# nunofachada/cl_ops

Measured on AMD Instinct MI355X. Metric: Mkeys/s sorting 2^28 uint32 (satradix, 4-bit digits); achieved % of HBM roofline, higher is better.
Workload: dtype u32

## Files before the change

### cl_ops_amd/_hip.py

```python
import ctypes as C
import os

_HERE = os.path.dirname(os.path.abspath(__file__))
LIB_PATH = os.environ.get("CLO_HIP_LIBRARY") or os.path.join(_HERE, "lib", "libcl_ops_hip.so")

if not os.path.exists(LIB_PATH):
    raise ImportError(
        "cl_ops_amd: %s is missing. Build it with `python -c 'import __graft_entry__ as g; g.build()'` "
        "or `make -C cl_ops_amd/csrc` (needs hipcc). There is no fallback path." % LIB_PATH)

lib = C.CDLL(LIB_PATH, mode=C.RTLD_GLOBAL)

vp, sz, ci = C.c_void_p, C.c_size_t, C.c_int


class DeviceProps(C.Structure):
    _fields_ = [("name", C.c_char * 128), ("compute_units", ci), ("max_threads_per_block", ci),
                ("wavefront_size", ci), ("lds_bytes_per_block", sz), ("global_mem_bytes", sz),
                ("gcn_arch", C.c_char * 64)]


def _sig(name, restype, *argtypes):
    try:
        f = getattr(lib, name)
    except AttributeError:
        if os.environ.get("CLO_HIP_LIBRARY"):
            return None
        raise
    f.restype = restype
    f.argtypes = list(argtypes)
    return f


_sig("clo_hip_device_count", ci, C.POINTER(ci))
_sig("clo_hip_set_device", ci, ci)
_sig("clo_hip_get_device", ci, C.POINTER(ci))
_sig("clo_hip_get_device_props", ci, ci, C.POINTER(DeviceProps))
_sig("clo_hip_stream_create", ci, C.POINTER(vp))
_sig("clo_hip_stream_create_high_priority", ci, C.POINTER(vp))
_sig("clo_hip_stream_destroy", ci, vp)
_sig("clo_hip_stream_synchronize", ci, vp)
_sig("clo_hip_malloc", ci, C.POINTER(vp), sz)
_sig("clo_hip_free", ci, vp)
_sig("clo_hip_memcpy_h2d_async", ci, vp, vp, sz, vp)
_sig("clo_hip_memcpy_d2h_async", ci, vp, vp, sz, vp)
_sig("clo_hip_memcpy_d2d_async", ci, vp, vp, sz, vp)
_sig("clo_hip_memset_async", ci, vp, ci, sz, vp)
_sig("clo_hip_host_register", ci, vp, sz)
_sig("clo_hip_host_unregister", ci, vp)
_sig("clo_hip_stream_is_capturing", ci, vp)
_sig("clo_hip_graph_capture_begin", ci, vp)
_sig("clo_hip_graph_capture_end", ci, vp, C.POINTER(vp))
_sig("clo_hip_graph_launch", ci, vp, vp)
_sig("clo_hip_graph_destroy", ci, vp)
_sig("clo_hip_timing_enabled", ci)
_sig("clo_hip_event_create", ci, C.POINTER(vp))
_sig("clo_hip_event_destroy", ci, vp)
_sig("clo_hip_event_record", ci, vp, vp)
_sig("clo_hip_event_synchronize", ci, vp)
_sig("clo_hip_event_query", ci, vp)
_sig("clo_hip_env_refresh", None)
_sig("clo_hip_event_elapsed_ms", ci, vp, vp, C.POINTER(C.c_float))
_sig("clo_hip_stream_wait_event", ci, vp, vp)
_sig("clo_hip_error_string", C.c_char_p, ci)
_sig("clo_hip_scan_workspace_bytes", sz, sz, ci, ci)
_sig("clo_hip_scan_workspace_init", ci, vp, sz, vp)
_sig("clo_hip_scan_workspace_forget", ci, vp)
_sig("clo_hip_scan_workspace_set_epoch", ci, vp, C.c_uint, vp)
_sig("clo_hip_scan_exclusive", ci, vp, vp, sz, ci, ci, ci, vp, sz, vp)
_sig("clo_hip_scan_exclusive_carry", ci, vp, vp, sz, ci, ci, ci, vp, vp, vp, sz, vp)
_sig("clo_hip_scan_fp_workspace_bytes", sz, sz, ci)
_sig("clo_hip_scan_is_typed", ci, ci, ci)
_sig("clo_hip_scan_typed_workspace_bytes", sz, sz, ci)
_sig("clo_hip_scan_exclusive_typed", ci, vp, vp, sz, ci, ci, vp, sz, vp)
_sig("clo_hip_scan_exclusive_fp", ci, vp, vp, sz, ci, ci, vp, sz, vp)
_sig("clo_hip_reduce_sum", ci, vp, sz, ci, ci, vp, vp)
_sig("clo_hip_radix_workspace_bytes", sz, sz, ci, ci, ci)
_sig("clo_hip_radix_polls", ci, sz, ci, ci)
_sig("clo_hip_radix_sort", ci, vp, vp, vp, sz, ci, ci, ci, ci, ci, vp, sz, vp)
_sig("clo_hip_radix_takes_first_digits", ci, sz, ci, ci, ci)
_sig("clo_hip_radix_sort_fed", ci, vp, vp, vp, sz, ci, ci, ci, ci, ci, vp, vp, sz, vp)
_sig("clo_hip_radix_seg_workspace_bytes", sz, sz, ci, ci, ci)
_sig("clo_hip_radix_sort_segmented", ci, vp, vp, vp, sz, C.POINTER(sz), ci, C.POINTER(sz), C.POINTER(sz), C.POINTER(ci), ci,
     ci, ci, ci, ci, vp, sz, vp, C.POINTER(ci))
_sig("clo_hip_radix_sort_segmented2", ci, vp, vp, vp, vp, sz, C.POINTER(sz), ci, C.POINTER(sz), C.POINTER(sz), C.POINTER(ci), C.POINTER(ci), ci,
     ci, ci, ci, ci, vp, sz, vp, C.POINTER(ci))
_sig("clo_hip_msd_histogram", ci, vp, sz, ci, ci, ci, ci, vp, vp)
_sig("clo_hip_msd_partition", ci, vp, vp, sz, ci, ci, ci, ci, vp, vp, sz, vp)
_sig("clo_hip_msd_workspace_bytes", sz, sz, ci, ci)
_sig("clo_hip_bitonic_padded_numel", sz, sz)
_sig("clo_hip_bitonic_simple", ci, vp, sz, ci, ci, ci, ci, ci, ci, C.POINTER(ci), vp)
_sig("clo_hip_bitonic_tiled", ci, vp, sz, ci, ci, ci, ci, ci, ci, C.POINTER(ci), vp)
_sig("clo_hip_bitonic_any", ci, vp, sz, ci, ci, ci, ci, ci, ci, C.POINTER(ci), vp)
_sig("clo_hip_kernel_lds_bytes", sz, C.c_char_p, ci, ci)
_sig("clo_hip_bitonic_jit_create", ci, ci, ci, C.c_char_p, C.c_char_p, C.c_char_p, C.POINTER(vp), C.POINTER(C.c_char_p))
_sig("clo_hip_bitonic_jit_destroy", None, vp)
_sig("clo_hip_bitonic_jit_sort", ci, vp, vp, sz, ci, C.POINTER(ci), vp)
_sig("clo_hip_bitonic_jit_gselect", ci, vp, vp, vp, sz, vp)
_sig("clo_hip_check_status", ci, vp, vp)
_sig("clo_hip_rccl_unique_id", ci, vp)
_sig("clo_hip_rccl_comm_create", ci, C.POINTER(vp), vp, ci, ci)
_sig("clo_hip_rccl_comm_destroy", ci, vp)
_sig("clo_hip_rccl_comm_abort", ci, vp)
_sig("clo_hip_rccl_all_gather_u64", ci, vp, vp, vp, sz, vp)
_sig("clo_hip_rccl_all_to_all_v", ci, vp, ci, ci, vp, vp, vp, vp, vp, vp, vp)
_sig("clo_hip_set_launch_observer", ci, vp, vp)
_sig("clo_hip_radix_jit_create", ci, ci, ci, C.c_char_p, C.c_char_p, C.POINTER(vp), C.POINTER(C.c_char_p))
_sig("clo_hip_radix_jit_destroy", None, vp)
_sig("clo_hip_radix_jit_sort", ci, vp, vp, vp, vp, vp, sz, ci, vp, sz, vp)
_sig("clo_hip_timing_enable", ci, ci)
_sig("clo_hip_timing_reset", ci)
_sig("clo_hip_timing_read", ci, C.c_char_p, C.POINTER(C.c_uint), C.POINTER(C.c_float))


CLO_HIP_EARGS, CLO_HIP_EUNSUPPORTED, CLO_HIP_EWORKSPACE, CLO_HIP_ETIMEOUT = -1, -2, -3, -4


class HipError(RuntimeError):
    def __init__(self, status, what=""):
        self.status = status
        msg = lib.clo_hip_error_string(status)
        super().__init__("%s: %s (status %d)" % (what or "clo_hip", msg.decode() if msg else "?", status))


def check(status, what=""):
    if status != 0:
        raise HipError(status, what)


def device_count():
    n = ci(0)
    st = lib.clo_hip_device_count(C.byref(n))
    return n.value if st == 0 else 0


def timing_read(label):
    n, ms = C.c_uint(0), C.c_float(0)
    check(lib.clo_hip_timing_read(label.encode(), C.byref(n), C.byref(ms)), "clo_hip_timing_read")
    return n.value, ms.value
```

### cl_ops_amd/csrc/hip/clo_hip_internal.h

```cpp
#ifndef CLO_HIP_INTERNAL_H
#define CLO_HIP_INTERNAL_H

#include <stddef.h>
#include <stdint.h>

#include "clo_hip.h"

#define CLO_WS_STATUS_OFFSET 0
#define CLO_WS_EPOCH_WORD    2
#define CLO_WS_DONE_WORD     3
#define CLO_WS_TICKET_WORD   16
#define CLO_WS_MAX_PASSES    64
#define CLO_WS_HEADER_BYTES  512

struct clo_hip_env_t { unsigned max_spins; int radix_sweep; int r1_pools; int no_digits; int bitonic_merge2; };
const clo_hip_env_t* clo_hip_env();
int clo_radixw_preload();

inline bool clo_misaligned(const void* p, size_t align) { return ((uintptr_t) p & (align - 1)) != 0; }
inline bool clo_ws_misaligned(const void* ws) { return clo_misaligned(ws, CLO_HIP_WORKSPACE_ALIGN); }

#ifdef __HIPCC__
#include <hip/hip_runtime.h>

void clo_timing_begin(const char* label, hipStream_t s);
void clo_timing_end(hipStream_t s);
struct clo_timing_scope {
	hipStream_t s;
	clo_timing_scope(const char* label, hipStream_t stream) : s(stream) { clo_timing_begin(label, s); }
	~clo_timing_scope() { clo_timing_end(s); }
};

struct clo_keyx {
	unsigned long long sign, field;
	int kind;
};
template <typename E>
__device__ __forceinline__ E clo_keyx_fwd(E x, const clo_keyx& k) {
	if (k.kind == 1) return (E) (x ^ (E) k.sign);
	if (k.kind == 2) return (E) (x ^ ((x & (E) k.sign) ? (E) k.field : (E) k.sign));
	return x;
}
template <typename E>
__device__ __forceinline__ E clo_keyx_inv(E x, const clo_keyx& k) {
	if (k.kind == 1) return (E) (x ^ (E) k.sign);
	if (k.kind == 2) return (E) (x ^ ((x & (E) k.sign) ? (E) k.sign : (E) k.field));
	return x;
}
inline clo_keyx clo_keyx_make(int kind, int key_shift, int key_bits) {
	clo_keyx k = { 0, 0, 0 };
	if (kind == 1 || kind == 2) {
		k.kind = kind;
		k.sign = 1ull << (key_shift + key_bits - 1);
		k.field = (key_bits >= 64 ? ~0ull : ((1ull << key_bits) - 1ull)) << key_shift;
	}
	return k;
}

struct clo_kv_io {
	const void* keys_in;
	const unsigned* values_in;
	void* keys_out;
	unsigned* values_out;
};

size_t clo_radix4_workspace_bytes(size_t n, int elem_size, int digit_bits, int key_bits);
int clo_radix4_sort_kv(const clo_kv_io& io, void* pairs_a, void* pairs_b, size_t n, int key_size, int key_shift,
	int key_bits, int digit_bits, clo_keyx kx, void* ws, hipStream_t s);
size_t clo_radix4_partition_workspace_bytes(size_t n, int elem_size, int bits);
int clo_radix4_partition(const void* src, void* dst, size_t n, int elem_size, unsigned shift, int bits,
	unsigned long long* counts, void* ws, hipStream_t s);
int clo_radix4_sort(const void* src, void* dst, void* tmp, size_t n, int elem_size, int key_shift,
	int key_bits, int digit_bits, clo_keyx kx, const unsigned char* first_dig, void* ws, hipStream_t s);
int clo_radix4_takes_first_digits(size_t n, int elem_size, int digit_bits);
size_t clo_radix4_lds_bytes(int elem_size, int digit_bits);
int clo_radix1_applies(size_t n, int elem_size, int digit_bits);
size_t clo_radix1_workspace_bytes(size_t n, int elem_size, int key_bits);
int clo_radix1_sort(const void* src, void* dst, void* tmp, size_t n, int elem_size, int key_shift, int key_bits,
	clo_keyx kx, void* ws, unsigned* status, hipStream_t s);
int clo_bitonic_tiled_e1(void* data, size_t numel, int key_shift, int key_bits, int key_size, int key_kind, int descending, int* launches, hipStream_t s);
int clo_bitonic_tiled_e2(void* data, size_t numel, int key_shift, int key_bits, int key_size, int key_kind, int descending, int* launches, hipStream_t s);
int clo_bitonic_tiled_e4(void* data, size_t numel, int key_shift, int key_bits, int key_size, int key_kind, int descending, int* launches, hipStream_t s);
int clo_bitonic_tiled_e8(void* data, size_t numel, int key_shift, int key_bits, int key_size, int key_kind, int descending, int* launches, hipStream_t s);
size_t clo_radixw_lds_bytes(int digit_bits);
struct clo_radix_counters { unsigned* thist; unsigned* toff; unsigned* partial; unsigned* tinfo; unsigned tiles; bool big; };
int clo_radixw_launch_tilehist(const void* in, size_t n, int elem_size, int bits, unsigned shift, unsigned mask,
	const clo_radix_counters& c, clo_keyx kx, hipStream_t s);
int clo_radixw_launch_tilehist_kv(const void* keys, size_t n, int key_size, int bits, unsigned shift, unsigned mask,
	const clo_radix_counters& c, clo_keyx kx, hipStream_t s);
int clo_radixw_launch_tilehist_bytes(const unsigned char* dig, size_t n, int elem_size, int bits, unsigned mask,
	const clo_radix_counters& c, hipStream_t s);
int clo_radixw_launch_offsets(int bits, const clo_radix_counters& c, const unsigned** dbase, hipStream_t s);
size_t clo_radixw_partial_rows(size_t tiles);

#define CLO_SEG_MAX 256
struct clo_seg_tile { unsigned in_base, count_seg, out_base, seg_n; };
struct clo_seg_chunk { unsigned t0, tend, c_first, seg_last; };
struct clo_seg_pieces {
	unsigned n[CLO_SEG_MAX], in_base[CLO_SEG_MAX];
	unsigned short seg[CLO_SEG_MAX];
};
struct clo_seg_tables { const clo_seg_tile* tiles; const clo_seg_chunk* chunks; unsigned ntiles, nchunks, nseg; };
int clo_radixw_launch_tilehist_seg(const void* in, const void* in2, const clo_seg_tables& sg, int elem_size, int bits, unsigned shift, unsigned mask,
	const clo_radix_counters& c, hipStream_t s);
int clo_radixw_launch_tilehist_bytes_seg(const unsigned char* dig, const clo_seg_tables& sg, int elem_size, int bits, unsigned mask,
	const clo_radix_counters& c, hipStream_t s);
int clo_radixw_launch_offsets_seg(int bits, const clo_radix_counters& c, const clo_seg_tables& sg, const unsigned** dbase, hipStream_t s);
size_t clo_radixw_partial_rows_seg(size_t chunks, size_t nseg);
int clo_radixw_seg_build(const size_t* piece_n, const size_t* piece_base, const int* piece_seg, const int* piece_src, int npieces, int nseg, size_t tile,
	clo_seg_tile* tiles, clo_seg_chunk* chunks, unsigned* ntiles, unsigned* nchunks, hipStream_t s);
void clo_radixw_seg_bounds(size_t numel, int npieces, int nseg, size_t tile, size_t* max_tiles, size_t* max_chunks);
size_t clo_radix4_seg_workspace_bytes(size_t n, int nseg, int elem_size, int digit_bits);
int clo_radix4_sort_segmented(const void* src, const void* src2, void* a, void* b, size_t n, const size_t* seg_counts, int nseg,
	const size_t* piece_n, const size_t* piece_base, const int* piece_seg, const int* piece_src, int npieces, int elem_size, int key_shift,
	int key_bits, int digit_bits, void* ws, hipStream_t s, int* result_in_b);

typedef unsigned long long clo_u64;

#define CLO_LB_EPOCH_MAX ((1u << 30) - 1u)
#define CLO_LB_AGG    1u
#define CLO_LB_PREFIX 2u

__device__ __forceinline__ clo_u64 clo_lb_pack(unsigned epoch, unsigned state, unsigned value) {
	return ((clo_u64) ((epoch << 2) | state) << 32) | value;
}
__device__ __forceinline__ unsigned clo_lb_tag(clo_u64 g) { return (unsigned) (g >> 32); }
__device__ __forceinline__ unsigned clo_lb_val(clo_u64 g) { return (unsigned) g; }

__device__ __forceinline__ clo_u64 clo_ld_agent(const clo_u64* p) {
	return __hip_atomic_load(p, __ATOMIC_RELAXED, __HIP_MEMORY_SCOPE_AGENT);
}
__device__ __forceinline__ void clo_st_agent(clo_u64* p, clo_u64 v) {
	__hip_atomic_store(p, v, __ATOMIC_RELAXED, __HIP_MEMORY_SCOPE_AGENT);
}

#define CLO_MAX_SPINS (1u << 22)

__device__ __forceinline__ unsigned clo_lane_id() {
	return __builtin_amdgcn_mbcnt_hi(~0u, __builtin_amdgcn_mbcnt_lo(~0u, 0u));
}

__device__ __forceinline__ unsigned clo_mbcnt(clo_u64 mask) {
	return __builtin_amdgcn_mbcnt_hi((unsigned) (mask >> 32),
		__builtin_amdgcn_mbcnt_lo((unsigned) mask, 0u));
}

__device__ __forceinline__ void clo_lds_barrier() {
	__builtin_amdgcn_fence(__ATOMIC_RELEASE, "workgroup", "local");
	__builtin_amdgcn_s_barrier();
	__builtin_amdgcn_fence(__ATOMIC_ACQUIRE, "workgroup", "local");
}

template <int CTRL, int ROW_MASK, typename T>
__device__ __forceinline__ T clo_dpp_add(T x) {
	static_assert(sizeof(T) == 4 || sizeof(T) == 8, "32- or 64-bit integers");
	if constexpr (sizeof(T) == 4) {
		return (T) ((unsigned) x + (unsigned) __builtin_amdgcn_update_dpp(0, (int) x, CTRL, ROW_MASK, 0xF, true));
	} else {
		const unsigned long long v = (unsigned long long) x;
		const unsigned lo = (unsigned) __builtin_amdgcn_update_dpp(0, (int) (unsigned) v, CTRL, ROW_MASK, 0xF, true);
		const unsigned hi = (unsigned) __builtin_amdgcn_update_dpp(0, (int) (unsigned) (v >> 32), CTRL, ROW_MASK, 0xF, true);
		return (T) (v + (((unsigned long long) hi << 32) | lo));
	}
}

template <typename T>
__device__ __forceinline__ T clo_wave_scan_inclusive(T x, unsigned lane) {
	(void) lane;
	x = clo_dpp_add<0x111, 0xF>(x);
	x = clo_dpp_add<0x112, 0xF>(x);
	x = clo_dpp_add<0x114, 0xF>(x);
	x = clo_dpp_add<0x118, 0xF>(x);
	x = clo_dpp_add<0x142, 0xA>(x);
	x = clo_dpp_add<0x143, 0xC>(x);
	return x;
}

template <typename T>
__device__ __forceinline__ T clo_wave_reduce_sum(T x) {
	const T incl = clo_wave_scan_inclusive<T>(x, 0u);
	if constexpr (sizeof(T) == 4) {
		return (T) (unsigned) __builtin_amdgcn_readlane((int) incl, 63);
	} else {
		const unsigned long long v = (unsigned long long) incl;
		const unsigned lo = (unsigned) __builtin_amdgcn_readlane((int) (unsigned) v, 63);
		const unsigned hi = (unsigned) __builtin_amdgcn_readlane((int) (unsigned) (v >> 32), 63);
		return (T) (((unsigned long long) hi << 32) | lo);
	}
}

#endif
#endif
```

### cl_ops_amd/csrc/hip/clo_hip_radix.hip

```cpp
#include <hip/hip_runtime.h>

#include "clo_hip.h"
#include "clo_hip_internal.h"

namespace {

constexpr int HIST_THREADS = 256;
constexpr int HIST_ITEMS = 16;

template <typename E>
__global__ __launch_bounds__(HIST_THREADS)
void clo_msd_hist_kernel(const E* __restrict__ in, size_t n, unsigned shift, unsigned mask,
	unsigned long long* __restrict__ counts) {
	__shared__ unsigned h[HIST_THREADS / 64][8];
	const unsigned tid = threadIdx.x, wave = tid >> 6;
	if (tid < (HIST_THREADS / 64) * 8) (&h[0][0])[tid] = 0;
	__syncthreads();
	const size_t chunk = (size_t) HIST_THREADS * HIST_ITEMS;
	for (size_t base = (size_t) blockIdx.x * chunk; base < n; base += (size_t) gridDim.x * chunk) {
		#pragma unroll
		for (int i = 0; i < HIST_ITEMS; ++i) {
			const size_t idx = base + (size_t) i * HIST_THREADS + tid;
			if (idx < n) atomicAdd(&h[wave][(unsigned) (in[idx] >> shift) & mask & 7u], 1u);
		}
	}
	__syncthreads();
	if (tid <= mask && tid < 8) {
		unsigned s = 0;
		#pragma unroll
		for (int w = 0; w < HIST_THREADS / 64; ++w) s += h[w][tid];
		if (s) atomicAdd(&counts[tid], (unsigned long long) s);
	}
}

template <typename E>
int msd_hist_impl(const void* src, size_t n, unsigned shift, unsigned mask, uint64_t* counts, hipStream_t s) {
	unsigned blocks = (unsigned) ((n + HIST_THREADS * HIST_ITEMS - 1) / (HIST_THREADS * HIST_ITEMS));
	if (blocks > 2048) blocks = 2048;
	if (blocks == 0) blocks = 1;
	hipLaunchKernelGGL((clo_msd_hist_kernel<E>), dim3(blocks), dim3(HIST_THREADS), 0, s,
		(const E*) src, n, shift, mask, (unsigned long long*) counts);
	return (int) hipGetLastError();
}

}

extern "C" {

size_t clo_hip_radix_workspace_bytes(size_t numel, int elem_size, int key_bits, int digit_bits) {
	if (digit_bits < 1 || digit_bits > 8 || key_bits < 1) return 0;
	return clo_radix4_workspace_bytes(numel, elem_size, digit_bits, key_bits);
}

int clo_hip_radix_polls(size_t numel, int elem_size, int digit_bits) {
	return clo_radix1_applies(numel, elem_size, digit_bits) ? 1 : 0;
}

int clo_hip_radix_takes_first_digits(size_t numel, int elem_size, int key_kind, int digit_bits) {
	return key_kind == 0 ? clo_radix4_takes_first_digits(numel, elem_size, digit_bits) : 0;
}

int clo_hip_radix_sort(const void* src, void* dst, void* tmp, size_t numel,
	int elem_size, int key_shift, int key_bits, int key_kind, int digit_bits,
	void* workspace, size_t workspace_bytes, void* stream) {
	return clo_hip_radix_sort_fed(src, dst, tmp, numel, elem_size, key_shift, key_bits, key_kind, digit_bits, nullptr,
		workspace, workspace_bytes, stream);
}

int clo_hip_radix_sort_fed(const void* src, void* dst, void* tmp, size_t numel,
	int elem_size, int key_shift, int key_bits, int key_kind, int digit_bits, const unsigned char* first_digits,
	void* workspace, size_t workspace_bytes, void* stream) {

	if (numel == 0) return 0;
	if (!src || !dst || !tmp || !workspace || tmp == src || tmp == dst || clo_ws_misaligned(workspace)) return CLO_HIP_EARGS;
	if (key_bits < 1 || key_shift < 0 || key_shift + key_bits > 8 * elem_size) return CLO_HIP_EARGS;
	if (key_kind < 0 || key_kind > 2) return CLO_HIP_EARGS;
	if (key_kind == 2 && key_bits != 16 && key_bits != 32 && key_bits != 64) return CLO_HIP_EARGS;
	if (digit_bits < 1 || digit_bits > 8) return CLO_HIP_EUNSUPPORTED;
	if (numel > 0xffffffffull) return CLO_HIP_EARGS;
	if (workspace_bytes < clo_hip_radix_workspace_bytes(numel, elem_size, key_bits, digit_bits)) return CLO_HIP_EWORKSPACE;
	hipStream_t s = (hipStream_t) stream;
	const clo_keyx kx = clo_keyx_make(key_kind, key_shift, key_bits);
	return clo_radix4_sort(src, dst, tmp, numel, elem_size, key_shift, key_bits, digit_bits, kx, first_digits, workspace, s);
}

size_t clo_hip_radix_kv_workspace_bytes(size_t numel, int key_size, int key_bits, int digit_bits) {
	if (key_size != 1 && key_size != 2 && key_size != 4) return 0;
	return clo_hip_radix_workspace_bytes(numel, 8, key_bits, digit_bits);
}

int clo_hip_radix_sort_kv(const void* keys_in, const void* values_in, void* keys_out, void* values_out, void* pairs_a, void* pairs_b,
	size_t numel, int key_size, int key_shift, int key_bits, int key_kind, int digit_bits,
	void* workspace, size_t workspace_bytes, void* stream) {
	if (numel == 0) return 0;
	if (!keys_in || !values_out || !pairs_a || !pairs_b || pairs_a == pairs_b || !workspace || clo_ws_misaligned(workspace)) return CLO_HIP_EARGS;
	const void* arrays[4] = { keys_in, values_in, keys_out, values_out };
	for (int i = 0; i < 4; ++i) if (arrays[i] == pairs_a || arrays[i] == pairs_b) return CLO_HIP_EARGS;
	if (key_size != 1 && key_size != 2 && key_size != 4) return CLO_HIP_EUNSUPPORTED;
	if (key_bits < 1 || key_shift < 0 || key_shift + key_bits > 8 * key_size) return CLO_HIP_EARGS;
	if (key_kind < 0 || key_kind > 2) return CLO_HIP_EARGS;
	if (key_kind == 2 && key_bits != 16 && key_bits != 32) return CLO_HIP_EARGS;
	if (digit_bits < 1 || digit_bits > 8) return CLO_HIP_EUNSUPPORTED;
	if (numel > 0xffffffffull) return CLO_HIP_EARGS;
	if (workspace_bytes < clo_hip_radix_kv_workspace_bytes(numel, key_size, key_bits, digit_bits)) return CLO_HIP_EWORKSPACE;
	const clo_kv_io io = { keys_in, (const unsigned*) values_in, keys_out, (unsigned*) values_out };
	const clo_keyx kx = clo_keyx_make(key_kind, 32 + key_shift, key_bits);
	return clo_radix4_sort_kv(io, pairs_a, pairs_b, numel, key_size, 32 + key_shift, key_bits, digit_bits, kx, workspace, (hipStream_t) stream);
}

int clo_hip_radix_preload(void) { return clo_radixw_preload(); }

size_t clo_hip_radix_seg_workspace_bytes(size_t numel, int nseg, int elem_size, int digit_bits) {
	return clo_radix4_seg_workspace_bytes(numel, nseg, elem_size, digit_bits);
}

int clo_hip_radix_sort_segmented(const void* src, void* a, void* b, size_t numel, const size_t* seg_counts, int nseg,
	const size_t* piece_counts, const size_t* piece_offsets, const int* piece_segment, int npieces,
	int elem_size, int key_shift, int key_bits, int digit_bits, void* workspace, size_t workspace_bytes, void* stream, int* result_in_b) {
	return clo_hip_radix_sort_segmented2(src, nullptr, a, b, numel, seg_counts, nseg, piece_counts, piece_offsets, piece_segment, nullptr, npieces,
		elem_size, key_shift, key_bits, digit_bits, workspace, workspace_bytes, stream, result_in_b);
}

int clo_hip_radix_sort_segmented2(const void* src, const void* src2, void* a, void* b, size_t numel, const size_t* seg_counts, int nseg,
	const size_t* piece_counts, const size_t* piece_offsets, const int* piece_segment, const int* piece_source, int npieces,
	int elem_size, int key_shift, int key_bits, int digit_bits, void* workspace, size_t workspace_bytes, void* stream, int* result_in_b) {
	if (!result_in_b) return CLO_HIP_EARGS;
	*result_in_b = 0;
	if (numel == 0) return 0;
	if (!src || !a || !b || a == b || src == b || !workspace || !seg_counts || nseg < 1 || nseg > CLO_SEG_MAX) return CLO_HIP_EARGS;
	if (clo_ws_misaligned(workspace)) return CLO_HIP_EARGS;
	if (npieces < 0 || npieces > CLO_SEG_MAX || (npieces > 0 && (!piece_counts || !piece_offsets || !piece_segment))) return CLO_HIP_EARGS;
	if (elem_size != 4 && elem_size != 8) return CLO_HIP_EUNSUPPORTED;
	if (digit_bits != 4 && digit_bits != 8) return CLO_HIP_EUNSUPPORTED;
	if (key_bits < 1 || key_shift < 0 || key_shift + key_bits > 8 * elem_size) return CLO_HIP_EARGS;
	if (numel > 0xffffffffull) return CLO_HIP_EARGS;
	size_t total = 0;
	for (int i = 0; i < nseg; ++i) total += seg_counts[i];
	if (total != numel) return CLO_HIP_EARGS;
	if (npieces > 0) {
		size_t per[CLO_SEG_MAX];
		for (int k = 0; k < nseg; ++k) per[k] = 0;
		for (int i = 0; i < npieces; ++i) {
			if (piece_segment[i] < 0 || piece_segment[i] >= nseg || piece_offsets[i] > 0xffffffffull || piece_counts[i] > numel) return CLO_HIP_EARGS;
			if (piece_source && piece_source[i] != 0 && (piece_source[i] != 1 || !src2 || src2 == b)) return CLO_HIP_EARGS;
			per[piece_segment[i]] += piece_counts[i];
		}
		for (int k = 0; k < nseg; ++k) if (per[k] != seg_counts[k]) return CLO_HIP_EARGS;
	}
	const size_t need = clo_radix4_seg_workspace_bytes(numel, nseg, elem_size, digit_bits);
	if (need == 0) return CLO_HIP_EUNSUPPORTED;
	if (workspace_bytes < need) return CLO_HIP_EWORKSPACE;
	return clo_radix4_sort_segmented(src, src2, a, b, numel, seg_counts, nseg, piece_counts, piece_offsets, piece_segment, npieces > 0 ? piece_source : nullptr, npieces,
		elem_size, key_shift, key_bits, digit_bits, workspace, (hipStream_t) stream, result_in_b);
}

size_t clo_hip_msd_workspace_bytes(size_t numel, int elem_size, int bucket_bits) {
	if (bucket_bits < 1 || bucket_bits > 8) return 0;
	return clo_radix4_partition_workspace_bytes(numel, elem_size, bucket_bits);
}

int clo_hip_msd_histogram(const void* src, size_t numel, int elem_size,
	int key_shift, int key_bits, int bucket_bits, uint64_t* counts_dev, void* stream) {
	if (!counts_dev || clo_misaligned(counts_dev, 8) || bucket_bits < 1 || bucket_bits > 3 || bucket_bits > key_bits) return CLO_HIP_EARGS;
	hipStream_t s = (hipStream_t) stream;
	hipError_t e = hipMemsetAsync(counts_dev, 0, sizeof(uint64_t) << bucket_bits, s);
	if (e != hipSuccess) return (int) e;
	if (numel == 0) return 0;
	if (!src) return CLO_HIP_EARGS;
	const unsigned shift = (unsigned) (key_shift + key_bits - bucket_bits), mask = (1u << bucket_bits) - 1u;
	switch (elem_size) {
		case 4: return msd_hist_impl<uint32_t>(src, numel, shift, mask, counts_dev, s);
		case 8: return msd_hist_impl<uint64_t>(src, numel, shift, mask, counts_dev, s);
		default: return CLO_HIP_EUNSUPPORTED;
	}
}

int clo_hip_msd_partition(const void* src, void* dst, size_t numel, int elem_size,
	int key_shift, int key_bits, int bucket_bits, uint64_t* counts_dev,
	void* workspace, size_t workspace_bytes, void* stream) {
	hipStream_t s = (hipStream_t) stream;
	if (bucket_bits < 1 || bucket_bits > 8 || bucket_bits > key_bits) return CLO_HIP_EARGS;
	if (clo_misaligned(counts_dev, 8) || clo_ws_misaligned(workspace)) return CLO_HIP_EARGS;
	if (numel == 0) {
		if (counts_dev) return (int) hipMemsetAsync(counts_dev, 0, sizeof(uint64_t) << bucket_bits, s);
		return 0;
	}
	if (!src || !dst || src == dst || !workspace) return CLO_HIP_EARGS;
	if (numel > 0xffffffffull) return CLO_HIP_EARGS;
	if (elem_size != 4 && elem_size != 8) return CLO_HIP_EUNSUPPORTED;
	if (workspace_bytes < clo_hip_msd_workspace_bytes(numel, elem_size, bucket_bits)) return CLO_HIP_EWORKSPACE;
	const unsigned shift = (unsigned) (key_shift + key_bits - bucket_bits);
	return clo_radix4_partition(src, dst, numel, elem_size, shift, bucket_bits,
		(unsigned long long*) counts_dev, workspace, s);
}

}
```

### cl_ops_amd/csrc/hip/clo_hip_radix4.hip

```cpp
#include <hip/hip_runtime.h>

#include <cstdlib>
#include <type_traits>

#include "clo_hip.h"
#include "clo_hip_internal.h"
#include "clo_hip_radix_rank.h"

namespace {

template <int KB> struct kv_key;
template <> struct kv_key<1> { typedef uint8_t type; };
template <> struct kv_key<2> { typedef uint16_t type; };
template <> struct kv_key<4> { typedef uint32_t type; };

template <int KB, int ITEMS>
__device__ __forceinline__ void kv_load_pairs(const clo_kv_io& kv, size_t at, unsigned valid, bool aligned, uint64_t (&pair)[ITEMS]) {
	typedef typename kv_key<KB>::type K;
	const K* kp = reinterpret_cast<const K*>(kv.keys_in) + at;
	K k[ITEMS];
	unsigned v[ITEMS];
	if (valid == (unsigned) ITEMS) {
		load_blocked<K, ITEMS>(kp, k, aligned);
		if (kv.values_in) {
			load_blocked<unsigned, ITEMS>(kv.values_in + at, v, aligned);
		} else {
			#pragma unroll
			for (int i = 0; i < ITEMS; ++i) v[i] = (unsigned) at + (unsigned) i;
		}
	} else {
		#pragma unroll
		for (int i = 0; i < ITEMS; ++i) {
			k[i] = (unsigned) i < valid ? kp[i] : (K) 0;
			v[i] = (unsigned) i < valid ? (kv.values_in ? kv.values_in[at + i] : (unsigned) at + (unsigned) i) : 0u;
		}
	}
	#pragma unroll
	for (int i = 0; i < ITEMS; ++i) pair[i] = ((uint64_t) k[i] << 32) | v[i];
}

template <int KB>
__device__ __forceinline__ void kv_store_pair(const clo_kv_io& kv, unsigned gi, uint64_t e) {
	typedef typename kv_key<KB>::type K;
	if (kv.keys_out) reinterpret_cast<K*>(kv.keys_out)[gi] = (K) (e >> 32);
	kv.values_out[gi] = (unsigned) e;
}

template <typename E, int LB, int HB, bool BIG, bool DIG = false, bool SEG = false, int KV_IN = 0, int KV_OUT = 0>
__global__ __launch_bounds__((pair_shape<E, BIG>::THREADS), (pair_shape<E, BIG>::THREADS >= 1024 ? 8 : 6))
void clo_radix4_pair_kernel(const E* __restrict__ in, E* __restrict__ out, size_t n,
	unsigned shift, unsigned mask_lo, unsigned mask_hi,
	const unsigned* __restrict__ thist, const unsigned* __restrict__ toff, const unsigned* __restrict__ dbase,
	const unsigned* __restrict__ tinfo, int aligned,
	clo_keyx kx_in, clo_keyx kx_out, unsigned char* __restrict__ dig_out = nullptr, unsigned next_shift = 0,
	const clo_seg_tile* __restrict__ tdesc = nullptr, const E* __restrict__ in2 = nullptr, clo_kv_io kv = clo_kv_io()) {
	static_assert((KV_IN == 0 && KV_OUT == 0) || (sizeof(E) == 8 && !SEG), "key-value passes: 8-byte pairs, one array");

	constexpr int THREADS = pair_shape<E, BIG>::THREADS;
	constexpr int ITEMS = pair_shape<E, BIG>::ITEMS;
	constexpr int TILE = THREADS * ITEMS;
	constexpr int WAVES = THREADS / 64;
	constexpr int R2 = 1 << (LB + HB);
	constexpr int HMAX = pc_words<(LB > HB ? LB : HB)>::H;
	static_assert(R2 <= 256 && R2 <= THREADS, "one thread per combined digit, scanned by the first four waves");

	__shared__ __attribute__((aligned(16))) E s_stage[TILE];
	constexpr bool ALIAS = pair_shape<E, BIG>::ALIAS;
	__shared__ unsigned s_end[ALIAS ? 1 : THREADS * PC_END_STRIDE];
	__shared__ unsigned s_wtot[WAVES][HMAX];
	__shared__ __attribute__((aligned(16))) unsigned s_wbase[WAVES][HMAX];
	__shared__ unsigned s_delta[R2];
	__shared__ unsigned s_w4[4];

	const unsigned tid = threadIdx.x, lane = tid & 63u, wave = tid >> 6;
	const unsigned per_xcd = SEG ? (unsigned) ((n + 7) / 8) : (unsigned) ((n + (size_t) TILE * 8 - 1) / ((size_t) TILE * 8));
	const unsigned tile = (blockIdx.x & 7u) * per_xcd + (blockIdx.x >> 3);
	size_t base = (size_t) tile * TILE;
	unsigned count, n32;
	if constexpr (SEG) {
		if (tile >= (unsigned) n) return;
		const clo_seg_tile td = tdesc[tile];
		base = (size_t) td.in_base;
		count = td.count_seg & 0xffffu;
		n32 = td.seg_n;
		out += td.out_base;
		if constexpr (DIG) dig_out += td.out_base;
		dbase += (size_t) ((td.count_seg >> 16) & 0x7fffu) * R2;
		if (td.count_seg >> 31) in = in2;
	} else {
		if (base >= n) return;
		count = (n - base) < (size_t) TILE ? (unsigned) (n - base) : (unsigned) TILE;
		n32 = n > 0xffffffffull ? 0xffffffffu : (unsigned) n;
	}
	const bool full = count == (unsigned) TILE;
	const unsigned tbase = tid * ITEMS;
	const unsigned mask2 = (mask_hi << LB) | mask_lo;

	__builtin_amdgcn_s_setprio(3);
	unsigned h2 = 0, goff = 0;
	if (tid < (unsigned) R2) {
		h2 = thist[(size_t) tile * R2 + tid];
		goff = toff[(size_t) tile * R2 + tid];
		if (dbase) goff += dbase[tid];
	}
	E key[ITEMS];
	if constexpr (KV_IN != 0) {
		kv_load_pairs<KV_IN, ITEMS>(kv, base + tbase, full ? (unsigned) ITEMS : (count > tbase ? count - tbase : 0u), aligned != 0, key);
	} else if (full) {
		if constexpr (SEG) load_blocked_unaligned<E, ITEMS>(in + base + tbase, key);
		else load_blocked<E, ITEMS>(in + base + tbase, key, aligned != 0);
	} else {
		#pragma unroll
		for (int i = 0; i < ITEMS; ++i) key[i] = (tbase + i < count) ? in[base + tbase + i] : (E) 0;
	}
	__builtin_amdgcn_s_setprio(0);
	if (kx_in.kind) {
		#pragma unroll
		for (int i = 0; i < ITEMS; ++i) key[i] = clo_keyx_fwd<E>(key[i], kx_in);
	}
	{
		const unsigned incl2 = clo_wave_scan_inclusive<unsigned>(h2, lane);
		if (lane == 63 && wave < 4) s_w4[wave] = incl2;
		if (tid < (unsigned) R2) s_delta[tid] = goff - (incl2 - h2);
	}

	const bool single = tinfo[tile] != 0u;

	if (!single) {
		pc_local_split<E, LB, THREADS, ITEMS, HMAX, pc_no_mid, pc_no_counted, ALIAS>(key, shift, mask_lo, count, s_stage, s_end, s_wtot, s_wbase);
	} else {
		if (full) {
			constexpr int PER = ITEMS * (int) sizeof(E) >= 16 ? 16 / (int) sizeof(E) : ITEMS;
			typedef E vec16 __attribute__((ext_vector_type(PER)));
			#pragma unroll
			for (int k = 0; k < ITEMS / PER; ++k) {
				vec16 t;
				#pragma unroll
				for (int q = 0; q < PER; ++q) t[q] = key[k * PER + q];
				*reinterpret_cast<vec16*>(&s_stage[tbase + k * PER]) = t;
			}
		} else {
			#pragma unroll
			for (int i = 0; i < ITEMS; ++i) if (tbase + i < count) s_stage[tbase + i] = key[i];
		}
		clo_lds_barrier();
	}

	if (tid < (unsigned) R2) {
		unsigned before = 0;
		#pragma unroll
		for (unsigned w = 0; w < 4; ++w) if (w < wave) before += s_w4[w];
		s_delta[tid] -= before;
	}
	if (single) {
		__syncthreads();
	} else if (mask_hi != 0) {
		if (full) {
			constexpr int PER = ITEMS * (int) sizeof(E) >= 16 ? 16 / (int) sizeof(E) : ITEMS;
			typedef E vec16 __attribute__((ext_vector_type(PER)));
			#pragma unroll
			for (int k = 0; k < ITEMS / PER; ++k) {
				const vec16 t = *reinterpret_cast<const vec16*>(&s_stage[tbase + k * PER]);
				#pragma unroll
				for (int q = 0; q < PER; ++q) key[k * PER + q] = t[q];
			}
		} else {
			#pragma unroll
			for (int i = 0; i < ITEMS; ++i) if (tbase + i < count) key[i] = s_stage[tbase + i];
		}
		pc_local_split<E, HB, THREADS, ITEMS, HMAX, pc_no_mid, pc_no_counted, ALIAS>(key, shift + LB, mask_hi, count, s_stage, s_end, s_wtot, s_wbase);
	} else {
		__syncthreads();
	}

	constexpr int VEC = sizeof(E) >= 8 ? 1 : 4;
	typedef E vecE __attribute__((ext_vector_type(VEC)));
	typedef E vecE_u __attribute__((ext_vector_type(VEC), aligned(sizeof(E))));
	const bool dig_bytes = DIG && VEC == 4 && (next_shift & 7u) == 0u && next_shift < 8u * (unsigned) sizeof(E);
	const unsigned dig_b = next_shift >> 3;
	const unsigned dig_sel_lo = 0x0c0c0400u + dig_b * 0x0101u, dig_sel_hi = 0x04000c0cu + dig_b * 0x01010000u;
	const unsigned nbits2 = (unsigned) __builtin_popcount(mask2);
	const auto scatter = [&](auto kx_tag) {
		constexpr bool KX = decltype(kx_tag)::value;
		#pragma unroll
		for (int j = 0; j < ITEMS / VEC; ++j) {
			const unsigned p = (j * THREADS + tid) * VEC;
			if (full) {
				const vecE v = *reinterpret_cast<const vecE*>(&s_stage[p]);
				const unsigned d0 = pc_digit<E>(v[0], shift, mask2, nbits2), dl = pc_digit<E>(v[VEC - 1], shift, mask2, nbits2);
				const unsigned gi0 = p + s_delta[d0];
				if (d0 == dl && gi0 <= n32 - VEC) {
					vecE vo = v;
					if constexpr (KX) {
						#pragma unroll
						for (int k = 0; k < VEC; ++k) vo[k] = clo_keyx_inv<E>(v[k], kx_out);
					}
					if constexpr (KV_OUT != 0) kv_store_pair<KV_OUT>(kv, gi0, vo[0]);
					else *reinterpret_cast<vecE_u*>(&out[gi0]) = vo;
					if constexpr (DIG) {
						if constexpr (VEC == 4) {
							typedef unsigned u32_u __attribute__((aligned(1)));
							unsigned dg;
							if (dig_bytes)
								dg = __builtin_amdgcn_perm((unsigned) v[1], (unsigned) v[0], dig_sel_lo) | __builtin_amdgcn_perm((unsigned) v[3], (unsigned) v[2], dig_sel_hi);
							else
								dg = ((unsigned) (v[0] >> next_shift) & 255u) | (((unsigned) (v[1] >> next_shift) & 255u) << 8)
									| (((unsigned) (v[2] >> next_shift) & 255u) << 16) | ((unsigned) (v[3] >> next_shift) << 24);
							*reinterpret_cast<u32_u*>(dig_out + gi0) = dg;
						} else {
							dig_out[gi0] = (unsigned char) (v[0] >> next_shift);
						}
					}
				} else {
					#pragma unroll
					for (int k = 0; k < VEC; ++k) {
						const unsigned gi = p + k + s_delta[pc_digit<E>(v[k], shift, mask2, nbits2)];
						if (gi < n32) {
							if constexpr (KV_OUT != 0) kv_store_pair<KV_OUT>(kv, gi, KX ? clo_keyx_inv<E>(v[k], kx_out) : v[k]);
							else out[gi] = KX ? clo_keyx_inv<E>(v[k], kx_out) : v[k];
							if constexpr (DIG) dig_out[gi] = (unsigned char) (v[k] >> next_shift);
						}
					}
				}
			} else {
				#pragma unroll
				for (int k = 0; k < VEC; ++k) {
					if (p + k < count) {
						const E e = s_stage[p + k];
						const unsigned gi = p + k + s_delta[pc_digit<E>(e, shift, mask2, nbits2)];
						if (gi < n32) {
							if constexpr (KV_OUT != 0) kv_store_pair<KV_OUT>(kv, gi, KX ? clo_keyx_inv<E>(e, kx_out) : e);
							else out[gi] = KX ? clo_keyx_inv<E>(e, kx_out) : e;
							if constexpr (DIG) dig_out[gi] = (unsigned char) (e >> next_shift);
						}
					}
				}
			}
		}
	};
	if (kx_out.kind) scatter(std::true_type()); else scatter(std::false_type());
}

constexpr int SMALL_TILE = 512 * 8;
template <typename E> struct small_big { static constexpr int THREADS = 1024, ITEMS = sizeof(E) == 8 ? 8 : 16, TILE = THREADS * ITEMS; };

template <typename E, int BITS, int THREADS, int ITEMS>
__global__ __launch_bounds__(THREADS)
void clo_radix4_small_kernel(const E* in, E* out, unsigned n, unsigned key_shift, unsigned key_bits, clo_keyx kx) {
	constexpr int H = pc_words<BITS>::H;
	constexpr int WAVES = THREADS / 64;
	__shared__ __attribute__((aligned(16))) E s_stage[THREADS * ITEMS];
	__shared__ unsigned s_end[THREADS * PC_END_STRIDE];
	__shared__ unsigned s_wtot[WAVES][H];
	__shared__ __attribute__((aligned(16))) unsigned s_wbase[WAVES][H];

	const unsigned tbase = threadIdx.x * ITEMS;
	E key[ITEMS];
	#pragma unroll
	for (int i = 0; i < ITEMS; ++i) key[i] = (tbase + i < n) ? clo_keyx_fwd<E>(in[tbase + i], kx) : (E) 0;
	for (unsigned done = 0; done < key_bits; done += BITS) {
		const unsigned bits = key_bits - done < (unsigned) BITS ? key_bits - done : (unsigned) BITS;
		pc_local_split<E, BITS, THREADS, ITEMS, H>(key, key_shift + done, (1u << bits) - 1u, n,
			s_stage, s_end, s_wtot, s_wbase);
		if constexpr (ITEMS * sizeof(E) >= 16) {
			constexpr int PER = 16 / (int) sizeof(E);
			typedef E vec16 __attribute__((ext_vector_type(PER)));
			#pragma unroll
			for (int k = 0; k < ITEMS / PER; ++k) {
				const vec16 t = *reinterpret_cast<const vec16*>(&s_stage[tbase + k * PER]);
				#pragma unroll
				for (int q = 0; q < PER; ++q) key[k * PER + q] = t[q];
			}
		} else {
			#pragma unroll
			for (int i = 0; i < ITEMS; ++i) if (tbase + i < n) key[i] = s_stage[tbase + i];
		}
	}
	#pragma unroll
	for (int i = 0; i < ITEMS; ++i) if (tbase + i < n) out[tbase + i] = clo_keyx_inv<E>(key[i], kx);
}


struct rp_layout { size_t thist, toff, partial, tinfo, dig, total, tiles; bool big; };

rp_layout rp_make_layout(size_t n, int elem_size, int pass_bits, bool digits = true) {
	rp_layout L;
	const size_t R2 = (size_t) 1 << pass_bits;
	L.big = clo_radix_big_tiles(n, elem_size);
	const size_t tile = clo_pair_tile_elems(elem_size, L.big);
	L.tiles = (n + tile - 1) / tile;
	if (L.tiles == 0) L.tiles = 1;
	const size_t per = L.tiles * R2 * sizeof(unsigned);
	L.thist = CLO_WS_HEADER_BYTES;
	L.toff = L.thist + per;
	L.partial = L.toff + per;
	L.tinfo = L.partial + ((clo_radixw_partial_rows(L.tiles) * R2 * sizeof(unsigned) + 255) & ~(size_t) 255);
	L.total = L.tinfo + ((L.tiles * sizeof(unsigned) + 255) & ~(size_t) 255);
	L.dig = 0;
	if (digits && clo_radix_digit_stream(n, elem_size)) {
		L.dig = L.total;
		L.total += (n + 255) & ~(size_t) 255;
	}
	return L;
}

template <typename Layout>
clo_radix_counters rp_counters(void* ws, const Layout& L, size_t tiles) {
	char* w = (char*) ws;
	return { (unsigned*) (w + L.thist), (unsigned*) (w + L.toff), (unsigned*) (w + L.partial), (unsigned*) (w + L.tinfo), (unsigned) tiles, L.big };
}

struct rp_digits { unsigned shift, mask_lo, mask_hi, mask, next_shift; };

template <int LB, int HB>
rp_digits rp_pass_digits(int p, int key_shift, int key_bits) {
	constexpr int PB = LB + HB;
	const int rem = key_bits - p * PB;
	const int bits = rem < PB ? rem : PB;
	const int lo_bits = bits < LB ? bits : LB, hi_bits = bits - lo_bits;
	rp_digits d;
	d.shift = (unsigned) (key_shift + p * PB);
	d.mask_lo = (1u << lo_bits) - 1u;
	d.mask_hi = (1u << hi_bits) - 1u;
	d.mask = (d.mask_hi << LB) | d.mask_lo;
	d.next_shift = d.shift + PB;
	return d;
}

template <typename E, int LB, int HB, bool SEG = false, int KB = 0>
void rp_launch_pass(const clo_radix_counters& c, const rp_digits& d, const E* in, E* out, size_t n, const unsigned* dbase, int aligned,
	clo_keyx kx_in, clo_keyx kx_out, unsigned char* dig_out, hipStream_t s, const clo_seg_tile* tdesc = nullptr, const E* in2 = nullptr,
	bool kv_in = false, bool kv_out = false, const clo_kv_io& kv = clo_kv_io()) {
	const unsigned tiles = SEG ? (unsigned) n : c.tiles;
	const auto launch = [&](auto big, auto dig, auto kvi, auto kvo) {
		constexpr bool BIG = decltype(big)::value, DIG = decltype(dig)::value;
		hipLaunchKernelGGL((clo_radix4_pair_kernel<E, LB, HB, BIG, DIG, SEG, decltype(kvi)::value, decltype(kvo)::value>),
			dim3((tiles + 7u) / 8u * 8u), dim3(pair_shape<E, BIG>::THREADS), 0, s,
			in, out, n, d.shift, d.mask_lo, d.mask_hi, c.thist, c.toff, dbase, c.tinfo, aligned, kx_in, kx_out, dig_out, d.next_shift, tdesc, in2, kv);
	};
	const auto shape = [&](auto kvi, auto kvo) {
		constexpr bool BIG_OK = sizeof(E) >= 4, DIG_OK = BIG_OK && LB == 4 && HB == 4 && decltype(kvo)::value == 0;
		if constexpr (DIG_OK) {
			if (c.big && dig_out) { launch(std::true_type(), std::true_type(), kvi, kvo); return; }
		}
		if constexpr (BIG_OK) {
			if (c.big) { launch(std::true_type(), std::false_type(), kvi, kvo); return; }
		}
		launch(std::false_type(), std::false_type(), kvi, kvo);
	};
	typedef std::integral_constant<int, 0> plain;
	typedef std::integral_constant<int, KB> key;
	if (kv_in && kv_out) shape(key(), key());
	else if (kv_in) shape(key(), plain());
	else if (kv_out) shape(plain(), key());
	else shape(plain(), plain());
}

int kv_unpack(const uint64_t* pairs, const clo_kv_io& io, size_t n, int key_size, hipStream_t s);

template <typename E, int LB, int HB, int KB = 0>
int rp_sort_impl(const E* src, E* dst, E* tmp, size_t n, int key_shift, int key_bits, clo_keyx kx, const unsigned char* first_dig,
	const clo_kv_io& kv, void* ws, hipStream_t s) {
	constexpr int PB = LB + HB;
	const int passes = (key_bits + PB - 1) / PB;
	const rp_layout L = rp_make_layout(n, (int) sizeof(E), PB);
	const clo_radix_counters c = rp_counters(ws, L, L.tiles);
	const bool no_dig = clo_hip_env()->no_digits != 0;
	constexpr bool DIG_OK = LB == 4 && HB == 4 && sizeof(E) >= 4;
	unsigned char* dig = (DIG_OK && L.dig != 0 && passes > 1 && !no_dig) ? (unsigned char*) ws + L.dig : nullptr;
	const clo_keyx kx_none = { 0, 0, 0 };
	const bool split_after = KB != 0 && passes == 1 && (kv.keys_out == kv.keys_in || (const void*) kv.values_out == (const void*) kv.values_in);
	const bool kv_aligned = (uintptr_t) kv.keys_in % 16 == 0 && (uintptr_t) kv.values_in % 16 == 0;

	hipError_t e;

	const bool inplace_odd = (dst == src) && (passes % 2 == 1);
	const E* cur_in = src;
	for (int p = 0; p < passes; ++p) {
		E* cur_out;
		if (inplace_odd) cur_out = (p % 2 == 0) ? tmp : dst;
		else cur_out = ((passes - 1 - p) % 2 == 0) ? dst : tmp;
		const bool kv_in = KB != 0 && p == 0, kv_out = KB != 0 && p + 1 == passes && !split_after;
		const rp_digits d = rp_pass_digits<LB, HB>(p, key_shift, key_bits);
		{
			clo_timing_scope timing("radix_hist", s);
			const unsigned char* hist_bytes = (dig && p > 0) ? dig : ((DIG_OK && c.big && p == 0 && kx.kind == 0) ? first_dig : nullptr);
			const int st = kv_in ? clo_radixw_launch_tilehist_kv(kv.keys_in, n, KB, PB, d.shift, d.mask, c, kx, s)
				: hist_bytes ? clo_radixw_launch_tilehist_bytes(hist_bytes, n, (int) sizeof(E), PB, d.mask, c, s)
				: clo_radixw_launch_tilehist(cur_in, n, (int) sizeof(E), PB, d.shift, d.mask, c, p == 0 ? kx : kx_none, s);
			if (st != 0) return st;
		}
		const unsigned* dbase = nullptr;
		{
			clo_timing_scope timing("radix_offsets", s);
			const int st = clo_radixw_launch_offsets(PB, c, &dbase, s);
			if (st != 0) return st;
		}
		{
			clo_timing_scope timing("radix_pass", s);
			const int aligned = kv_in ? (int) kv_aligned : (int) ((uintptr_t) cur_in % 16 == 0);
			rp_launch_pass<E, LB, HB, false, KB>(c, d, cur_in, cur_out, n, dbase, aligned, p == 0 ? kx : kx_none, p + 1 == passes ? kx : kx_none,
				p + 1 < passes ? dig : nullptr, s, nullptr, nullptr, kv_in, kv_out, kv);
		}
		cur_in = cur_out;
	}
	e = hipGetLastError();
	if (e != hipSuccess) return (int) e;
	if (inplace_odd) {
		e = hipMemcpyAsync(dst, tmp, n * sizeof(E), hipMemcpyDeviceToDevice, s);
		if (e != hipSuccess) return (int) e;
	}
	if constexpr (KB != 0) {
		if (split_after) return kv_unpack(dst, kv, n, KB, s);
	}
	return 0;
}

template <typename E>
int rp_dispatch(const void* src, void* dst, void* tmp, size_t n, int key_shift, int key_bits, int digit_bits,
	clo_keyx kx, const unsigned char* first_dig, void* ws, hipStream_t s) {
	#define CLO_RP(LB, HB) return rp_sort_impl<E, LB, HB>((const E*) src, (E*) dst, (E*) tmp, n, key_shift, key_bits, kx, first_dig, clo_kv_io(), ws, s)
	switch (digit_bits) {
		case 1: CLO_RP(1, 1);
		case 2: CLO_RP(2, 2);
		case 3: CLO_RP(3, 3);
		case 4: CLO_RP(4, 4);
		case 5: CLO_RP(3, 2);
		case 6: CLO_RP(3, 3);
		case 7: CLO_RP(4, 3);
		case 8: CLO_RP(4, 4);
		default: return CLO_HIP_EUNSUPPORTED;
	}
	#undef CLO_RP
}

template <int R, int R2>
__global__ __launch_bounds__(256)
void clo_radix4_counts_kernel(const unsigned* __restrict__ thist, unsigned tiles, unsigned long long* __restrict__ counts) {
	constexpr int G = 256 / R;
	__shared__ unsigned long long s_part[G][R];
	const unsigned tid = threadIdx.x, d = tid % R, g = tid / R;
	unsigned long long c = 0;
	for (unsigned t = g; t < tiles; t += G) c += thist[(size_t) t * R2 + d];
	s_part[g][d] = c;
	__syncthreads();
	if (tid < (unsigned) R) {
		unsigned long long tot = 0;
		#pragma unroll
		for (int k = 0; k < G; ++k) tot += s_part[k][tid];
		counts[tid] = tot;
	}
}

template <int R, int R2>
__global__ __launch_bounds__(256)
void clo_radix4_counts_from_bases_kernel(const unsigned* __restrict__ dbase, unsigned n, unsigned long long* __restrict__ counts) {
	const unsigned d = threadIdx.x;
	if (d < (unsigned) R) counts[d] = (unsigned long long) ((d + 1u < (unsigned) R2 ? dbase[d + 1u] : n) - dbase[d]);
}

template <typename E, int BITS, int LB, int HB>
int r4_partition_impl(const E* src, E* dst, size_t n, unsigned shift, unsigned long long* counts, void* ws, hipStream_t s) {
	constexpr unsigned R = 1u << BITS;
	constexpr int PB = LB + HB;
	constexpr bool TWO = BITS > 3;
	static_assert(TWO ? PB == BITS : (LB == BITS && HB == BITS), "see above");
	const rp_layout L = rp_make_layout(n, (int) sizeof(E), PB, false);
	const clo_radix_counters c = rp_counters(ws, L, L.tiles);
	const clo_keyx kx_none = { 0, 0, 0 };
	hipError_t e = hipMemsetAsync(ws, 0, CLO_WS_HEADER_BYTES, s);
	if (e != hipSuccess) return (int) e;
	clo_timing_scope timing("msd_partition", s);
	const rp_digits d = rp_pass_digits<LB, HB>(0, (int) shift, BITS);
	int st = clo_radixw_launch_tilehist(src, n, (int) sizeof(E), PB, d.shift, d.mask, c, kx_none, s);
	if (st != 0) return st;
	const unsigned* dbase = nullptr;
	st = clo_radixw_launch_offsets(PB, c, &dbase, s);
	if (st != 0) return st;
	if (counts) {
		if (dbase) hipLaunchKernelGGL((clo_radix4_counts_from_bases_kernel<R, (1 << PB)>), dim3(1), dim3(256), 0, s, dbase, (unsigned) n, counts);
		else hipLaunchKernelGGL((clo_radix4_counts_kernel<R, (1 << PB)>), dim3(1), dim3(256), 0, s, c.thist, c.tiles, counts);
	}
	rp_launch_pass<E, LB, HB>(c, d, src, dst, n, dbase, (int) ((uintptr_t) src % 16 == 0), kx_none, kx_none, nullptr, s);
	return (int) hipGetLastError();
}

struct rp_seg_layout { size_t thist, toff, partial, tinfo, tdesc, cdesc, dig, total, tile, max_tiles, max_chunks; bool big; };

rp_seg_layout rp_make_seg_layout(size_t n, int nseg, int elem_size) {
	rp_seg_layout L;
	const size_t R2 = 256;
	L.big = clo_radix_big_tiles(n, elem_size);
	L.tile = clo_pair_tile_elems(elem_size, L.big);
	clo_radixw_seg_bounds(n, CLO_SEG_MAX, nseg, L.tile, &L.max_tiles, &L.max_chunks);
	const size_t per = L.max_tiles * R2 * sizeof(unsigned);
	const auto up = [](size_t x) { return (x + 255) & ~(size_t) 255; };
	L.thist = CLO_WS_HEADER_BYTES;
	L.toff = L.thist + per;
	L.partial = L.toff + per;
	L.tinfo = L.partial + up(clo_radixw_partial_rows_seg(L.max_chunks, (size_t) nseg) * R2 * sizeof(unsigned));
	L.tdesc = L.tinfo + up(L.max_tiles * sizeof(unsigned));
	L.cdesc = L.tdesc + 2 * up(L.max_tiles * sizeof(clo_seg_tile));
	L.total = L.cdesc + 2 * up(L.max_chunks * sizeof(clo_seg_chunk));
	L.dig = 0;
	if (clo_radix_digit_stream(n, elem_size)) {
		L.dig = L.total;
		L.total += up(n);
	}
	return L;
}

template <typename E>
int rp_sort_seg_impl(const E* src, const E* src2, E* a, E* b, size_t n, const size_t* seg_counts, int nseg,
	const size_t* piece_n, const size_t* piece_base, const int* piece_seg, const int* piece_src, int npieces, int key_shift, int key_bits, void* ws,
	hipStream_t s, int* result_in_b) {
	constexpr int LB = 4, HB = 4, PB = 8;
	const int passes = (key_bits + PB - 1) / PB;
	const rp_seg_layout L = rp_make_seg_layout(n, nseg, (int) sizeof(E));
	const clo_radix_counters c = rp_counters(ws, L, 0);
	const auto up = [](size_t x) { return (x + 255) & ~(size_t) 255; };
	size_t seg_base[CLO_SEG_MAX];
	int seg_id[CLO_SEG_MAX];
	{
		size_t at = 0;
		for (int k = 0; k < nseg; ++k) { seg_base[k] = at; seg_id[k] = k; at += seg_counts[k]; }
	}
	clo_seg_tables sg0, sg;
	sg.tiles = (const clo_seg_tile*) ((char*) ws + L.tdesc);
	sg.chunks = (const clo_seg_chunk*) ((char*) ws + L.cdesc);
	sg.nseg = (unsigned) nseg;
	{
		clo_timing_scope timing("radix_seg_tables", s);
		int st = clo_radixw_seg_build(seg_counts, seg_base, seg_id, nullptr, nseg, nseg, L.tile, (clo_seg_tile*) sg.tiles, (clo_seg_chunk*) sg.chunks, &sg.ntiles, &sg.nchunks, s);
		if (st != 0) return st;
		sg0 = sg;
		if (npieces > 0) {
			sg0.tiles = (const clo_seg_tile*) ((char*) ws + L.tdesc + up(L.max_tiles * sizeof(clo_seg_tile)));
			sg0.chunks = (const clo_seg_chunk*) ((char*) ws + L.cdesc + up(L.max_chunks * sizeof(clo_seg_chunk)));
			st = clo_radixw_seg_build(piece_n, piece_base, piece_seg, piece_src, npieces, nseg, L.tile, (clo_seg_tile*) sg0.tiles, (clo_seg_chunk*) sg0.chunks, &sg0.ntiles, &sg0.nchunks, s);
			if (st != 0) return st;
		}
	}
	*result_in_b = passes % 2;
	if (sg.ntiles == 0) return 0;
	if (sg.ntiles > L.max_tiles || sg.nchunks > L.max_chunks || sg0.ntiles > L.max_tiles || sg0.nchunks > L.max_chunks)
		return CLO_HIP_EWORKSPACE;
	unsigned char* dig = (L.dig != 0 && passes > 1) ? (unsigned char*) ws + L.dig : nullptr;
	const clo_keyx kx_none = { 0, 0, 0 };
	const E* cur_in = src;
	for (int p = 0; p < passes; ++p) {
		const clo_seg_tables& sgp = p == 0 ? sg0 : sg;
		E* cur_out = p % 2 == 0 ? b : a;
		const rp_digits d = rp_pass_digits<LB, HB>(p, key_shift, key_bits);
		{
			clo_timing_scope timing("radix_hist", s);
			const int st = (dig && p > 0)
				? clo_radixw_launch_tilehist_bytes_seg(dig, sgp, (int) sizeof(E), PB, d.mask, c, s)
				: clo_radixw_launch_tilehist_seg(cur_in, p == 0 ? src2 : nullptr, sgp, (int) sizeof(E), PB, d.shift, d.mask, c, s);
			if (st != 0) return st;
		}
		const unsigned* dbase = nullptr;
		{
			clo_timing_scope timing("radix_offsets", s);
			const int st = clo_radixw_launch_offsets_seg(PB, c, sgp, &dbase, s);
			if (st != 0) return st;
		}
		{
			clo_timing_scope timing("radix_pass", s);
			rp_launch_pass<E, LB, HB, true>(c, d, cur_in, cur_out, (size_t) sgp.ntiles, dbase, 0, kx_none, kx_none, p + 1 < passes ? dig : nullptr, s,
				sgp.tiles, p == 0 ? src2 : nullptr);
		}
		cur_in = cur_out;
	}
	return (int) hipGetLastError();
}

template <typename E>
int small_dispatch(const void* src, void* dst, size_t n, int key_shift, int key_bits, int digit_bits, clo_keyx kx, hipStream_t s) {
	clo_timing_scope timing("radix_small", s);
	#define CLO_SMALL(B) case B: \
		if (n <= (size_t) SMALL_TILE) \
			hipLaunchKernelGGL((clo_radix4_small_kernel<E, B, 512, 8>), dim3(1), dim3(512), 0, s, \
				(const E*) src, (E*) dst, (unsigned) n, (unsigned) key_shift, (unsigned) key_bits, kx); \
		else if (n <= (size_t) 1024 * 8) \
			hipLaunchKernelGGL((clo_radix4_small_kernel<E, B, 1024, 8>), dim3(1), dim3(1024), 0, s, \
				(const E*) src, (E*) dst, (unsigned) n, (unsigned) key_shift, (unsigned) key_bits, kx); \
		else \
			hipLaunchKernelGGL((clo_radix4_small_kernel<E, B, small_big<E>::THREADS, small_big<E>::ITEMS>), dim3(1), dim3(small_big<E>::THREADS), 0, s, \
				(const E*) src, (E*) dst, (unsigned) n, (unsigned) key_shift, (unsigned) key_bits, kx); \
		break
	switch (digit_bits) {
		CLO_SMALL(1); CLO_SMALL(2); CLO_SMALL(3); CLO_SMALL(4);
		default: return CLO_HIP_EUNSUPPORTED;
	}
	#undef CLO_SMALL
	return (int) hipGetLastError();
}

constexpr int KV_PACK_THREADS = 256;

template <typename K>
__global__ __launch_bounds__(KV_PACK_THREADS)
void clo_radix_kv_pack_kernel(const K* __restrict__ keys, const unsigned* __restrict__ values, uint64_t* __restrict__ pairs, size_t n) {
	for (size_t i = (size_t) blockIdx.x * KV_PACK_THREADS + threadIdx.x; i < n; i += (size_t) gridDim.x * KV_PACK_THREADS)
		pairs[i] = ((uint64_t) keys[i] << 32) | (values ? values[i] : (unsigned) i);
}

template <typename K>
__global__ __launch_bounds__(KV_PACK_THREADS)
void clo_radix_kv_unpack_kernel(const uint64_t* __restrict__ pairs, K* __restrict__ keys, unsigned* __restrict__ values, size_t n) {
	for (size_t i = (size_t) blockIdx.x * KV_PACK_THREADS + threadIdx.x; i < n; i += (size_t) gridDim.x * KV_PACK_THREADS) {
		const uint64_t e = pairs[i];
		if (keys) keys[i] = (K) (e >> 32);
		values[i] = (unsigned) e;
	}
}

unsigned kv_pack_grid(size_t n) {
	const size_t g = (n + KV_PACK_THREADS - 1) / KV_PACK_THREADS;
	return (unsigned) (g < 8192 ? (g ? g : 1) : 8192);
}

int kv_pack(const clo_kv_io& io, uint64_t* pairs, size_t n, int key_size, hipStream_t s) {
	clo_timing_scope timing("radix_kv_pack", s);
	#define CLO_KVP(K) hipLaunchKernelGGL((clo_radix_kv_pack_kernel<K>), dim3(kv_pack_grid(n)), dim3(KV_PACK_THREADS), 0, s, (const K*) io.keys_in, io.values_in, pairs, n)
	switch (key_size) {
		case 1: CLO_KVP(uint8_t); break;
		case 2: CLO_KVP(uint16_t); break;
		case 4: CLO_KVP(uint32_t); break;
		default: return CLO_HIP_EUNSUPPORTED;
	}
	#undef CLO_KVP
	return (int) hipGetLastError();
}

int kv_unpack(const uint64_t* pairs, const clo_kv_io& io, size_t n, int key_size, hipStream_t s) {
	clo_timing_scope timing("radix_kv_unpack", s);
	#define CLO_KVU(K) hipLaunchKernelGGL((clo_radix_kv_unpack_kernel<K>), dim3(kv_pack_grid(n)), dim3(KV_PACK_THREADS), 0, s, pairs, (K*) io.keys_out, io.values_out, n)
	switch (key_size) {
		case 1: CLO_KVU(uint8_t); break;
		case 2: CLO_KVU(uint16_t); break;
		case 4: CLO_KVU(uint32_t); break;
		default: return CLO_HIP_EUNSUPPORTED;
	}
	#undef CLO_KVU
	return (int) hipGetLastError();
}

}

static size_t r4_pair_workspace_bytes(size_t n, int elem_size, int digit_bits) {
	return (rp_make_layout(n, elem_size, digit_bits <= 4 ? 2 * digit_bits : digit_bits).total + 255) & ~(size_t) 255;
}

size_t clo_radix4_workspace_bytes(size_t n, int elem_size, int digit_bits, int key_bits) {
	size_t b = r4_pair_workspace_bytes(n, elem_size, digit_bits);
	if (clo_radix1_applies(n, elem_size, digit_bits)) b += clo_radix1_workspace_bytes(n, elem_size, key_bits);
	return b;
}

size_t clo_radix4_seg_workspace_bytes(size_t n, int nseg, int elem_size, int digit_bits) {
	if ((digit_bits != 4 && digit_bits != 8) || (elem_size != 4 && elem_size != 8) || nseg < 1 || nseg > CLO_SEG_MAX) return 0;
	return rp_make_seg_layout(n, nseg, elem_size).total;
}

int clo_radix4_sort_segmented(const void* src, const void* src2, void* a, void* b, size_t n, const size_t* seg_counts, int nseg,
	const size_t* piece_n, const size_t* piece_base, const int* piece_seg, const int* piece_src, int npieces, int elem_size, int key_shift,
	int key_bits, int digit_bits, void* ws, hipStream_t s, int* result_in_b) {
	if (digit_bits != 4 && digit_bits != 8) return CLO_HIP_EUNSUPPORTED;
	if (elem_size == 4) return rp_sort_seg_impl<uint32_t>((const uint32_t*) src, (const uint32_t*) src2, (uint32_t*) a, (uint32_t*) b, n, seg_counts, nseg, piece_n, piece_base, piece_seg, piece_src, npieces, key_shift, key_bits, ws, s, result_in_b);
	if (elem_size == 8) return rp_sort_seg_impl<uint64_t>((const uint64_t*) src, (const uint64_t*) src2, (uint64_t*) a, (uint64_t*) b, n, seg_counts, nseg, piece_n, piece_base, piece_seg, piece_src, npieces, key_shift, key_bits, ws, s, result_in_b);
	return CLO_HIP_EUNSUPPORTED;
}

size_t clo_radix4_partition_workspace_bytes(size_t n, int elem_size, int bits) {
	return rp_make_layout(n, elem_size, bits <= 3 ? 2 * bits : bits, false).total;
}

int clo_radix4_partition(const void* src, void* dst, size_t n, int elem_size, unsigned shift, int bits,
	unsigned long long* counts, void* ws, hipStream_t s) {
	#define CLO_R4P(E, B, LB, HB) return r4_partition_impl<E, B, LB, HB>((const E*) src, (E*) dst, n, shift, counts, ws, s)
	if (elem_size == 4) {
		if (bits == 1) CLO_R4P(uint32_t, 1, 1, 1);
		if (bits == 2) CLO_R4P(uint32_t, 2, 2, 2);
		if (bits == 3) CLO_R4P(uint32_t, 3, 3, 3);
		if (bits == 4) CLO_R4P(uint32_t, 4, 2, 2);
		if (bits == 5) CLO_R4P(uint32_t, 5, 3, 2);
		if (bits == 6) CLO_R4P(uint32_t, 6, 3, 3);
		if (bits == 7) CLO_R4P(uint32_t, 7, 4, 3);
		if (bits == 8) CLO_R4P(uint32_t, 8, 4, 4);
	} else if (elem_size == 8) {
		if (bits == 1) CLO_R4P(uint64_t, 1, 1, 1);
		if (bits == 2) CLO_R4P(uint64_t, 2, 2, 2);
		if (bits == 3) CLO_R4P(uint64_t, 3, 3, 3);
		if (bits == 4) CLO_R4P(uint64_t, 4, 2, 2);
		if (bits == 5) CLO_R4P(uint64_t, 5, 3, 2);
		if (bits == 6) CLO_R4P(uint64_t, 6, 3, 3);
		if (bits == 7) CLO_R4P(uint64_t, 7, 4, 3);
		if (bits == 8) CLO_R4P(uint64_t, 8, 4, 4);
	}
	#undef CLO_R4P
	return CLO_HIP_EUNSUPPORTED;
}

size_t clo_radix4_lds_bytes(int elem_size, int digit_bits) {
	const size_t threads = 512;
	const int half = digit_bits <= 4 ? digit_bits : (digit_bits + 1) / 2;
	const size_t hmax = half >= 4 ? 8 : (half == 3 ? 4 : (half == 2 ? 2 : 1));
	const size_t pass_bits = digit_bits <= 4 ? 2 * digit_bits : digit_bits;
	const size_t items = elem_size == 8 ? 8 : 16;
	return threads * items * (size_t) elem_size + threads * PC_END_STRIDE * sizeof(unsigned)
		+ (2 * (threads / 64) * hmax + ((size_t) 1 << pass_bits) + 4) * sizeof(unsigned);
}

int clo_radix4_takes_first_digits(size_t n, int elem_size, int digit_bits) {
	if (elem_size < 4 || (digit_bits != 4 && digit_bits != 8) || clo_hip_env()->no_digits) return 0;
	if (clo_radix1_applies(n, elem_size, digit_bits)) return 0;
	return clo_radix_big_tiles(n, elem_size) ? 1 : 0;
}

int clo_radix4_sort(const void* src, void* dst, void* tmp, size_t n, int elem_size, int key_shift,
	int key_bits, int digit_bits, clo_keyx kx, const unsigned char* first_dig, void* ws, hipStream_t s) {
	const size_t small_max = elem_size == 8 ? (size_t) small_big<uint64_t>::TILE : (size_t) small_big<uint32_t>::TILE;
	if (n <= small_max && digit_bits <= 4) {
		switch (elem_size) {
			case 1: return small_dispatch<uint8_t>(src, dst, n, key_shift, key_bits, digit_bits, kx, s);
			case 2: return small_dispatch<uint16_t>(src, dst, n, key_shift, key_bits, digit_bits, kx, s);
			case 4: return small_dispatch<uint32_t>(src, dst, n, key_shift, key_bits, digit_bits, kx, s);
			case 8: return small_dispatch<uint64_t>(src, dst, n, key_shift, key_bits, digit_bits, kx, s);
			default: return CLO_HIP_EUNSUPPORTED;
		}
	}
	if (clo_radix1_applies(n, elem_size, digit_bits))
		return clo_radix1_sort(src, dst, tmp, n, elem_size, key_shift, key_bits, kx,
			(char*) ws + r4_pair_workspace_bytes(n, elem_size, digit_bits), (unsigned*) ws, s);
	switch (elem_size) {
		case 1: return rp_dispatch<uint8_t>(src, dst, tmp, n, key_shift, key_bits, digit_bits, kx, first_dig, ws, s);
		case 2: return rp_dispatch<uint16_t>(src, dst, tmp, n, key_shift, key_bits, digit_bits, kx, first_dig, ws, s);
		case 4: return rp_dispatch<uint32_t>(src, dst, tmp, n, key_shift, key_bits, digit_bits, kx, first_dig, ws, s);
		case 8: return rp_dispatch<uint64_t>(src, dst, tmp, n, key_shift, key_bits, digit_bits, kx, first_dig, ws, s);
		default: return CLO_HIP_EUNSUPPORTED;
	}
}

int clo_radix4_sort_kv(const clo_kv_io& io, void* pairs_a, void* pairs_b, size_t n, int key_size, int key_shift,
	int key_bits, int digit_bits, clo_keyx kx, void* ws, hipStream_t s) {
	uint64_t* pa = (uint64_t*) pairs_a;
	uint64_t* pb = (uint64_t*) pairs_b;
	const bool small = n <= (size_t) small_big<uint64_t>::TILE && digit_bits <= 4;
	if ((digit_bits == 4 || digit_bits == 8) && !small && !clo_radix1_applies(n, 8, digit_bits)) {
		switch (key_size) {
			case 1: return rp_sort_impl<uint64_t, 4, 4, 1>(nullptr, pa, pb, n, key_shift, key_bits, kx, nullptr, io, ws, s);
			case 2: return rp_sort_impl<uint64_t, 4, 4, 2>(nullptr, pa, pb, n, key_shift, key_bits, kx, nullptr, io, ws, s);
			case 4: return rp_sort_impl<uint64_t, 4, 4, 4>(nullptr, pa, pb, n, key_shift, key_bits, kx, nullptr, io, ws, s);
			default: return CLO_HIP_EUNSUPPORTED;
		}
	}
	int st = kv_pack(io, pa, n, key_size, s);
	if (st == 0) st = clo_radix4_sort(pa, pa, pb, n, 8, key_shift, key_bits, digit_bits, kx, nullptr, ws, s);
	if (st == 0) st = kv_unpack(pa, io, n, key_size, s);
	return st;
}
```

### cl_ops_amd/csrc/hip/clo_hip_radixw.hip

```cpp
#include <hip/hip_runtime.h>

#include <type_traits>

#include "clo_hip.h"
#include "clo_hip_internal.h"
#include "clo_hip_radix_rank.h"

namespace {

constexpr int RW_CHUNK = 128;

template <typename E, bool BIG> struct rw_shape {
	static constexpr int TILE = pair_shape<E, BIG>::TILE;
	static constexpr int THREADS = pair_shape<E, BIG>::THREADS;
	static constexpr int ITEMS = TILE / THREADS;
	static constexpr bool STREAM = BIG && sizeof(E) == 4;
};

__device__ __forceinline__ void rw_clear(unsigned* __restrict__ clear, unsigned clear_words, unsigned i) {
	if (i < clear_words) clear[i] = 0u;
}


__device__ __forceinline__ void rw_tile_info(unsigned h, unsigned count, unsigned* __restrict__ tinfo, unsigned tile) {
	if (h == count) tinfo[tile] = 1u;
	else if (h != 0u) tinfo[tile] = 0u;
}

__device__ __forceinline__ bool rw_seg_tile(const clo_seg_tile* __restrict__ tdesc, size_t& base, unsigned& count, unsigned tile_elems) {
	const clo_seg_tile td = tdesc[blockIdx.x];
	base = (size_t) td.in_base;
	count = td.count_seg & 0xffffu;
	(void) tile_elems;
	return (td.count_seg >> 31) != 0u;
}

template <typename E, int BITS, bool BIG, bool SEG = false, int TPW = 1, typename L = E>
__global__ __launch_bounds__((rw_shape<E, BIG>::THREADS))
void clo_radixw_tilehist_kernel(const L* __restrict__ in, size_t n, unsigned shift, unsigned mask,
	unsigned* __restrict__ thist, unsigned* __restrict__ tinfo, int aligned, clo_keyx kx,
	unsigned* __restrict__ clear, unsigned clear_words, const clo_seg_tile* __restrict__ tdesc = nullptr, const L* __restrict__ in2 = nullptr) {
	static_assert(!SEG || TPW == 1, "segmented launches: one tile per work-group");
	static_assert(std::is_same<L, E>::value || (sizeof(E) == 8 && sizeof(L) <= 4 && !SEG), "keys of a key-value sort: 8-byte pairs");
	const auto widen = [](L x) -> E {
		if constexpr (std::is_same<L, E>::value) return x;
		else return (E) x << 32;
	};
	constexpr int R = 1 << BITS;
	constexpr int TILE = rw_shape<E, BIG>::TILE;
	constexpr int RW_THREADS = rw_shape<E, BIG>::THREADS;
	constexpr int PART = RW_THREADS / TPW;
	constexpr int ITEMS = TILE / PART;
	static_assert(PART % 64 == 0 && PART * TPW == RW_THREADS, "whole waves per tile");
	constexpr int VB = ITEMS * (int) sizeof(L) >= 16 ? 16 : ITEMS * (int) sizeof(L);
	constexpr int VECS = ITEMS * (int) sizeof(L) / VB;
	constexpr int PER = VB / (int) sizeof(L);
	constexpr bool STREAM = rw_shape<E, BIG>::STREAM;
	constexpr int COPIES = 32;
	__shared__ __attribute__((aligned(16))) unsigned s_cnt[TPW * R * COPIES];
	const unsigned tid = threadIdx.x, lane = tid & 63u;
	const unsigned part = tid / PART, ptid = tid % PART;
	const unsigned tile = blockIdx.x * TPW + part;
	size_t base = (size_t) tile * TILE;
	unsigned count = base >= n ? 0u : ((n - base) < (size_t) TILE ? (unsigned) (n - base) : (unsigned) TILE);
	if constexpr (SEG) { if (rw_seg_tile(tdesc, base, count, (unsigned) TILE)) in = in2; }
	const unsigned tbase = ptid * ITEMS;
	unsigned* const cnt = s_cnt + part * (R * COPIES) + (lane & (COPIES - 1));
	typedef L vecA __attribute__((ext_vector_type(PER)));
	typedef L vecU __attribute__((ext_vector_type(PER), aligned(sizeof(L))));
	typedef typename std::conditional<SEG, vecU, vecA>::type vecE;
	const bool whole = count == (unsigned) TILE && (aligned || SEG);
	vecE v[VECS];
	if (whole) {
		const vecE* p = reinterpret_cast<const vecE*>(in + base) + ptid;
		#pragma unroll
		for (int k = 0; k < VECS; ++k) v[k] = STREAM ? __builtin_nontemporal_load(p + k * PART) : p[k * PART];
	}
	{
		typedef unsigned vec4u __attribute__((ext_vector_type(4)));
		const vec4u z = { 0u, 0u, 0u, 0u };
		for (unsigned i = tid; i < (unsigned) (TPW * R * COPIES / 4); i += RW_THREADS) reinterpret_cast<vec4u*>(s_cnt)[i] = z;
	}
	clo_lds_barrier();
	if (whole) {
		#pragma unroll
		for (int k = 0; k < VECS; ++k) {
			#pragma unroll
			for (int q = 0; q < PER; ++q)
				atomicAdd(&cnt[((unsigned) (clo_keyx_fwd<E>(widen(v[k][q]), kx) >> shift) & mask) << 5], 1u);
		}
	} else {
		#pragma unroll
		for (int i = 0; i < ITEMS; ++i)
			if (tbase + i < count)
				atomicAdd(&cnt[((unsigned) (clo_keyx_fwd<E>(widen(in[base + tbase + i]), kx) >> shift) & mask) << 5], 1u);
	}
	__syncthreads();
	for (unsigned i = tid; i < (unsigned) (TPW * R); i += RW_THREADS) {
		typedef unsigned vec4u __attribute__((ext_vector_type(4)));
		const unsigned row_part = i / R, d = i % R, rt = blockIdx.x * TPW + row_part;
		unsigned rcount = count;
		if constexpr (TPW > 1) {
			const size_t rb = (size_t) rt * TILE;
			if (rb >= n) break;
			rcount = (n - rb) < (size_t) TILE ? (unsigned) (n - rb) : (unsigned) TILE;
		}
		const vec4u* row = reinterpret_cast<const vec4u*>(&s_cnt[row_part * (R * COPIES) + d * COPIES]);
		unsigned h = 0;
		#pragma unroll
		for (int k = 0; k < COPIES / 4; ++k) {
			const vec4u x = row[(k + d) & (COPIES / 4 - 1)];
			h += x[0] + x[1] + x[2] + x[3];
		}
		thist[(size_t) rt * R + d] = h;
		rw_tile_info(h, rcount, tinfo, rt);
		rw_clear(clear, clear_words, rt * R + d);
		if constexpr (SEG) rw_clear(clear, clear_words, (gridDim.x + rt) * R + d);
	}
}

template <int BITS, int ITEMS, int THREADS, bool SEG = false, int TPW = 1, bool UA = false>
__global__ __launch_bounds__(THREADS)
void clo_radixw_tilehist_bytes_kernel(const unsigned char* __restrict__ dig, size_t n, unsigned tiles, unsigned mask, unsigned* __restrict__ thist,
	unsigned* __restrict__ tinfo, unsigned* __restrict__ clear, unsigned clear_words, const clo_seg_tile* __restrict__ tdesc = nullptr) {
	constexpr int R = 1 << BITS;
	constexpr int PART = THREADS / TPW;
	constexpr int TILE = PART * ITEMS;
	constexpr int COPIES = 32;
	constexpr bool STREAM = ITEMS == 32;
	static_assert(PART % 64 == 0 && PART * TPW == THREADS, "whole waves per tile");
	__shared__ __attribute__((aligned(16))) unsigned s_cnt[TPW * R * COPIES];
	const unsigned tid = threadIdx.x, lane = tid & 63u;
	const unsigned part = tid / PART, ptid = tid % PART;
	const unsigned t = blockIdx.x * TPW + part;
	size_t base = (size_t) t * TILE;
	unsigned count = 0;
	if (t < tiles) {
		count = (n - base) < (size_t) TILE ? (unsigned) (n - base) : (unsigned) TILE;
		if constexpr (SEG) {
			const clo_seg_tile td = tdesc[t];
			base = (size_t) td.in_base;
			count = td.count_seg & 0xffffu;
		}
	}
	const unsigned tbase = ptid * ITEMS;
	unsigned* const cnt = s_cnt + part * (R * COPIES) + (lane & (COPIES - 1));
	typedef unsigned vecA __attribute__((ext_vector_type(ITEMS / 4)));
	typedef unsigned vecU __attribute__((ext_vector_type(ITEMS / 4), aligned(1)));
	typedef typename std::conditional<SEG || UA, vecU, vecA>::type vecw;
	vecw v;
	if (count == (unsigned) TILE) {
		typedef unsigned q4A __attribute__((ext_vector_type(4)));
		typedef unsigned q4U __attribute__((ext_vector_type(4), aligned(1)));
		typedef typename std::conditional<SEG || UA, q4U, q4A>::type q4;
		static_assert(ITEMS % 16 == 0, "whole 16-byte vectors per thread");
		const q4* p = reinterpret_cast<const q4*>(dig + base) + ptid;
		#pragma unroll
		for (int k = 0; k < ITEMS / 16; ++k) {
			const q4 x = STREAM ? __builtin_nontemporal_load(p + k * PART) : p[k * PART];
			#pragma unroll
			for (int q = 0; q < 4; ++q) v[k * 4 + q] = x[q];
		}
	}
	{
		typedef unsigned vec4u __attribute__((ext_vector_type(4)));
		const vec4u z = { 0u, 0u, 0u, 0u };
		for (unsigned i = tid; i < (unsigned) (TPW * R * COPIES / 4); i += THREADS) reinterpret_cast<vec4u*>(s_cnt)[i] = z;
	}
	clo_lds_barrier();
	if (count == (unsigned) TILE) {
		#pragma unroll
		for (int k = 0; k < ITEMS / 4; ++k) {
			#pragma unroll
			for (int b = 0; b < 4; ++b)
				atomicAdd(&cnt[(((unsigned) v[k] >> (8 * b)) & mask) << 5], 1u);
		}
	} else {
		#pragma unroll
		for (int i = 0; i < ITEMS; ++i)
			if (tbase + i < count) atomicAdd(&cnt[((unsigned) dig[base + tbase + i] & mask) << 5], 1u);
	}
	__syncthreads();
	for (unsigned i = tid; i < (unsigned) (TPW * R); i += THREADS) {
		typedef unsigned vec4u __attribute__((ext_vector_type(4)));
		const unsigned row_part = i / R, d = i % R, rt = blockIdx.x * TPW + row_part;
		if (rt >= tiles) break;
		const vec4u* row = reinterpret_cast<const vec4u*>(&s_cnt[row_part * (R * COPIES) + d * COPIES]);
		unsigned h = 0;
		#pragma unroll
		for (int k = 0; k < COPIES / 4; ++k) {
			const vec4u x = row[(k + d) & (COPIES / 4 - 1)];
			h += x[0] + x[1] + x[2] + x[3];
		}
		unsigned rcount;
		if constexpr (SEG) rcount = tdesc[rt].count_seg & 0xffffu;
		else { const size_t rb = (size_t) rt * TILE; rcount = (n - rb) < (size_t) TILE ? (unsigned) (n - rb) : (unsigned) TILE; }
		thist[(size_t) rt * R + d] = h;
		rw_tile_info(h, rcount, tinfo, rt);
		rw_clear(clear, clear_words, rt * R + d);
		if constexpr (SEG) rw_clear(clear, clear_words, (tiles + rt) * R + d);
	}
}

constexpr int RW_CS_THREADS = 1024;
constexpr int RW_CHUNK_SMALL = 32;
constexpr unsigned RW_SMALL_TILES = 2048;
constexpr int rw_chunk_for(unsigned tiles) { return tiles <= RW_SMALL_TILES ? RW_CHUNK_SMALL : RW_CHUNK; }
template <int R, int CHUNK = RW_CHUNK> struct rw_cs {
	static constexpr int G = (RW_CS_THREADS / R) < CHUNK ? (RW_CS_THREADS / R) : CHUNK;
	static constexpr int SUB = CHUNK / G;
	static_assert(G * SUB == CHUNK && G * R <= RW_CS_THREADS, "the groups tile the chunk");
};

constexpr unsigned RW_WRITTEN = 0x80000000u;
template <int R, bool SEG = false, int CHUNK = RW_CHUNK>
__global__ __launch_bounds__(RW_CS_THREADS)
void clo_radixw_offsets_lb_kernel(const unsigned* __restrict__ thist, unsigned tiles, unsigned chunks,
	unsigned* __restrict__ partial, unsigned* __restrict__ toff, const clo_seg_chunk* __restrict__ cdesc = nullptr) {
	constexpr int G = rw_cs<R, CHUNK>::G, SUB = rw_cs<R, CHUNK>::SUB;
	constexpr int GA = RW_CS_THREADS / R;
	constexpr int LB = 8;
	__shared__ unsigned s_p[G * R], s_lb[GA * R], s_w[4], s_c;
	const unsigned tid = threadIdx.x, d = tid % R, g = tid / R, lane = tid & 63u, wave = tid >> 6;
	if (tid == 0) s_c = __hip_atomic_fetch_add(&partial[(size_t) chunks * R], 1u, __ATOMIC_RELAXED, __HIP_MEMORY_SCOPE_AGENT);
	__syncthreads();
	const unsigned c = s_c;
	unsigned t0 = c * CHUNK;
	unsigned tend = t0 + CHUNK < tiles ? t0 + CHUNK : tiles;
	unsigned c_first = 0u, dbase_row = chunks + 1u;
	bool last = c + 1u == chunks;
	if constexpr (SEG) {
		const clo_seg_chunk cd = cdesc[c];
		t0 = cd.t0; tend = cd.tend; c_first = cd.c_first;
		last = (cd.seg_last >> 31) != 0u;
		dbase_row = chunks + 1u + (cd.seg_last & 0x7fffffffu);
	}
	const bool active = g < (unsigned) G;
	unsigned v[SUB];
	if (active) {
		#pragma unroll
		for (int k = 0; k < SUB; ++k) {
			const unsigned t = t0 + g * SUB + k;
			v[k] = t < tend ? thist[(size_t) t * R + d] : 0u;
		}
		unsigned own = 0;
		#pragma unroll
		for (int k = 0; k < SUB; ++k) own += v[k];
		s_p[g * R + d] = own;
	}
	__syncthreads();
	unsigned tot = 0;
	if (tid < (unsigned) R) {
		#pragma unroll 8
		for (int k = 0; k < G; ++k) tot += s_p[k * R + tid];
		__hip_atomic_store(&partial[(size_t) c * R + tid], tot | RW_WRITTEN, __ATOMIC_RELAXED, __HIP_MEMORY_SCOPE_AGENT);
	}
	unsigned acc = 0;
	for (unsigned b = c_first + g; b < c; b += (unsigned) (GA * LB)) {
		unsigned x[LB];
		bool ok;
		do {
			#pragma unroll
			for (int k = 0; k < LB; ++k) {
				const unsigned cc = b + (unsigned) (k * GA);
				x[k] = cc < c ? __hip_atomic_load(&partial[(size_t) cc * R + d], __ATOMIC_RELAXED, __HIP_MEMORY_SCOPE_AGENT) : RW_WRITTEN;
			}
			ok = true;
			#pragma unroll
			for (int k = 0; k < LB; ++k) ok = ok && (x[k] & RW_WRITTEN) != 0u;
			if (!ok) __builtin_amdgcn_s_sleep(1);
		} while (!ok);
		#pragma unroll
		for (int k = 0; k < LB; ++k) acc += x[k] & ~RW_WRITTEN;
	}
	s_lb[g * R + d] = acc;
	__syncthreads();
	unsigned before = 0;
	#pragma unroll 8
	for (int k = 0; k < GA; ++k) before += s_lb[k * R + d];
	if (last) {
		const unsigned t = tid < (unsigned) R ? before + tot : 0u;
		const unsigned incl = clo_wave_scan_inclusive<unsigned>(t, lane);
		if (lane == 63 && wave < 4) s_w[wave] = incl;
		__syncthreads();
		if (tid < (unsigned) R) {
			unsigned dbase = incl - t;
			#pragma unroll
			for (unsigned w = 0; w < 4; ++w) if (w < wave) dbase += s_w[w];
			partial[(size_t) dbase_row * R + tid] = dbase;
		}
	}
	if (!active) return;
	unsigned run = before;
	for (unsigned k = 0; k < g; ++k) run += s_p[k * R + d];
	#pragma unroll
	for (int k = 0; k < SUB; ++k) {
		const unsigned t = t0 + g * SUB + k;
		if (t < tend) toff[(size_t) t * R + d] = run;
		run += v[k];
	}
}

template <int R>
__global__ __launch_bounds__(256)
void clo_radixw_offsets1_kernel(const unsigned* __restrict__ thist, unsigned tiles, unsigned* __restrict__ toff) {
	constexpr int G = 256 / R;
	constexpr int SUB = RW_CHUNK / G;
	__shared__ unsigned s_a[G][R], s_base[R], s_w[4];
	const unsigned tid = threadIdx.x, d = tid % R, g = tid / R, lane = tid & 63u, wave = tid >> 6;
	const unsigned ts = g * SUB < tiles ? g * SUB : tiles;
	const unsigned te = ts + SUB < tiles ? ts + SUB : tiles;
	unsigned own = 0;
	#pragma unroll 8
	for (unsigned t = ts; t < te; ++t) own += thist[(size_t) t * R + d];
	s_a[g][d] = own;
	__syncthreads();
	unsigned before = 0, tot = 0;
	#pragma unroll
	for (int k = 0; k < G; ++k) {
		const unsigned v = s_a[k][d];
		if ((unsigned) k < g) before += v;
		tot += v;
	}
	const unsigned t0 = tid < (unsigned) R ? tot : 0u;
	const unsigned incl = clo_wave_scan_inclusive<unsigned>(t0, lane);
	if (lane == 63) s_w[wave] = incl;
	__syncthreads();
	if (tid < (unsigned) R) {
		unsigned dbase = incl - t0;
		#pragma unroll
		for (unsigned w = 0; w < 4; ++w) if (w < wave) dbase += s_w[w];
		s_base[tid] = dbase;
	}
	__syncthreads();
	unsigned run = s_base[d] + before;
	#pragma unroll 8
	for (unsigned t = ts; t < te; ++t) {
		const unsigned c = thist[(size_t) t * R + d];
		toff[(size_t) t * R + d] = run;
		run += c;
	}
}

constexpr int SEG_BUILD_THREADS = 1024;
__global__ __launch_bounds__(SEG_BUILD_THREADS)
void clo_radix_seg_build_kernel(clo_seg_pieces pc, unsigned npieces, unsigned tile, unsigned ntiles, unsigned nchunks,
	clo_seg_tile* __restrict__ tdesc, clo_seg_chunk* __restrict__ cdesc) {
	__shared__ unsigned s_pt[CLO_SEG_MAX + 1], s_sn[CLO_SEG_MAX], s_stl[CLO_SEG_MAX], s_ob[CLO_SEG_MAX + 1], s_st[CLO_SEG_MAX + 1], s_sc[CLO_SEG_MAX + 1], s_w[4][4];
	const unsigned tid = threadIdx.x, lane = tid & 63u, wave = tid >> 6;
	if (tid < (unsigned) CLO_SEG_MAX) { s_sn[tid] = 0u; s_stl[tid] = 0u; }
	__syncthreads();
	unsigned pn = 0, ptl = 0;
	if (tid < npieces) {
		pn = pc.n[tid];
		ptl = (pn + tile - 1u) / tile;
		atomicAdd(&s_sn[pc.seg[tid] & 0x7fffu], pn);
		atomicAdd(&s_stl[pc.seg[tid] & 0x7fffu], ptl);
	}
	__syncthreads();
	if (tid < (unsigned) CLO_SEG_MAX) {
		const unsigned sn = s_sn[tid], stl = s_stl[tid], sch = (stl + (unsigned) RW_CHUNK - 1u) / (unsigned) RW_CHUNK;
		const unsigned i0 = clo_wave_scan_inclusive<unsigned>(ptl, lane), i1 = clo_wave_scan_inclusive<unsigned>(sn, lane),
			i2 = clo_wave_scan_inclusive<unsigned>(stl, lane), i3 = clo_wave_scan_inclusive<unsigned>(sch, lane);
		if (lane == 63u) { s_w[0][wave] = i0; s_w[1][wave] = i1; s_w[2][wave] = i2; s_w[3][wave] = i3; }
		s_pt[tid + 1] = i0; s_ob[tid + 1] = i1; s_st[tid + 1] = i2; s_sc[tid + 1] = i3;
	}
	__syncthreads();
	if (tid < (unsigned) CLO_SEG_MAX) {
		unsigned b0 = 0, b1 = 0, b2 = 0, b3 = 0;
		for (unsigned w = 0; w < wave; ++w) { b0 += s_w[0][w]; b1 += s_w[1][w]; b2 += s_w[2][w]; b3 += s_w[3][w]; }
		s_pt[tid + 1] += b0; s_ob[tid + 1] += b1; s_st[tid + 1] += b2; s_sc[tid + 1] += b3;
		if (tid == 0) s_pt[0] = s_ob[0] = s_st[0] = s_sc[0] = 0u;
	}
	__syncthreads();
	const unsigned i = blockIdx.x * SEG_BUILD_THREADS + tid;
	if (i < ntiles) {
		unsigned lo = 0, hi = CLO_SEG_MAX;
		while (hi - lo > 1u) { const unsigned mid = (lo + hi) >> 1; if (s_pt[mid] <= i) lo = mid; else hi = mid; }
		const unsigned off = (i - s_pt[lo]) * tile, left = pc.n[lo] - off, sg = pc.seg[lo] & 0x7fffu, from2 = pc.seg[lo] >> 15;
		clo_seg_tile td;
		td.in_base = pc.in_base[lo] + off;
		td.count_seg = (left < tile ? left : tile) | (sg << 16) | (from2 << 31);
		td.out_base = s_ob[sg];
		td.seg_n = s_sn[sg];
		tdesc[i] = td;
	}
	if (i < nchunks) {
		unsigned lo = 0, hi = CLO_SEG_MAX;
		while (hi - lo > 1u) { const unsigned mid = (lo + hi) >> 1; if (s_sc[mid] <= i) lo = mid; else hi = mid; }
		clo_seg_chunk cd;
		cd.t0 = s_st[lo] + (i - s_sc[lo]) * (unsigned) RW_CHUNK;
		cd.tend = cd.t0 + (unsigned) RW_CHUNK < s_st[lo + 1] ? cd.t0 + (unsigned) RW_CHUNK : s_st[lo + 1];
		cd.c_first = s_sc[lo];
		cd.seg_last = lo | (i + 1u == s_sc[lo + 1] ? 0x80000000u : 0u);
		cdesc[i] = cd;
	}
}

}

void clo_radixw_seg_bounds(size_t numel, int npieces, int nseg, size_t tile, size_t* max_tiles, size_t* max_chunks) {
	*max_tiles = numel / tile + (size_t) npieces;
	*max_chunks = *max_tiles / RW_CHUNK + (size_t) nseg;
}

int clo_radixw_seg_build(const size_t* piece_n, const size_t* piece_base, const int* piece_seg, const int* piece_src, int npieces, int nseg, size_t tile,
	clo_seg_tile* tiles, clo_seg_chunk* chunks, unsigned* ntiles, unsigned* nchunks, hipStream_t s) {
	if (nseg < 1 || nseg > CLO_SEG_MAX || npieces < 1 || npieces > CLO_SEG_MAX) return CLO_HIP_EARGS;
	clo_seg_pieces c;
	size_t seg_tiles[CLO_SEG_MAX];
	for (int k = 0; k < CLO_SEG_MAX; ++k) seg_tiles[k] = 0;
	size_t nt = 0, nc = 0, total = 0;
	int prev = 0;
	for (int i = 0; i < CLO_SEG_MAX; ++i) {
		const size_t n = i < npieces ? piece_n[i] : 0;
		const int sg = i < npieces ? piece_seg[i] : prev;
		if (n > 0xffffffffull || sg < prev || sg >= nseg) return CLO_HIP_EARGS;
		prev = sg;
		c.n[i] = (unsigned) n;
		c.in_base[i] = i < npieces ? (unsigned) piece_base[i] : 0u;
		c.seg[i] = (unsigned short) (sg | ((i < npieces && piece_src && piece_src[i]) ? 0x8000 : 0));
		const size_t t = (n + tile - 1) / tile;
		seg_tiles[sg] += t;
		nt += t;
		total += n;
	}
	for (int k = 0; k < nseg; ++k) nc += (seg_tiles[k] + RW_CHUNK - 1) / RW_CHUNK;
	if (total > 0xffffffffull) return CLO_HIP_EARGS;
	*ntiles = (unsigned) nt;
	*nchunks = (unsigned) nc;
	if (nt == 0) return 0;
	hipLaunchKernelGGL(clo_radix_seg_build_kernel, dim3((unsigned) ((nt + SEG_BUILD_THREADS - 1) / SEG_BUILD_THREADS)), dim3(SEG_BUILD_THREADS), 0, s,
		c, (unsigned) npieces, (unsigned) tile, (unsigned) nt, (unsigned) nc, tiles, chunks);
	return (int) hipGetLastError();
}

size_t clo_radixw_partial_rows_seg(size_t chunks, size_t nseg) { return chunks + 1 + nseg; }

template <typename E>
static int rw_launch_tilehist_seg(const void* in, const void* in2, const clo_seg_tables& sg, int bits, unsigned shift, unsigned mask,
	const clo_radix_counters& c, hipStream_t s) {
	const unsigned clear_words = (sg.nchunks + 1u) << bits;
	const clo_keyx kx_none = { 0, 0, 0 };
	if (bits != 8) return CLO_HIP_EUNSUPPORTED;
	if (c.big) hipLaunchKernelGGL((clo_radixw_tilehist_kernel<E, 8, true, true>), dim3(sg.ntiles), dim3(rw_shape<E, true>::THREADS), 0, s,
		(const E*) in, (size_t) 0, shift, mask, c.thist, c.tinfo, 0, kx_none, c.partial, clear_words, sg.tiles, (const E*) in2);
	else hipLaunchKernelGGL((clo_radixw_tilehist_kernel<E, 8, false, true>), dim3(sg.ntiles), dim3(rw_shape<E, false>::THREADS), 0, s,
		(const E*) in, (size_t) 0, shift, mask, c.thist, c.tinfo, 0, kx_none, c.partial, clear_words, sg.tiles, (const E*) in2);
	return (int) hipGetLastError();
}

int clo_radixw_launch_tilehist_seg(const void* in, const void* in2, const clo_seg_tables& sg, int elem_size, int bits, unsigned shift, unsigned mask,
	const clo_radix_counters& c, hipStream_t s) {
	switch (elem_size) {
		case 4: return rw_launch_tilehist_seg<uint32_t>(in, in2, sg, bits, shift, mask, c, s);
		case 8: return rw_launch_tilehist_seg<uint64_t>(in, in2, sg, bits, shift, mask, c, s);
		default: return CLO_HIP_EUNSUPPORTED;
	}
}

int clo_radixw_launch_tilehist_bytes_seg(const unsigned char* dig, const clo_seg_tables& sg, int elem_size, int bits, unsigned mask,
	const clo_radix_counters& c, hipStream_t s) {
	const unsigned clear_words = (sg.nchunks + 1u) << bits;
	if (bits != 8 || !c.big) return CLO_HIP_EUNSUPPORTED;
	if (elem_size == 8) hipLaunchKernelGGL((clo_radixw_tilehist_bytes_kernel<8, 16, 1024, true, 2>), dim3((sg.ntiles + 1u) / 2u), dim3(1024), 0, s,
		dig, (size_t) 0, sg.ntiles, mask, c.thist, c.tinfo, c.partial, clear_words, sg.tiles);
	else if (elem_size == 4) hipLaunchKernelGGL((clo_radixw_tilehist_bytes_kernel<8, 32, 1024, true, 2>), dim3((sg.ntiles + 1u) / 2u), dim3(1024), 0, s,
		dig, (size_t) 0, sg.ntiles, mask, c.thist, c.tinfo, c.partial, clear_words, sg.tiles);
	else return CLO_HIP_EUNSUPPORTED;
	return (int) hipGetLastError();
}

int clo_radixw_launch_offsets_seg(int bits, const clo_radix_counters& c, const clo_seg_tables& sg, const unsigned** dbase, hipStream_t s) {
	if (bits != 8) return CLO_HIP_EUNSUPPORTED;
	hipLaunchKernelGGL((clo_radixw_offsets_lb_kernel<256, true>), dim3(sg.nchunks), dim3(RW_CS_THREADS), 0, s,
		c.thist, sg.ntiles, sg.nchunks, c.partial, c.toff, sg.chunks);
	*dbase = c.partial + ((size_t) (sg.nchunks + 1u) << bits);
	return (int) hipGetLastError();
}


unsigned clo_radixw_clear_words(int bits, unsigned tiles);

template <typename E>
static int rw_launch_tilehist(const void* in, size_t n, int bits, unsigned shift, unsigned mask, const clo_radix_counters& c, clo_keyx kx,
	hipStream_t s) {
	const int aligned = (int) ((uintptr_t) in % 16 == 0);
	const unsigned clear_words = c.partial ? clo_radixw_clear_words(bits, c.tiles) : 0u;
	#define CLO_RW_TH(B) case B: \
		if (c.big && sizeof(E) >= 4) hipLaunchKernelGGL((clo_radixw_tilehist_kernel<E, B, (sizeof(E) >= 4)>), dim3(c.tiles), dim3(rw_shape<E, (sizeof(E) >= 4)>::THREADS), 0, s, \
			(const E*) in, n, shift, mask, c.thist, c.tinfo, aligned, kx, c.partial, clear_words); \
		else hipLaunchKernelGGL((clo_radixw_tilehist_kernel<E, B, false>), dim3(c.tiles), dim3(rw_shape<E, false>::THREADS), 0, s, \
			(const E*) in, n, shift, mask, c.thist, c.tinfo, aligned, kx, c.partial, clear_words); \
		break
	switch (bits) {
		CLO_RW_TH(1); CLO_RW_TH(2); CLO_RW_TH(3); CLO_RW_TH(4); CLO_RW_TH(5); CLO_RW_TH(6); CLO_RW_TH(7); CLO_RW_TH(8);
		default: return CLO_HIP_EUNSUPPORTED;
	}
	#undef CLO_RW_TH
	return (int) hipGetLastError();
}

int clo_radixw_launch_tilehist(const void* in, size_t n, int elem_size, int bits, unsigned shift, unsigned mask,
	const clo_radix_counters& c, clo_keyx kx, hipStream_t s) {
	switch (elem_size) {
		case 1: return rw_launch_tilehist<uint8_t>(in, n, bits, shift, mask, c, kx, s);
		case 2: return rw_launch_tilehist<uint16_t>(in, n, bits, shift, mask, c, kx, s);
		case 4: return rw_launch_tilehist<uint32_t>(in, n, bits, shift, mask, c, kx, s);
		case 8: return rw_launch_tilehist<uint64_t>(in, n, bits, shift, mask, c, kx, s);
		default: return CLO_HIP_EUNSUPPORTED;
	}
}

template <typename K>
static int rw_launch_tilehist_kv(const void* keys, size_t n, unsigned shift, unsigned mask, const clo_radix_counters& c, clo_keyx kx, hipStream_t s) {
	const int aligned = (int) ((uintptr_t) keys % 16 == 0);
	const unsigned clear_words = c.partial ? clo_radixw_clear_words(8, c.tiles) : 0u;
	if (c.big)
		hipLaunchKernelGGL((clo_radixw_tilehist_kernel<uint64_t, 8, true, false, 1, K>), dim3(c.tiles), dim3(rw_shape<uint64_t, true>::THREADS), 0, s,
			(const K*) keys, n, shift, mask, c.thist, c.tinfo, aligned, kx, c.partial, clear_words, nullptr, nullptr);
	else
		hipLaunchKernelGGL((clo_radixw_tilehist_kernel<uint64_t, 8, false, false, 1, K>), dim3(c.tiles), dim3(rw_shape<uint64_t, false>::THREADS), 0, s,
			(const K*) keys, n, shift, mask, c.thist, c.tinfo, aligned, kx, c.partial, clear_words, nullptr, nullptr);
	return (int) hipGetLastError();
}

int clo_radixw_launch_tilehist_kv(const void* keys, size_t n, int key_size, int bits, unsigned shift, unsigned mask,
	const clo_radix_counters& c, clo_keyx kx, hipStream_t s) {
	if (bits != 8) return CLO_HIP_EUNSUPPORTED;
	switch (key_size) {
		case 1: return rw_launch_tilehist_kv<uint8_t>(keys, n, shift, mask, c, kx, s);
		case 2: return rw_launch_tilehist_kv<uint16_t>(keys, n, shift, mask, c, kx, s);
		case 4: return rw_launch_tilehist_kv<uint32_t>(keys, n, shift, mask, c, kx, s);
		default: return CLO_HIP_EUNSUPPORTED;
	}
}

int clo_radixw_launch_tilehist_bytes(const unsigned char* dig, size_t n, int elem_size, int bits, unsigned mask,
	const clo_radix_counters& c, hipStream_t s) {
	const unsigned clear_words = c.partial ? clo_radixw_clear_words(bits, c.tiles) : 0u;
	#define CLO_RW_THB1(B, I, T, W, UA) hipLaunchKernelGGL((clo_radixw_tilehist_bytes_kernel<B, I, T, false, W, UA>), dim3((c.tiles + W - 1u) / W), dim3(T), 0, s, dig, n, c.tiles, mask, c.thist, c.tinfo, c.partial, clear_words)
	#define CLO_RW_THB4(B) CLO_RW_THB1(B, 32, 1024, 2u, false)
	#define CLO_RW_THB(B) case B: \
		if (!c.big) return CLO_HIP_EUNSUPPORTED;    \
		if (elem_size == 8) CLO_RW_THB1(B, 16, 1024, 2u, false); else CLO_RW_THB4(B); \
		break
	if (elem_size != 4 && elem_size != 8) return CLO_HIP_EUNSUPPORTED;
	if ((uintptr_t) dig % 16 != 0) {
		if (bits != 8 || !c.big) return CLO_HIP_EUNSUPPORTED;
		if (elem_size == 8) CLO_RW_THB1(8, 16, 1024, 2u, true); else CLO_RW_THB1(8, 32, 1024, 2u, true);
		return (int) hipGetLastError();
	}
	switch (bits) {
		CLO_RW_THB(1); CLO_RW_THB(2); CLO_RW_THB(3); CLO_RW_THB(4); CLO_RW_THB(5); CLO_RW_THB(6); CLO_RW_THB(7); CLO_RW_THB(8);
		default: return CLO_HIP_EUNSUPPORTED;
	}
	#undef CLO_RW_THB
	#undef CLO_RW_THB4
	#undef CLO_RW_THB1
	return (int) hipGetLastError();
}

unsigned clo_radixw_clear_words(int bits, unsigned tiles) {
	const unsigned chunk = (unsigned) rw_chunk_for(tiles), chunks = (tiles + chunk - 1) / chunk;
	return tiles > 1 ? ((chunks + 1u) << bits) : 0u;
}
size_t clo_radixw_partial_rows(size_t tiles) { const size_t chunk = (size_t) rw_chunk_for((unsigned) (tiles > 0xffffffffull ? 0xffffffffull : tiles)); return (tiles + chunk - 1) / chunk + 2; }

int clo_radixw_launch_offsets(int bits, const clo_radix_counters& c, const unsigned** dbase, hipStream_t s) {
	const unsigned chunk = (unsigned) rw_chunk_for(c.tiles);
	const unsigned chunks = (c.tiles + chunk - 1) / chunk;
	*dbase = nullptr;
	#define CLO_RW_OFF1(B) case B: hipLaunchKernelGGL((clo_radixw_offsets1_kernel<(1 << B)>), dim3(1), dim3(256), 0, s, c.thist, c.tiles, c.toff); break
	if (c.tiles == 1) {
		switch (bits) {
			CLO_RW_OFF1(1); CLO_RW_OFF1(2); CLO_RW_OFF1(3); CLO_RW_OFF1(4); CLO_RW_OFF1(5); CLO_RW_OFF1(6); CLO_RW_OFF1(7); CLO_RW_OFF1(8);
			default: return CLO_HIP_EUNSUPPORTED;
		}
		return (int) hipGetLastError();
	}
	#undef CLO_RW_OFF1
	#define CLO_RW_LB(B) case B: \
		if (chunk == (unsigned) RW_CHUNK) hipLaunchKernelGGL((clo_radixw_offsets_lb_kernel<(1 << B), false, RW_CHUNK>), dim3(chunks), dim3(RW_CS_THREADS), 0, s, c.thist, c.tiles, chunks, c.partial, c.toff); \
		else hipLaunchKernelGGL((clo_radixw_offsets_lb_kernel<(1 << B), false, RW_CHUNK_SMALL>), dim3(chunks), dim3(RW_CS_THREADS), 0, s, c.thist, c.tiles, chunks, c.partial, c.toff); \
		break
	switch (bits) {
		CLO_RW_LB(1); CLO_RW_LB(2); CLO_RW_LB(3); CLO_RW_LB(4); CLO_RW_LB(5); CLO_RW_LB(6); CLO_RW_LB(7); CLO_RW_LB(8);
		default: return CLO_HIP_EUNSUPPORTED;
	}
	#undef CLO_RW_LB
	*dbase = c.partial + ((size_t) (chunks + 1u) << bits);
	return (int) hipGetLastError();
}

int clo_radixw_preload() {
	hipFuncAttributes a;
	return (int) hipFuncGetAttributes(&a, reinterpret_cast<const void*>(&clo_radix_seg_build_kernel));
}

size_t clo_radixw_lds_bytes(int digit_bits) { return 32 * ((size_t) 1 << digit_bits) * sizeof(unsigned); }
```

### cl_ops_amd/csrc/hip/clo_hip_runtime.hip

```cpp
#include <hip/hip_runtime.h>

#include <cstdio>
#include <cstring>
#include <mutex>
#include <string>
#include <vector>

#include "clo_hip.h"
#include "clo_hip_internal.h"

namespace {
struct timing_rec { std::string label; hipEvent_t e0, e1; };
std::mutex g_timing_mu;
std::vector<timing_rec> g_timing;
bool g_timing_on = false;
thread_local clo_hip_launch_observer g_observer = nullptr;
thread_local void* g_observer_user = nullptr;
}

void clo_timing_begin(const char* label, hipStream_t s) {
	if (g_observer) g_observer(g_observer_user, label, 0, (void*) s);
	if (!g_timing_on) return;
	std::lock_guard<std::mutex> lk(g_timing_mu);
	timing_rec r;
	r.label = label;
	if (hipEventCreate(&r.e0) != hipSuccess || hipEventCreate(&r.e1) != hipSuccess) return;
	(void) hipEventRecord(r.e0, s);
	g_timing.push_back(r);
}

void clo_timing_end(hipStream_t s) {
	if (g_timing_on) {
		std::lock_guard<std::mutex> lk(g_timing_mu);
		if (!g_timing.empty()) (void) hipEventRecord(g_timing.back().e1, s);
	}
	if (g_observer) g_observer(g_observer_user, nullptr, 1, (void*) s);
}

extern "C" {

int clo_hip_set_launch_observer(clo_hip_launch_observer fn, void* user) {
	g_observer = fn;
	g_observer_user = fn ? user : nullptr;
	return 0;
}

int clo_hip_timing_enabled(void) { return g_timing_on ? 1 : 0; }

int clo_hip_timing_enable(int on) {
	std::lock_guard<std::mutex> lk(g_timing_mu);
	g_timing_on = on != 0;
	return 0;
}

int clo_hip_timing_reset(void) {
	std::lock_guard<std::mutex> lk(g_timing_mu);
	for (auto& r : g_timing) { (void) hipEventDestroy(r.e0); (void) hipEventDestroy(r.e1); }
	g_timing.clear();
	return 0;
}

int clo_hip_timing_read(const char* label, unsigned* count, float* total_ms) {
	if (!label || !count || !total_ms) return CLO_HIP_EARGS;
	std::lock_guard<std::mutex> lk(g_timing_mu);
	*count = 0;
	*total_ms = 0.f;
	for (auto& r : g_timing) {
		if (r.label != label) continue;
		hipError_t e = hipEventSynchronize(r.e1);
		if (e != hipSuccess) return (int) e;
		float ms = 0.f;
		e = hipEventElapsedTime(&ms, r.e0, r.e1);
		if (e != hipSuccess) return (int) e;
		*total_ms += ms;
		++*count;
	}
	return 0;
}

int clo_hip_device_count(int* count) {
	if (!count) return CLO_HIP_EARGS;
	hipError_t e = hipGetDeviceCount(count);
	if (e != hipSuccess) { *count = 0; }
	return (int) e;
}

int clo_hip_set_device(int device) { return (int) hipSetDevice(device); }
int clo_hip_get_device(int* device) { return device ? (int) hipGetDevice(device) : CLO_HIP_EARGS; }

int clo_hip_get_device_props(int device, clo_hip_device_props* props) {
	if (!props) return CLO_HIP_EARGS;
	hipDeviceProp_t p;
	hipError_t e = hipGetDeviceProperties(&p, device);
	if (e != hipSuccess) return (int) e;
	memset(props, 0, sizeof(*props));
	snprintf(props->name, sizeof(props->name), "%s", p.name);
	snprintf(props->gcn_arch, sizeof(props->gcn_arch), "%s", p.gcnArchName);
	props->compute_units = p.multiProcessorCount;
	props->max_threads_per_block = p.maxThreadsPerBlock;
	props->wavefront_size = p.warpSize;
	props->lds_bytes_per_block = p.sharedMemPerBlock;
	props->global_mem_bytes = p.totalGlobalMem;
	return 0;
}

int clo_hip_stream_create(void** stream) {
	if (!stream) return CLO_HIP_EARGS;
	hipStream_t s;
	hipError_t e = hipStreamCreateWithFlags(&s, hipStreamNonBlocking);
	*stream = (e == hipSuccess) ? (void*) s : nullptr;
	return (int) e;
}
int clo_hip_stream_create_high_priority(void** stream) {
	if (!stream) return CLO_HIP_EARGS;
	int least = 0, greatest = 0;
	hipError_t e = hipDeviceGetStreamPriorityRange(&least, &greatest);
	if (e != hipSuccess) return (int) e;
	hipStream_t s;
	e = hipStreamCreateWithPriority(&s, hipStreamNonBlocking, greatest);
	*stream = (e == hipSuccess) ? (void*) s : nullptr;
	return (int) e;
}
int clo_hip_stream_destroy(void* stream) { return (int) hipStreamDestroy((hipStream_t) stream); }
int clo_hip_stream_synchronize(void* stream) { return (int) hipStreamSynchronize((hipStream_t) stream); }
int clo_hip_stream_query(void* stream) {
	const hipError_t e = hipStreamQuery((hipStream_t) stream);
	if (e == hipErrorNotReady) { (void) hipGetLastError(); return CLO_HIP_ENOTREADY; }
	return (int) e;
}

int clo_hip_malloc(void** dptr, size_t bytes) {
	if (!dptr) return CLO_HIP_EARGS;
	*dptr = nullptr;
	if (bytes == 0) bytes = 4;
	return (int) hipMalloc(dptr, bytes);
}
int clo_hip_free(void* dptr) { return dptr ? (int) hipFree(dptr) : 0; }

int clo_hip_memcpy_h2d_async(void* dst, const void* src, size_t bytes, void* stream) {
	return (int) hipMemcpyAsync(dst, src, bytes, hipMemcpyHostToDevice, (hipStream_t) stream);
}
int clo_hip_memcpy_d2h_async(void* dst, const void* src, size_t bytes, void* stream) {
	return (int) hipMemcpyAsync(dst, src, bytes, hipMemcpyDeviceToHost, (hipStream_t) stream);
}
int clo_hip_memcpy_d2d_async(void* dst, const void* src, size_t bytes, void* stream) {
	return (int) hipMemcpyAsync(dst, src, bytes, hipMemcpyDeviceToDevice, (hipStream_t) stream);
}
int clo_hip_memset_async(void* dst, int value, size_t bytes, void* stream) {
	return (int) hipMemsetAsync(dst, value, bytes, (hipStream_t) stream);
}

int clo_hip_host_register(void* host_ptr, size_t bytes) {
	if (!host_ptr || bytes == 0) return CLO_HIP_EARGS;
	return (int) hipHostRegister(host_ptr, bytes, hipHostRegisterDefault);
}
int clo_hip_host_unregister(void* host_ptr) { return host_ptr ? (int) hipHostUnregister(host_ptr) : 0; }

int clo_hip_event_create(void** event) {
	if (!event) return CLO_HIP_EARGS;
	hipEvent_t ev;
	hipError_t e = hipEventCreate(&ev);
	*event = (e == hipSuccess) ? (void*) ev : nullptr;
	return (int) e;
}
int clo_hip_event_destroy(void* event) { return event ? (int) hipEventDestroy((hipEvent_t) event) : 0; }
int clo_hip_event_record(void* event, void* stream) {
	return (int) hipEventRecord((hipEvent_t) event, (hipStream_t) stream);
}
static clo_hip_env_t g_env = { CLO_MAX_SPINS, 2, 0, 0, 1 };
static int g_env_read = 0;
void clo_hip_env_refresh(void) {
	clo_hip_env_t e = { CLO_MAX_SPINS, 2, 0, 0, 1 };
	if (const char* m = getenv("CLO_MAX_SPINS")) e.max_spins = (unsigned) strtoul(m, nullptr, 10);
	if (const char* m = getenv("CLO_RADIX_SWEEP")) e.radix_sweep = atoi(m) != 0 ? 1 : 0;
	if (const char* m = getenv("CLO_R1_POOLS")) e.r1_pools = atoi(m);
	e.no_digits = getenv("CLO_RADIX_NO_DIGITS") != nullptr;
	if (const char* m = getenv("CLO_BITONIC_MERGE2")) e.bitonic_merge2 = atoi(m);
	__atomic_store_n(&g_env.max_spins, e.max_spins, __ATOMIC_RELAXED);
	__atomic_store_n(&g_env.radix_sweep, e.radix_sweep, __ATOMIC_RELAXED);
	__atomic_store_n(&g_env.r1_pools, e.r1_pools, __ATOMIC_RELAXED);
	__atomic_store_n(&g_env.no_digits, e.no_digits, __ATOMIC_RELAXED);
	__atomic_store_n(&g_env.bitonic_merge2, e.bitonic_merge2, __ATOMIC_RELAXED);
	__atomic_store_n(&g_env_read, 1, __ATOMIC_RELEASE);
}
int clo_hip_event_synchronize(void* event) { return (int) hipEventSynchronize((hipEvent_t) event); }
int clo_hip_event_query(void* event) { return event ? (int) hipEventQuery((hipEvent_t) event) : CLO_HIP_EARGS; }
int clo_hip_event_elapsed_ms(void* start, void* stop, float* ms) {
	return ms ? (int) hipEventElapsedTime(ms, (hipEvent_t) start, (hipEvent_t) stop) : CLO_HIP_EARGS;
}
int clo_hip_stream_wait_event(void* stream, void* event) {
	return (int) hipStreamWaitEvent((hipStream_t) stream, (hipEvent_t) event, 0);
}

int clo_hip_graph_capture_begin(void* stream) {
	return (int) hipStreamBeginCapture((hipStream_t) stream, hipStreamCaptureModeThreadLocal);
}

int clo_hip_stream_is_capturing(void* stream) {
	hipStreamCaptureStatus st = hipStreamCaptureStatusNone;
	if (hipStreamIsCapturing((hipStream_t) stream, &st) != hipSuccess) { (void) hipGetLastError(); return 1; }
	return st != hipStreamCaptureStatusNone ? 1 : 0;
}

int clo_hip_graph_capture_end(void* stream, void** graph_exec) {
	if (!graph_exec) return CLO_HIP_EARGS;
	*graph_exec = nullptr;
	hipGraph_t graph = nullptr;
	hipError_t e = hipStreamEndCapture((hipStream_t) stream, &graph);
	if (e != hipSuccess) return (int) e;
	hipGraphExec_t exec = nullptr;
	e = hipGraphInstantiate(&exec, graph, nullptr, nullptr, 0);
	(void) hipGraphDestroy(graph);
	if (e != hipSuccess) return (int) e;
	*graph_exec = exec;
	return 0;
}

int clo_hip_graph_launch(void* graph_exec, void* stream) {
	return graph_exec ? (int) hipGraphLaunch((hipGraphExec_t) graph_exec, (hipStream_t) stream) : CLO_HIP_EARGS;
}

int clo_hip_graph_destroy(void* graph_exec) {
	return graph_exec ? (int) hipGraphExecDestroy((hipGraphExec_t) graph_exec) : 0;
}

const char* clo_hip_error_string(int status) {
	switch (status) {
		case 0: return "success";
		case CLO_HIP_EARGS: return "clo_hip: invalid arguments";
		case CLO_HIP_EUNSUPPORTED: return "clo_hip: unsupported type or option";
		case CLO_HIP_EWORKSPACE: return "clo_hip: workspace too small";
		case CLO_HIP_ETIMEOUT: return "clo_hip: in-kernel look-back spin timed out";
		case CLO_HIP_ENOTREADY: return "clo_hip: work on the stream is still running";
		default:
			if (status <= CLO_HIP_ERCCL) return "clo_hip: RCCL reported an error (status = CLO_HIP_ERCCL - ncclResult_t)";
			return status > 0 ? hipGetErrorString((hipError_t) status) : "clo_hip: unknown error";
	}
}

int clo_hip_check_status(void* workspace, void* stream) {
	if (!workspace) return CLO_HIP_EARGS;
	unsigned int word = 0;
	hipError_t e = hipMemcpyAsync(&word, (char*) workspace + CLO_WS_STATUS_OFFSET, sizeof(word),
		hipMemcpyDeviceToHost, (hipStream_t) stream);
	if (e != hipSuccess) return (int) e;
	e = hipStreamSynchronize((hipStream_t) stream);
	if (e != hipSuccess) return (int) e;
	return word ? CLO_HIP_ETIMEOUT : 0;
}

}

const clo_hip_env_t* clo_hip_env() {
	if (!g_env_read) clo_hip_env_refresh();
	return &g_env;
}
```

### include/clo_hip.h

```cpp
#ifndef CLO_HIP_H
#define CLO_HIP_H

#include <stddef.h>
#include <stdint.h>

#ifdef __cplusplus
extern "C" {
#endif

#define CLO_HIP_EARGS      (-1)
#define CLO_HIP_EUNSUPPORTED (-2)
#define CLO_HIP_EWORKSPACE (-3)
#define CLO_HIP_ETIMEOUT   (-4)
#define CLO_HIP_ENOTREADY  (-5)
#define CLO_HIP_ERCCL      (-100)

#define CLO_HIP_WORKSPACE_ALIGN 256


typedef struct {
	char name[128];
	int compute_units;
	int max_threads_per_block;
	int wavefront_size;
	size_t lds_bytes_per_block;
	size_t global_mem_bytes;
	char gcn_arch[64];
} clo_hip_device_props;

int clo_hip_device_count(int* count);
int clo_hip_set_device(int device);
int clo_hip_get_device(int* device);
int clo_hip_get_device_props(int device, clo_hip_device_props* props);

int clo_hip_stream_create(void** stream);
int clo_hip_stream_create_high_priority(void** stream);
int clo_hip_stream_destroy(void* stream);
int clo_hip_stream_synchronize(void* stream);
int clo_hip_stream_query(void* stream);

int clo_hip_malloc(void** dptr, size_t bytes);
int clo_hip_free(void* dptr);
int clo_hip_memcpy_h2d_async(void* dst, const void* src, size_t bytes, void* stream);
int clo_hip_memcpy_d2h_async(void* dst, const void* src, size_t bytes, void* stream);
int clo_hip_memcpy_d2d_async(void* dst, const void* src, size_t bytes, void* stream);
int clo_hip_memset_async(void* dst, int value, size_t bytes, void* stream);
int clo_hip_host_register(void* host_ptr, size_t bytes);
int clo_hip_host_unregister(void* host_ptr);

void clo_hip_env_refresh(void);
int clo_hip_event_create(void** event);
int clo_hip_event_destroy(void* event);
int clo_hip_event_record(void* event, void* stream);
int clo_hip_event_synchronize(void* event);
int clo_hip_event_query(void* event);
int clo_hip_event_elapsed_ms(void* start, void* stop, float* ms);
int clo_hip_stream_wait_event(void* stream, void* event);

int clo_hip_stream_is_capturing(void* stream);
int clo_hip_graph_capture_begin(void* stream);
int clo_hip_graph_capture_end(void* stream, void** graph_exec);
int clo_hip_graph_launch(void* graph_exec, void* stream);
int clo_hip_graph_destroy(void* graph_exec);

const char* clo_hip_error_string(int status);

size_t clo_hip_scan_workspace_bytes(size_t numel, int elem_size, int sum_size);
int clo_hip_scan_workspace_init(void* workspace, size_t workspace_bytes, void* stream);
int clo_hip_scan_workspace_forget(void* workspace);
int clo_hip_scan_workspace_set_epoch(void* workspace, unsigned epoch, void* stream);
int clo_hip_scan_exclusive(const void* data_in, void* data_out, size_t numel,
	int elem_size, int elem_signed, int sum_size,
	void* workspace, size_t workspace_bytes, void* stream);
int clo_hip_scan_exclusive_carry(const void* data_in, void* data_out, size_t numel,
	int elem_size, int elem_signed, int sum_size,
	const uint64_t* carry_in_dev, uint64_t* carry_out_dev,
	void* workspace, size_t workspace_bytes, void* stream);
int clo_hip_scan_is_typed(int elem_type, int sum_type);
size_t clo_hip_scan_typed_workspace_bytes(size_t numel, int sum_type);
int clo_hip_scan_exclusive_typed(const void* data_in, void* data_out, size_t numel, int elem_type, int sum_type,
	void* workspace, size_t workspace_bytes, void* stream);
size_t clo_hip_scan_fp_workspace_bytes(size_t numel, int sum_size);
int clo_hip_scan_exclusive_fp(const void* data_in, void* data_out, size_t numel, int elem_type, int sum_size,
	void* workspace, size_t workspace_bytes, void* stream);
int clo_hip_reduce_sum(const void* data_in, size_t numel, int elem_size, int elem_signed,
	uint64_t* total_dev, void* stream);

size_t clo_hip_reduce_by_key_tile(int key_size, int value_size);
size_t clo_hip_reduce_by_key_workspace_bytes(size_t numel);
int clo_hip_reduce_by_key(const void* keys_in, const void* values_in, void* keys_out, void* aggr_out, uint64_t* num_runs_dev,
	size_t numel, int key_size, int value_type, int sum_type, int op,
	void* workspace, size_t workspace_bytes, void* stream);

size_t clo_hip_scan_by_key_tile(int key_size, int value_size);
size_t clo_hip_scan_by_key_workspace_bytes(size_t numel);
int clo_hip_scan_by_key(const void* keys_in, const void* values_in, void* out, size_t numel,
	int key_size, int value_type, int sum_type, int op, int inclusive,
	void* workspace, size_t workspace_bytes, void* stream);

size_t clo_hip_histogram_tile(int key_size, int value_size);
size_t clo_hip_histogram_lds_bins(int sum_size);
size_t clo_hip_histogram_workspace_bytes(size_t numel, size_t num_bins);
int clo_hip_histogram(const void* keys_in, const void* values_in, void* hist_out, size_t numel, int key_size, int key_signed,
	int value_type, int sum_type, uint64_t lower, unsigned shift, size_t num_bins, int accumulate, unsigned max_groups,
	void* workspace, size_t workspace_bytes, void* stream);

size_t clo_hip_merge_tile(int key_size, int value_size);
size_t clo_hip_merge_workspace_bytes(size_t numel_a, size_t numel_b);
int clo_hip_merge(const void* keys_a, const void* values_a, size_t numel_a,
	const void* keys_b, const void* values_b, size_t numel_b,
	void* keys_out, void* values_out, int key_size, int key_kind,
	int value_size, void* workspace, size_t workspace_bytes, void* stream);

#define CLO_HIP_SEARCH_UPPER          1u
#define CLO_HIP_SEARCH_NEEDLES_SORTED 2u
size_t clo_hip_search_tile(int key_size);
size_t clo_hip_search_lds_keys(int key_size);
size_t clo_hip_search_pivots(int key_size);
size_t clo_hip_search_workspace_bytes(size_t numel_h, size_t numel_n, unsigned flags);
int clo_hip_search(const void* haystack, size_t numel_h, const void* needles, size_t numel_n, void* pos_out,
	int key_size, int key_kind, unsigned flags, unsigned max_groups,
	void* workspace, size_t workspace_bytes, void* stream);

#define CLO_HIP_SETOP_UNION                0
#define CLO_HIP_SETOP_INTERSECTION         1
#define CLO_HIP_SETOP_DIFFERENCE           2
#define CLO_HIP_SETOP_SYMMETRIC_DIFFERENCE 3
size_t clo_hip_setop_tile(int key_size, int value_size);
size_t clo_hip_setop_workspace_bytes(size_t numel_a, size_t numel_b);
int clo_hip_setop(int op, const void* keys_a, const void* values_a, size_t numel_a,
	const void* keys_b, const void* values_b, size_t numel_b,
	void* keys_out, void* values_out, uint64_t* num_out, int key_size, int key_kind,
	int value_size, void* workspace, size_t workspace_bytes, void* stream);

#define CLO_HIP_JOIN_INNER 0
#define CLO_HIP_JOIN_LEFT  1
#define CLO_HIP_JOIN_RIGHT 2
#define CLO_HIP_JOIN_FULL  3
#define CLO_HIP_JOIN_NONE  0xFFFFFFFFu
size_t clo_hip_join_tile(int key_size);
size_t clo_hip_join_out_tile(void);
size_t clo_hip_join_workspace_bytes(int kind, size_t numel_a, size_t numel_b);
int clo_hip_join(int kind, const void* keys_a, size_t numel_a, const void* keys_b, size_t numel_b,
	uint32_t* idx_a_out, uint32_t* idx_b_out, void* keys_out, size_t capacity,
	uint64_t* num_out, int key_size, int key_kind,
	void* workspace, size_t workspace_bytes, void* stream);

#define CLO_HIP_SELECT_SELECT    0
#define CLO_HIP_SELECT_PARTITION 1
#define CLO_HIP_SELECT_FLAGGED 0
#define CLO_HIP_SELECT_LT      1
#define CLO_HIP_SELECT_LE      2
#define CLO_HIP_SELECT_GT      3
#define CLO_HIP_SELECT_GE      4
#define CLO_HIP_SELECT_EQ      5
#define CLO_HIP_SELECT_NE      6
#define CLO_HIP_SELECT_SCAN_TRIP 2048
size_t clo_hip_select_tile(int key_size, int value_size);
size_t clo_hip_select_workspace_bytes(size_t numel, int key_size, int value_size);
int clo_hip_select(int op, int pred, const void* keys_in, const void* values_in, const void* flags_or_threshold,
	void* keys_out, void* values_out, uint64_t* num_out, size_t numel, int key_size, int key_kind,
	int value_size, void* workspace, size_t workspace_bytes, void* stream);

#define CLO_HIP_BUCKET_MAX_BINS 65535
#define CLO_HIP_BUCKET_SCAN_GROUP 4096
#define CLO_HIP_BUCKET_SCAN_TRIP 2048
size_t clo_hip_bucket_tile(int key_size, int value_size);
size_t clo_hip_bucket_workspace_bytes(size_t numel, int key_size, int value_size, size_t num_bins);
int clo_hip_bucket(const void* keys_in, const void* values_in, void* keys_out, void* values_out, void* offsets_out, size_t numel,
	int key_size, int key_signed, int value_size, int count_size, uint64_t lower, unsigned shift, size_t num_bins,
	void* workspace, size_t workspace_bytes, void* stream);

#define CLO_HIP_TOPK_SMALLEST 0
#define CLO_HIP_TOPK_LARGEST  1
#define CLO_HIP_TOPK_INPUT  0
#define CLO_HIP_TOPK_SORTED 1
#define CLO_HIP_TOPK_SCAN_TRIP 2048
size_t clo_hip_topk_tile(int key_size, int value_size);
size_t clo_hip_topk_sweep_groups(void);
size_t clo_hip_topk_sorted_max(int key_size, int value_size);
size_t clo_hip_topk_workspace_bytes(size_t numel, int key_size, int value_size);
int clo_hip_topk(int which, int order, const void* keys_in, const void* values_in, void* keys_out, void* values_out, void* kth_out,
	size_t numel, size_t k, int key_size, int key_kind, int value_size, void* workspace, size_t workspace_bytes, void* stream);

#define CLO_HIP_EXPAND_COUNTS 0
#define CLO_HIP_EXPAND_OFFSETS 1
size_t clo_hip_expand_tile(int value_size);
size_t clo_hip_expand_lds_segments(void);
size_t clo_hip_expand_workspace_bytes(size_t numel_in, size_t capacity);
int clo_hip_expand(int form, const void* counts_or_offsets, int count_size, const uint64_t* num_in, const void* values_in,
	void* values_out, void* seg_out, void* rank_out, uint64_t* num_out, size_t numel_in, size_t capacity, int value_size,
	void* workspace, size_t workspace_bytes, void* stream);

#define CLO_HIP_SEGREDUCE_COUNTS 0
#define CLO_HIP_SEGREDUCE_OFFSETS 1
size_t clo_hip_segreduce_tile(int value_size, int sum_size);
size_t clo_hip_segreduce_workspace_bytes(size_t numel_seg, size_t numel);
int clo_hip_segreduce(int op, int form, const void* counts_or_offsets, int count_size, const uint64_t* num_in, const void* values_in,
	void* aggr_out, uint64_t* num_out, size_t numel_seg, size_t numel, int value_type, int sum_type,
	void* workspace, size_t workspace_bytes, void* stream);

#define CLO_HIP_SEGSORT_COUNTS 0
#define CLO_HIP_SEGSORT_OFFSETS 1
size_t clo_hip_segsort_tile(int key_size, int value_size);
size_t clo_hip_segsort_workspace_bytes(size_t numel_seg, size_t numel, int key_size, int value_size);
int clo_hip_segsort(int form, const void* counts_or_offsets, int count_size, const uint64_t* num_in, const void* keys_in, const void* values_in,
	void* keys_out, void* values_out, uint64_t* num_out, size_t numel_seg, size_t numel, int key_type, int value_size,
	void* workspace, size_t workspace_bytes, void* stream);

#define CLO_HIP_SEGSCAN_COUNTS 0
#define CLO_HIP_SEGSCAN_OFFSETS 1
size_t clo_hip_segscan_tile(int value_size, int sum_size);
size_t clo_hip_segscan_workspace_bytes(size_t numel_seg, size_t numel);
int clo_hip_segscan(int op, int inclusive, int form, const void* counts_or_offsets, int count_size, const uint64_t* num_in, const void* values_in,
	void* data_out, uint64_t* num_out, size_t numel_seg, size_t numel, int value_type, int sum_type,
	void* workspace, size_t workspace_bytes, void* stream);

#define CLO_HIP_SEGARG_ARGMIN 0
#define CLO_HIP_SEGARG_ARGMAX 1
#define CLO_HIP_SEGARG_FIRST 0
#define CLO_HIP_SEGARG_LAST 1
#define CLO_HIP_SEGARG_COUNTS 0
#define CLO_HIP_SEGARG_OFFSETS 1
size_t clo_hip_segarg_tile(int value_size);
size_t clo_hip_segarg_carry_tiles(void);
size_t clo_hip_segarg_workspace_bytes(size_t numel_seg, size_t numel);
int clo_hip_segarg(int op, int tie, int form, const void* counts_or_offsets, int count_size, const uint64_t* num_in, const void* values_in,
	uint32_t* idx_out, void* val_out, uint64_t* num_out, size_t numel_seg, size_t numel, int value_type,
	void* workspace, size_t workspace_bytes, void* stream);

#define CLO_HIP_SEGTOPK_SMALLEST 0
#define CLO_HIP_SEGTOPK_LARGEST 1
#define CLO_HIP_SEGTOPK_COUNTS 0
#define CLO_HIP_SEGTOPK_OFFSETS 1
size_t clo_hip_segtopk_tile(int key_size, int value_size);
size_t clo_hip_segtopk_k_max(int key_size, int value_size);
size_t clo_hip_segtopk_workspace_bytes(size_t numel_seg, size_t numel, size_t k, int key_size, int value_size);
int clo_hip_segtopk(int which, int form, const void* counts_or_offsets, int count_size, const uint64_t* num_in, const void* keys_in, const void* values_in,
	void* keys_out, void* values_out, uint32_t* counts_out, uint64_t* num_out, size_t numel_seg, size_t numel, size_t k, int key_type, int value_size,
	void* workspace, size_t workspace_bytes, void* stream);

#define CLO_HIP_SEGFSUM_COUNTS 0
#define CLO_HIP_SEGFSUM_OFFSETS 1
size_t clo_hip_segfsum_tile(int value_size, int sum_size);
size_t clo_hip_segfsum_workspace_bytes(size_t numel_seg, size_t numel);
int clo_hip_segfsum(int form, const void* counts_or_offsets, int count_size, const uint64_t* num_in, const void* values_in,
	void* sums_out, uint64_t* num_out, size_t numel_seg, size_t numel, int value_type, int sum_type,
	void* workspace, size_t workspace_bytes, void* stream);

int clo_hip_radix_preload(void);
size_t clo_hip_radix_workspace_bytes(size_t numel, int elem_size, int key_bits, int digit_bits);
int clo_hip_radix_polls(size_t numel, int elem_size, int digit_bits);
int clo_hip_radix_sort(const void* src, void* dst, void* tmp, size_t numel,
	int elem_size, int key_shift, int key_bits, int key_kind, int digit_bits,
	void* workspace, size_t workspace_bytes, void* stream);
int clo_hip_radix_takes_first_digits(size_t numel, int elem_size, int key_kind, int digit_bits);
int clo_hip_radix_sort_fed(const void* src, void* dst, void* tmp, size_t numel,
	int elem_size, int key_shift, int key_bits, int key_kind, int digit_bits, const unsigned char* first_digits,
	void* workspace, size_t workspace_bytes, void* stream);
size_t clo_hip_radix_kv_workspace_bytes(size_t numel, int key_size, int key_bits, int digit_bits);
int clo_hip_radix_sort_kv(const void* keys_in, const void* values_in, void* keys_out, void* values_out, void* pairs_a, void* pairs_b,
	size_t numel, int key_size, int key_shift, int key_bits, int key_kind, int digit_bits,
	void* workspace, size_t workspace_bytes, void* stream);
int clo_hip_radix_debug_stamps(void* buffer, size_t tiles);

size_t clo_hip_radix_seg_workspace_bytes(size_t numel, int nseg, int elem_size, int digit_bits);
int clo_hip_radix_sort_segmented(const void* src, void* a, void* b, size_t numel, const size_t* seg_counts, int nseg,
	const size_t* piece_counts, const size_t* piece_offsets, const int* piece_segment, int npieces,
	int elem_size, int key_shift, int key_bits, int digit_bits, void* workspace, size_t workspace_bytes, void* stream,
	int* result_in_b);
int clo_hip_radix_sort_segmented2(const void* src, const void* src2, void* a, void* b, size_t numel, const size_t* seg_counts, int nseg,
	const size_t* piece_counts, const size_t* piece_offsets, const int* piece_segment, const int* piece_source, int npieces,
	int elem_size, int key_shift, int key_bits, int digit_bits, void* workspace, size_t workspace_bytes, void* stream,
	int* result_in_b);

int clo_hip_msd_histogram(const void* src, size_t numel, int elem_size,
	int key_shift, int key_bits, int bucket_bits,
	uint64_t* counts_dev, void* stream);
int clo_hip_msd_partition(const void* src, void* dst, size_t numel, int elem_size,
	int key_shift, int key_bits, int bucket_bits, uint64_t* counts_dev,
	void* workspace, size_t workspace_bytes, void* stream);
size_t clo_hip_msd_workspace_bytes(size_t numel, int elem_size, int bucket_bits);

#define CLO_HIP_RCCL_ID_BYTES 128
int clo_hip_rccl_unique_id(void* id_out);
int clo_hip_rccl_comm_create(void** comm, const void* id_in, int rank, int world);
int clo_hip_rccl_comm_destroy(void* comm);
int clo_hip_rccl_comm_abort(void* comm);
int clo_hip_rccl_comm_async_error(void* comm);
int clo_hip_rccl_all_gather_u64(void* comm, const uint64_t* send_dev, uint64_t* recv_dev, size_t count, void* stream);
int clo_hip_rccl_all_to_all_v(void* comm, int rank, int world,
	const void* send_dev, const size_t* send_bytes, const size_t* send_offset_bytes,
	void* recv_dev, const size_t* recv_bytes, const size_t* recv_offset_bytes, void* stream);

size_t clo_hip_bitonic_padded_numel(size_t numel);
int clo_hip_bitonic_simple(void* data, size_t numel, int elem_size,
	int key_shift, int key_bits, int key_size, int key_kind, int descending,
	int* launches, void* stream);
int clo_hip_bitonic_any(void* data, size_t numel, int elem_size,
	int key_shift, int key_bits, int key_size, int key_kind, int descending, int* launches, void* stream);
int clo_hip_bitonic_tiled(void* data, size_t numel, int elem_size,
	int key_shift, int key_bits, int key_size, int key_kind, int descending,
	int* launches, void* stream);

int clo_hip_gselect(const void* src, void* dst, size_t numel, int elem_size,
	int key_shift, int key_bits, int key_size, int key_kind, int descending, void* stream);

int clo_hip_bitonic_jit_create(int elem_type, int key_type, const char* compare, const char* get_key, const char* compiler_opts,
	void** handle, char** log);
void clo_hip_bitonic_jit_destroy(void* handle);
int clo_hip_bitonic_jit_gselect(void* handle, const void* src, void* dst, size_t numel, void* stream);
int clo_hip_bitonic_jit_sort(void* handle, void* data, size_t numel, int tiled, int* launches, void* stream);
size_t clo_hip_bitonic_jit_lds_bytes(void* handle, size_t numel, int tiled);

int clo_hip_radix_jit_create(int elem_type, int key_type, const char* get_key, const char* compiler_opts, void** handle, char** log);
void clo_hip_radix_jit_destroy(void* handle);
int clo_hip_radix_jit_sort(void* handle, const void* src, void* dst, void* pairs, void* pairs_tmp, size_t numel,
	int digit_bits, void* workspace, size_t workspace_bytes, void* stream);

int clo_hip_check_status(void* workspace, void* stream);

typedef void (*clo_hip_launch_observer)(void* user, const char* label, int phase, void* stream);
int clo_hip_set_launch_observer(clo_hip_launch_observer fn, void* user);

int clo_hip_timing_enable(int on);
int clo_hip_timing_enabled(void);
int clo_hip_timing_reset(void);
int clo_hip_timing_read(const char* label, unsigned* count, float* total_ms);

size_t clo_hip_kernel_lds_bytes(const char* family, int elem_size, int param);
size_t clo_hip_bitonic_lds_bytes(size_t numel, int elem_size, int tiled);

const char* clo_hip_rng_device_source(void);
int clo_hip_rng_init(int gen, void* states, size_t count, uint64_t main_seed, int hash, void* stream);
int clo_hip_rng_init_jit(int gen, const char* hash, void* states, size_t count, uint64_t main_seed, void* stream, char** log);
int clo_hip_rng_fill(int gen, void* states, size_t count, unsigned* out, size_t numel, unsigned bits, unsigned maxint,
	int layout, void* stream);

#ifdef __cplusplus
}
#endif
#endif
```

Baseline: 116,400.

## Compute per-tile radix offsets in chunked histogram kernel, single-block chunk scan

Result: slower. 113,700 (-2.3%).

```diff
diff --git a/cl_ops_amd/_hip.py b/cl_ops_amd/_hip.py
--- a/cl_ops_amd/_hip.py
+++ b/cl_ops_amd/_hip.py
@@ -77,6 +77,7 @@
 _sig("clo_hip_reduce_sum", ci, vp, sz, ci, ci, vp, vp)
 _sig("clo_hip_radix_workspace_bytes", sz, sz, ci, ci, ci)
 _sig("clo_hip_radix_polls", ci, sz, ci, ci)
+_sig("clo_hip_radix_chunk_plan", None, sz, C.POINTER(C.c_uint), C.POINTER(C.c_uint))
 _sig("clo_hip_radix_sort", ci, vp, vp, vp, sz, ci, ci, ci, ci, ci, vp, sz, vp)
 _sig("clo_hip_radix_takes_first_digits", ci, sz, ci, ci, ci)
 _sig("clo_hip_radix_sort_fed", ci, vp, vp, vp, sz, ci, ci, ci, ci, ci, vp, vp, sz, vp)
diff --git a/cl_ops_amd/csrc/hip/clo_hip_internal.h b/cl_ops_amd/csrc/hip/clo_hip_internal.h
--- a/cl_ops_amd/csrc/hip/clo_hip_internal.h
+++ b/cl_ops_amd/csrc/hip/clo_hip_internal.h
@@ -13,7 +13,7 @@
 #define CLO_WS_MAX_PASSES    64
 #define CLO_WS_HEADER_BYTES  512
 
-struct clo_hip_env_t { unsigned max_spins; int radix_sweep; int r1_pools; int no_digits; int bitonic_merge2; };
+struct clo_hip_env_t { unsigned max_spins; int radix_sweep; int r1_pools; int no_digits; int bitonic_merge2; int chunk_tiles; };
 const clo_hip_env_t* clo_hip_env();
 int clo_radixw_preload();
 
@@ -83,15 +83,16 @@
 int clo_bitonic_tiled_e4(void* data, size_t numel, int key_shift, int key_bits, int key_size, int key_kind, int descending, int* launches, hipStream_t s);
 int clo_bitonic_tiled_e8(void* data, size_t numel, int key_shift, int key_bits, int key_size, int key_kind, int descending, int* launches, hipStream_t s);
 size_t clo_radixw_lds_bytes(int digit_bits);
-struct clo_radix_counters { unsigned* thist; unsigned* toff; unsigned* partial; unsigned* tinfo; unsigned tiles; bool big; };
+struct clo_radix_counters { unsigned* thist; unsigned* toff; unsigned* partial; unsigned* tinfo; unsigned tiles; bool big; unsigned* delta; unsigned* csum; };
+void clo_radixw_chunk_plan(size_t tiles, unsigned* ch, unsigned* chunks);
+size_t clo_radixw_csum_rows(size_t tiles);
 int clo_radixw_launch_tilehist(const void* in, size_t n, int elem_size, int bits, unsigned shift, unsigned mask,
 	const clo_radix_counters& c, clo_keyx kx, hipStream_t s);
 int clo_radixw_launch_tilehist_kv(const void* keys, size_t n, int key_size, int bits, unsigned shift, unsigned mask,
 	const clo_radix_counters& c, clo_keyx kx, hipStream_t s);
 int clo_radixw_launch_tilehist_bytes(const unsigned char* dig, size_t n, int elem_size, int bits, unsigned mask,
 	const clo_radix_counters& c, hipStream_t s);
-int clo_radixw_launch_offsets(int bits, const clo_radix_counters& c, const unsigned** dbase, hipStream_t s);
-size_t clo_radixw_partial_rows(size_t tiles);
+int clo_radixw_launch_offsets(int bits, const clo_radix_counters& c, hipStream_t s);
 
 #define CLO_SEG_MAX 256
 struct clo_seg_tile { unsigned in_base, count_seg, out_base, seg_n; };
diff --git a/cl_ops_amd/csrc/hip/clo_hip_radix.hip b/cl_ops_amd/csrc/hip/clo_hip_radix.hip
--- a/cl_ops_amd/csrc/hip/clo_hip_radix.hip
+++ b/cl_ops_amd/csrc/hip/clo_hip_radix.hip
@@ -55,6 +55,8 @@
 int clo_hip_radix_polls(size_t numel, int elem_size, int digit_bits) {
 	return clo_radix1_applies(numel, elem_size, digit_bits) ? 1 : 0;
 }
+
+void clo_hip_radix_chunk_plan(size_t tiles, unsigned* chunk_tiles, unsigned* chunks) { clo_radixw_chunk_plan(tiles, chunk_tiles, chunks); }
 
 int clo_hip_radix_takes_first_digits(size_t numel, int elem_size, int key_kind, int digit_bits) {
 	return key_kind == 0 ? clo_radix4_takes_first_digits(numel, elem_size, digit_bits) : 0;
diff --git a/cl_ops_amd/csrc/hip/clo_hip_radix4.hip b/cl_ops_amd/csrc/hip/clo_hip_radix4.hip
--- a/cl_ops_amd/csrc/hip/clo_hip_radix4.hip
+++ b/cl_ops_amd/csrc/hip/clo_hip_radix4.hip
@@ -52,7 +52,7 @@
 	unsigned shift, unsigned mask_lo, unsigned mask_hi,
 	const unsigned* __restrict__ thist, const unsigned* __restrict__ toff, const unsigned* __restrict__ dbase,
 	const unsigned* __restrict__ tinfo, int aligned,
-	clo_keyx kx_in, clo_keyx kx_out, unsigned char* __restrict__ dig_out = nullptr, unsigned next_shift = 0,
+	clo_keyx kx_in, clo_keyx kx_out, unsigned ch, unsigned char* __restrict__ dig_out = nullptr, unsigned next_shift = 0,
 	const clo_seg_tile* __restrict__ tdesc = nullptr, const E* __restrict__ in2 = nullptr, clo_kv_io kv = clo_kv_io()) {
 	static_assert((KV_IN == 0 && KV_OUT == 0) || (sizeof(E) == 8 && !SEG), "key-value passes: 8-byte pairs, one array");
 
@@ -70,7 +70,7 @@
 	__shared__ unsigned s_wtot[WAVES][HMAX];
 	__shared__ __attribute__((aligned(16))) unsigned s_wbase[WAVES][HMAX];
 	__shared__ unsigned s_delta[R2];
-	__shared__ unsigned s_w4[4];
+	__shared__ unsigned s_w4[SEG ? 4 : 1];
 
 	const unsigned tid = threadIdx.x, lane = tid & 63u, wave = tid >> 6;
 	const unsigned per_xcd = SEG ? (unsigned) ((n + 7) / 8) : (unsigned) ((n + (size_t) TILE * 8 - 1) / ((size_t) TILE * 8));
@@ -99,9 +99,13 @@
 	__builtin_amdgcn_s_setprio(3);
 	unsigned h2 = 0, goff = 0;
 	if (tid < (unsigned) R2) {
-		h2 = thist[(size_t) tile * R2 + tid];
 		goff = toff[(size_t) tile * R2 + tid];
-		if (dbase) goff += dbase[tid];
+		if constexpr (SEG) {
+			h2 = thist[(size_t) tile * R2 + tid];
+			goff += dbase[tid];
+		} else {
+			goff += dbase[(size_t) (tile / ch) * R2 + tid];
+		}
 	}
 	E key[ITEMS];
 	if constexpr (KV_IN != 0) {
@@ -118,7 +122,9 @@
 		#pragma unroll
 		for (int i = 0; i < ITEMS; ++i) key[i] = clo_keyx_fwd<E>(key[i], kx_in);
 	}
-	{
+	if constexpr (!SEG) {
+		if (tid < (unsigned) R2) s_delta[tid] = goff;
+	} else {
 		const unsigned incl2 = clo_wave_scan_inclusive<unsigned>(h2, lane);
 		if (lane == 63 && wave < 4) s_w4[wave] = incl2;
 		if (tid < (unsigned) R2) s_delta[tid] = goff - (incl2 - h2);
@@ -143,10 +149,10 @@
 			#pragma unroll
 			for (int i = 0; i < ITEMS; ++i) if (tbase + i < count) s_stage[tbase + i] = key[i];
 		}
-		clo_lds_barrier();
-	}
-
-	if (tid < (unsigned) R2) {
+		if constexpr (SEG) clo_lds_barrier();
+	}
+
+	if (SEG && tid < (unsigned) R2) {
 		unsigned before = 0;
 		#pragma unroll
 		for (unsigned w = 0; w < 4; ++w) if (w < wave) before += s_w4[w];
@@ -281,7 +287,7 @@
 }
 
 
-struct rp_layout { size_t thist, toff, partial, tinfo, dig, total, tiles; bool big; };
+struct rp_layout { size_t delta, csum, tinfo, dig, total, tiles; bool big; };
 
 rp_layout rp_make_layout(size_t n, int elem_size, int pass_bits, bool digits = true) {
 	rp_layout L;
@@ -291,10 +297,9 @@
 	L.tiles = (n + tile - 1) / tile;
 	if (L.tiles == 0) L.tiles = 1;
 	const size_t per = L.tiles * R2 * sizeof(unsigned);
-	L.thist = CLO_WS_HEADER_BYTES;
-	L.toff = L.thist + per;
-	L.partial = L.toff + per;
-	L.tinfo = L.partial + ((clo_radixw_partial_rows(L.tiles) * R2 * sizeof(unsigned) + 255) & ~(size_t) 255);
+	L.delta = CLO_WS_HEADER_BYTES;
+	L.csum = L.delta + per;
+	L.tinfo = L.csum + ((clo_radixw_csum_rows(L.tiles) * R2 * sizeof(unsigned) + 255) & ~(size_t) 255);
 	L.total = L.tinfo + ((L.tiles * sizeof(unsigned) + 255) & ~(size_t) 255);
 	L.dig = 0;
 	if (digits && clo_radix_digit_stream(n, elem_size)) {
@@ -304,10 +309,14 @@
 	return L;
 }
 
+clo_radix_counters rp_counters(void* ws, const rp_layout& L) {
+	char* w = (char*) ws;
+	return { nullptr, nullptr, nullptr, (unsigned*) (w + L.tinfo), (unsigned) L.tiles, L.big, (unsigned*) (w + L.delta), (unsigned*) (w + L.csum) };
+}
 template <typename Layout>
-clo_radix_counters rp_counters(void* ws, const Layout& L, size_t tiles) {
+clo_radix_counters rp_seg_counters(void* ws, const Layout& L) {
 	char* w = (char*) ws;
-	return { (unsigned*) (w + L.thist), (unsigned*) (w + L.toff), (unsigned*) (w + L.partial), (unsigned*) (w + L.tinfo), (unsigned) tiles, L.big };
+	return { (unsigned*) (w + L.thist), (unsigned*) (w + L.toff), (unsigned*) (w + L.partial), (unsigned*) (w + L.tinfo), 0u, L.big, nullptr, nullptr };
 }
 
 struct rp_digits { unsigned shift, mask_lo, mask_hi, mask, next_shift; };
@@ -332,11 +341,13 @@
 	clo_keyx kx_in, clo_keyx kx_out, unsigned char* dig_out, hipStream_t s, const clo_seg_tile* tdesc = nullptr, const E* in2 = nullptr,
 	bool kv_in = false, bool kv_out = false, const clo_kv_io& kv = clo_kv_io()) {
 	const unsigned tiles = SEG ? (unsigned) n : c.tiles;
+	unsigned ch = 1u, chunks = 0u;
+	if (!SEG) clo_radixw_chunk_plan(c.tiles, &ch, &chunks);
 	const auto launch = [&](auto big, auto dig, auto kvi, auto kvo) {
 		constexpr bool BIG = decltype(big)::value, DIG = decltype(dig)::value;
 		hipLaunchKernelGGL((clo_radix4_pair_kernel<E, LB, HB, BIG, DIG, SEG, decltype(kvi)::value, decltype(kvo)::value>),
 			dim3((tiles + 7u) / 8u * 8u), dim3(pair_shape<E, BIG>::THREADS), 0, s,
-			in, out, n, d.shift, d.mask_lo, d.mask_hi, c.thist, c.toff, dbase, c.tinfo, aligned, kx_in, kx_out, dig_out, d.next_shift, tdesc, in2, kv);
+			in, out, n, d.shift, d.mask_lo, d.mask_hi, c.thist, SEG ? c.toff : c.delta, SEG ? dbase : c.csum, c.tinfo, aligned, kx_in, kx_out, ch, dig_out, d.next_shift, tdesc, in2, kv);
 	};
 	const auto shape = [&](auto kvi, auto kvo) {
 		constexpr bool BIG_OK = sizeof(E) >= 4, DIG_OK = BIG_OK && LB == 4 && HB == 4 && decltype(kvo)::value == 0;
@@ -364,7 +375,7 @@
 	constexpr int PB = LB + HB;
 	const int passes = (key_bits + PB - 1) / PB;
 	const rp_layout L = rp_make_layout(n, (int) sizeof(E), PB);
-	const clo_radix_counters c = rp_counters(ws, L, L.tiles);
+	const clo_radix_counters c = rp_counters(ws, L);
 	const bool no_dig = clo_hip_env()->no_digits != 0;
 	constexpr bool DIG_OK = LB == 4 && HB == 4 && sizeof(E) >= 4;
 	unsigned char* dig = (DIG_OK && L.dig != 0 && passes > 1 && !no_dig) ? (unsigned char*) ws + L.dig : nullptr;
@@ -390,16 +401,15 @@
 				: clo_radixw_launch_tilehist(cur_in, n, (int) sizeof(E), PB, d.shift, d.mask, c, p == 0 ? kx : kx_none, s);
 			if (st != 0) return st;
 		}
-		const unsigned* dbase = nullptr;
 		{
 			clo_timing_scope timing("radix_offsets", s);
-			const int st = clo_radixw_launch_offsets(PB, c, &dbase, s);
+			const int st = clo_radixw_launch_offsets(PB, c, s);
 			if (st != 0) return st;
 		}
 		{
 			clo_timing_scope timing("radix_pass", s);
 			const int aligned = kv_in ? (int) kv_aligned : (int) ((uintptr_t) cur_in % 16 == 0);
-			rp_launch_pass<E, LB, HB, false, KB>(c, d, cur_in, cur_out, n, dbase, aligned, p == 0 ? kx : kx_none, p + 1 == passes ? kx : kx_none,
+			rp_launch_pass<E, LB, HB, false, KB>(c, d, cur_in, cur_out, n, nullptr, aligned, p == 0 ? kx : kx_none, p + 1 == passes ? kx : kx_none,
 				p + 1 < passes ? dig : nullptr, s, nullptr, nullptr, kv_in, kv_out, kv);
 		}
 		cur_in = cur_out;
@@ -436,24 +446,6 @@
 
 template <int R, int R2>
 __global__ __launch_bounds__(256)
-void clo_radix4_counts_kernel(const unsigned* __restrict__ thist, unsigned tiles, unsigned long long* __restrict__ counts) {
-	constexpr int G = 256 / R;
-	__shared__ unsigned long long s_part[G][R];
-	const unsigned tid = threadIdx.x, d = tid % R, g = tid / R;
-	unsigned long long c = 0;
-	for (unsigned t = g; t < tiles; t += G) c += thist[(size_t) t * R2 + d];
-	s_part[g][d] = c;
-	__syncthreads();
-	if (tid < (unsigned) R) {
-		unsigned long long tot = 0;
-		#pragma unroll
-		for (int k = 0; k < G; ++k) tot += s_part[k][tid];
-		counts[tid] = tot;
-	}
-}
-
-template <int R, int R2>
-__global__ __launch_bounds__(256)
 void clo_radix4_counts_from_bases_kernel(const unsigned* __restrict__ dbase, unsigned n, unsigned long long* __restrict__ counts) {
 	const unsigned d = threadIdx.x;
 	if (d < (unsigned) R) counts[d] = (unsigned long long) ((d + 1u < (unsigned) R2 ? dbase[d + 1u] : n) - dbase[d]);
@@ -466,7 +458,7 @@
 	constexpr bool TWO = BITS > 3;
 	static_assert(TWO ? PB == BITS : (LB == BITS && HB == BITS), "see above");
 	const rp_layout L = rp_make_layout(n, (int) sizeof(E), PB, false);
-	const clo_radix_counters c = rp_counters(ws, L, L.tiles);
+	const clo_radix_counters c = rp_counters(ws, L);
 	const clo_keyx kx_none = { 0, 0, 0 };
 	hipError_t e = hipMemsetAsync(ws, 0, CLO_WS_HEADER_BYTES, s);
 	if (e != hipSuccess) return (int) e;
@@ -474,14 +466,10 @@
 	const rp_digits d = rp_pass_digits<LB, HB>(0, (int) shift, BITS);
 	int st = clo_radixw_launch_tilehist(src, n, (int) sizeof(E), PB, d.shift, d.mask, c, kx_none, s);
 	if (st != 0) return st;
-	const unsigned* dbase = nullptr;
-	st = clo_radixw_launch_offsets(PB, c, &dbase, s);
+	st = clo_radixw_launch_offsets(PB, c, s);
 	if (st != 0) return st;
-	if (counts) {
-		if (dbase) hipLaunchKernelGGL((clo_radix4_counts_from_bases_kernel<R, (1 << PB)>), dim3(1), dim3(256), 0, s, dbase, (unsigned) n, counts);
-		else hipLaunchKernelGGL((clo_radix4_counts_kernel<R, (1 << PB)>), dim3(1), dim3(256), 0, s, c.thist, c.tiles, counts);
-	}
-	rp_launch_pass<E, LB, HB>(c, d, src, dst, n, dbase, (int) ((uintptr_t) src % 16 == 0), kx_none, kx_none, nullptr, s);
+	if (counts) hipLaunchKernelGGL((clo_radix4_counts_from_bases_kernel<R, (1 << PB)>), dim3(1), dim3(256), 0, s, c.csum, (unsigned) n, counts);
+	rp_launch_pass<E, LB, HB>(c, d, src, dst, n, nullptr, (int) ((uintptr_t) src % 16 == 0), kx_none, kx_none, nullptr, s);
 	return (int) hipGetLastError();
 }
 
@@ -517,7 +505,7 @@
 	constexpr int LB = 4, HB = 4, PB = 8;
 	const int passes = (key_bits + PB - 1) / PB;
 	const rp_seg_layout L = rp_make_seg_layout(n, nseg, (int) sizeof(E));
-	const clo_radix_counters c = rp_counters(ws, L, 0);
+	const clo_radix_counters c = rp_seg_counters(ws, L);
 	const auto up = [](size_t x) { return (x + 255) & ~(size_t) 255; };
 	size_t seg_base[CLO_SEG_MAX];
 	int seg_id[CLO_SEG_MAX];
diff --git a/cl_ops_amd/csrc/hip/clo_hip_radixw.hip b/cl_ops_amd/csrc/hip/clo_hip_radixw.hip
--- a/cl_ops_amd/csrc/hip/clo_hip_radixw.hip
+++ b/cl_ops_amd/csrc/hip/clo_hip_radixw.hip
@@ -202,10 +202,245 @@
 	}
 }
 
+template <int R, int TPW> struct rw_emit_lds { unsigned h[TPW][R]; unsigned w[TPW][4]; };
+
+template <int R, int TPW, int TILE>
+__device__ __forceinline__ void rw_chunk_emit(unsigned* __restrict__ s_cnt, rw_emit_lds<R, TPW>& s, unsigned tid, unsigned t_first, unsigned tend,
+	size_t n, unsigned& running, unsigned* __restrict__ delta, unsigned* __restrict__ tinfo) {
+	static_assert(TPW == 1 || R == 256, "several tiles per group: whole waves per row of counters");
+	constexpr int COPIES = 32;
+	typedef unsigned vec4u __attribute__((ext_vector_type(4)));
+	const bool mine = tid < (unsigned) (TPW * R);
+	const unsigned part = tid / R, d = tid % R, lane = tid & 63u, pwave = d >> 6;
+	unsigned h = 0;
+	if (mine) {
+		vec4u* row = reinterpret_cast<vec4u*>(&s_cnt[part * (R * COPIES) + d * COPIES]);
+		const vec4u z = { 0u, 0u, 0u, 0u };
+		#pragma unroll
+		for (int k = 0; k < COPIES / 4; ++k) {
+			const unsigned at = (unsigned) (k + d) & (COPIES / 4 - 1);
+			const vec4u x = row[at];
+			row[at] = z;
+			h += x[0] + x[1] + x[2] + x[3];
+		}
+		if constexpr (TPW > 1) s.h[part][d] = h;
+	}
+	const unsigned incl = clo_wave_scan_inclusive<unsigned>(h, lane);
+	if (mine && lane == 63u) s.w[part][pwave] = incl;
+	clo_lds_barrier();
+	if (mine) {
+		unsigned start = incl - h;
+		#pragma unroll
+		for (unsigned w = 0; w < 4; ++w) if (w < pwave) start += s.w[part][w];
+		unsigned before = 0, tot = h;
+		if constexpr (TPW > 1) {
+			tot = 0;
+			#pragma unroll
+			for (int p = 0; p < TPW; ++p) {
+				const unsigned x = s.h[p][d];
+				if ((unsigned) p < part) before += x;
+				tot += x;
+			}
+		}
+		const unsigned t = t_first + part;
+		if (t < tend) {
+			const size_t tb = (size_t) t * TILE;
+			const unsigned tcount = (n - tb) < (size_t) TILE ? (unsigned) (n - tb) : (unsigned) TILE;
+			delta[(size_t) t * R + d] = running + before - start;
+			rw_tile_info(h, tcount, tinfo, t);
+		}
+		running += tot;
+	}
+}
+
+template <typename E, int BITS, bool BIG, typename L = E>
+__global__ __launch_bounds__((rw_shape<E, BIG>::THREADS))
+void clo_radixw_tilehist_chunk_kernel(const L* __restrict__ in, size_t n, unsigned tiles, unsigned ch, unsigned shift, unsigned mask,
+	unsigned* __restrict__ delta, unsigned* __restrict__ tinfo, unsigned* __restrict__ csum, int aligned, clo_keyx kx) {
+	static_assert(std::is_same<L, E>::value || (sizeof(E) == 8 && sizeof(L) <= 4), "keys of a key-value sort: 8-byte pairs");
+	const auto widen = [](L x) -> E {
+		if constexpr (std::is_same<L, E>::value) return x;
+		else return (E) x << 32;
+	};
+	constexpr int R = 1 << BITS;
+	constexpr int TILE = rw_shape<E, BIG>::TILE;
+	constexpr int RW_THREADS = rw_shape<E, BIG>::THREADS;
+	constexpr int ITEMS = TILE / RW_THREADS;
+	constexpr int VB = ITEMS * (int) sizeof(L) >= 16 ? 16 : ITEMS * (int) sizeof(L);
+	constexpr int VECS = ITEMS * (int) sizeof(L) / VB;
+	constexpr int PER = VB / (int) sizeof(L);
+	constexpr bool STREAM = rw_shape<E, BIG>::STREAM;
+	constexpr int COPIES = 32;
+	__shared__ __attribute__((aligned(16))) unsigned s_cnt[R * COPIES];
+	__shared__ rw_emit_lds<R, 1> s_emit;
+	const unsigned tid = threadIdx.x, lane = tid & 63u;
+	const unsigned t0 = blockIdx.x * ch, tend = t0 + ch < tiles ? t0 + ch : tiles;
+	unsigned* const cnt = s_cnt + (lane & (COPIES - 1));
+	typedef L vecE __attribute__((ext_vector_type(PER)));
+	const auto is_whole = [&](unsigned t) { return aligned != 0 && t < tend && ((size_t) t + 1) * TILE <= n; };
+	const auto request = [&](unsigned t, vecE (&v)[VECS]) {
+		const vecE* p = reinterpret_cast<const vecE*>(in + (size_t) t * TILE) + tid;
+		#pragma unroll
+		for (int k = 0; k < VECS; ++k) v[k] = STREAM ? __builtin_nontemporal_load(p + k * RW_THREADS) : p[k * RW_THREADS];
+	};
+	vecE va[VECS], vb[VECS];
+	if (is_whole(t0)) request(t0, va);
+	{
+		typedef unsigned vec4u __attribute__((ext_vector_type(4)));
+		const vec4u z = { 0u, 0u, 0u, 0u };
+		for (unsigned i = tid; i < (unsigned) (R * COPIES / 4); i += RW_THREADS) reinterpret_cast<vec4u*>(s_cnt)[i] = z;
+	}
+	clo_lds_barrier();
+	unsigned running = 0;
+	const auto round = [&](unsigned t, vecE (&v)[VECS], vecE (&vnext)[VECS]) {
+		if (is_whole(t + 1u)) request(t + 1u, vnext);
+		if (is_whole(t)) {
+			#pragma unroll
+			for (int k = 0; k < VECS; ++k) {
+				#pragma unroll
+				for (int q = 0; q < PER; ++q)
+					atomicAdd(&cnt[((unsigned) (clo_keyx_fwd<E>(widen(v[k][q]), kx) >> shift) & mask) << 5], 1u);
+			}
+		} else {
+			const size_t base = (size_t) t * TILE;
+			const unsigned count = (n - base) < (size_t) TILE ? (unsigned) (n - base) : (unsigned) TILE, tbase = tid * ITEMS;
+			#pragma unroll
+			for (int i = 0; i < ITEMS; ++i)
+				if (tbase + i < count)
+					atomicAdd(&cnt[((unsigned) (clo_keyx_fwd<E>(widen(in[base + tbase + i]), kx) >> shift) & mask) << 5], 1u);
+		}
+		clo_lds_barrier();
+		rw_chunk_emit<R, 1, TILE>(s_cnt, s_emit, tid, t, tend, n, running, delta, tinfo);
+	};
+	for (unsigned t = t0; t < tend; t += 2u) {
+		round(t, va, vb);
+		if (t + 1u < tend) round(t + 1u, vb, va);
+	}
+	if (tid < (unsigned) R) csum[(size_t) blockIdx.x * R + tid] = running;
+}
+
+template <int BITS, int ITEMS, int THREADS, int TPW, bool UA>
+__global__ __launch_bounds__(THREADS)
+void clo_radixw_tilehist_chunk_bytes_kernel(const unsigned char* __restrict__ dig, size_t n, unsigned tiles, unsigned ch, unsigned mask,
+	unsigned* __restrict__ delta, unsigned* __restrict__ tinfo, unsigned* __restrict__ csum) {
+	constexpr int R = 1 << BITS;
+	constexpr int PART = THREADS / TPW;
+	constexpr int TILE = PART * ITEMS;
+	constexpr int COPIES = 32;
+	constexpr bool STREAM = ITEMS == 32;
+	static_assert(PART % 64 == 0 && PART * TPW == THREADS && ITEMS % 16 == 0, "whole waves per tile, whole 16-byte vectors per thread");
+	__shared__ __attribute__((aligned(16))) unsigned s_cnt[TPW * R * COPIES];
+	__shared__ rw_emit_lds<R, TPW> s_emit;
+	const unsigned tid = threadIdx.x, lane = tid & 63u;
+	const unsigned part = tid / PART, ptid = tid % PART;
+	const unsigned t0 = blockIdx.x * ch, tend = t0 + ch < tiles ? t0 + ch : tiles;
+	unsigned* const cnt = s_cnt + part * (R * COPIES) + (lane & (COPIES - 1));
+	typedef unsigned q4A __attribute__((ext_vector_type(4)));
+	typedef unsigned q4U __attribute__((ext_vector_type(4), aligned(1)));
+	typedef typename std::conditional<UA, q4U, q4A>::type q4;
+	constexpr int VECS = ITEMS / 16;
+	const auto is_whole = [&](unsigned t) { return t < tend && ((size_t) t + 1) * TILE <= n; };
+	const auto request = [&](unsigned t, q4 (&v)[VECS]) {
+		const q4* p = reinterpret_cast<const q4*>(dig + (size_t) t * TILE) + ptid;
+		#pragma unroll
+		for (int k = 0; k < VECS; ++k) v[k] = STREAM ? __builtin_nontemporal_load(p + k * PART) : p[k * PART];
+	};
+	q4 va[VECS], vb[VECS];
+	if (is_whole(t0 + part)) request(t0 + part, va);
+	{
+		const q4A z = { 0u, 0u, 0u, 0u };
+		for (unsigned i = tid; i < (unsigned) (TPW * R * COPIES / 4); i += THREADS) reinterpret_cast<q4A*>(s_cnt)[i] = z;
+	}
+	clo_lds_barrier();
+	unsigned running = 0;
+	const auto round = [&](unsigned tf, q4 (&v)[VECS], q4 (&vnext)[VECS]) {
+		const unsigned t = tf + part;
+		if (is_whole(t + TPW)) request(t + TPW, vnext);
+		if (is_whole(t)) {
+			#pragma unroll
+			for (int k = 0; k < VECS; ++k) {
+				#pragma unroll
+				for (int q = 0; q < 4; ++q) {
+					#pragma unroll
+					for (int b = 0; b < 4; ++b)
+						atomicAdd(&cnt[(((unsigned) v[k][q] >> (8 * b)) & mask) << 5], 1u);
+				}
+			}
+		} else if (t < tend) {
+			const size_t base = (size_t) t * TILE;
+			const unsigned count = (n - base) < (size_t) TILE ? (unsigned) (n - base) : (unsigned) TILE, tbase = ptid * ITEMS;
+			#pragma unroll
+			for (int i = 0; i < ITEMS; ++i)
+				if (tbase + i < count) atomicAdd(&cnt[((unsigned) dig[base + tbase + i] & mask) << 5], 1u);
+		}
+		clo_lds_barrier();
+		rw_chunk_emit<R, TPW, TILE>(s_cnt, s_emit, tid, tf, tend, n, running, delta, tinfo);
+	};
+	for (unsigned tf = t0; tf < tend; tf += 2u * TPW) {
+		round(tf, va, vb);
+		if (tf + TPW < tend) round(tf + TPW, vb, va);
+	}
+	if (tid < (unsigned) R) csum[(size_t) blockIdx.x * R + tid] = running;
+}
+
+constexpr int RW_SCAN_THREADS = 1024;
+template <int R>
+__global__ __launch_bounds__(RW_SCAN_THREADS)
+void clo_radixw_chunkscan_kernel(unsigned* __restrict__ csum, unsigned chunks) {
+	static_assert(R % 4 == 0 && R <= 256, "four digits per thread");
+	constexpr int LPR = R / 4, G = 16, B = 8;
+	typedef unsigned vec4u __attribute__((ext_vector_type(4)));
+	__shared__ __attribute__((aligned(16))) unsigned s_p[G][R];
+	__shared__ __attribute__((aligned(16))) unsigned s_base[R];
+	__shared__ unsigned s_w[4];
+	const unsigned tid = threadIdx.x, g = tid / LPR, l = tid % LPR, lane = tid & 63u, wave = tid >> 6;
+	const bool active = g < (unsigned) G;
+	const unsigned per = (chunks + G - 1) / G;
+	const unsigned c0 = g * per < chunks ? g * per : chunks, c1 = c0 + per < chunks ? c0 + per : chunks;
+	vec4u* const rows = reinterpret_cast<vec4u*>(csum) + l;
+	if (active) {
+		vec4u own = { 0u, 0u, 0u, 0u };
+		for (unsigned c = c0; c < c1; c += B) {
+			vec4u x[B];
+			#pragma unroll
+			for (int k = 0; k < B; ++k) x[k] = c + k < c1 ? rows[(size_t) (c + k) * LPR] : vec4u{ 0u, 0u, 0u, 0u };
+			#pragma unroll
+			for (int k = 0; k < B; ++k) own += x[k];
+		}
+		reinterpret_cast<vec4u*>(s_p[g])[l] = own;
+	}
+	__syncthreads();
+	unsigned tot = 0;
+	if (tid < (unsigned) R) {
+		#pragma unroll
+		for (int k = 0; k < G; ++k) tot += s_p[k][tid];
+	}
+	const unsigned incl = clo_wave_scan_inclusive<unsigned>(tot, lane);
+	if (lane == 63u && wave < 4u) s_w[wave] = incl;
+	__syncthreads();
+	if (tid < (unsigned) R) {
+		unsigned dbase = incl - tot;
+		#pragma unroll
+		for (unsigned w = 0; w < 4; ++w) if (w < wave) dbase += s_w[w];
+		s_base[tid] = dbase;
+	}
+	__syncthreads();
+	if (!active) return;
+	vec4u run = reinterpret_cast<const vec4u*>(s_base)[l];
+	for (unsigned k = 0; k < g; ++k) run += reinterpret_cast<const vec4u*>(s_p[k])[l];
+	for (unsigned c = c0; c < c1; c += B) {
+		vec4u x[B];
+		#pragma unroll
+		for (int k = 0; k < B; ++k) x[k] = c + k < c1 ? rows[(size_t) (c + k) * LPR] : vec4u{ 0u, 0u, 0u, 0u };
+		#pragma unroll
+		for (int k = 0; k < B; ++k) {
+			if (c + k < c1) rows[(size_t) (c + k) * LPR] = run;
+			run += x[k];
+		}
+	}
+}
+
 constexpr int RW_CS_THREADS = 1024;
-constexpr int RW_CHUNK_SMALL = 32;
-constexpr unsigned RW_SMALL_TILES = 2048;
-constexpr int rw_chunk_for(unsigned tiles) { return tiles <= RW_SMALL_TILES ? RW_CHUNK_SMALL : RW_CHUNK; }
 template <int R, int CHUNK = RW_CHUNK> struct rw_cs {
 	static constexpr int G = (RW_CS_THREADS / R) < CHUNK ? (RW_CS_THREADS / R) : CHUNK;
 	static constexpr int SUB = CHUNK / G;
@@ -298,47 +533,6 @@
 		const unsigned t = t0 + g * SUB + k;
 		if (t < tend) toff[(size_t) t * R + d] = run;
 		run += v[k];
-	}
-}
-
-template <int R>
-__global__ __launch_bounds__(256)
-void clo_radixw_offsets1_kernel(const unsigned* __restrict__ thist, unsigned tiles, unsigned* __restrict__ toff) {
-	constexpr int G = 256 / R;
-	constexpr int SUB = RW_CHUNK / G;
-	__shared__ unsigned s_a[G][R], s_base[R], s_w[4];
-	const unsigned tid = threadIdx.x, d = tid % R, g = tid / R, lane = tid & 63u, wave = tid >> 6;
-	const unsigned ts = g * SUB < tiles ? g * SUB : tiles;
-	const unsigned te = ts + SUB < tiles ? ts + SUB : tiles;
-	unsigned own = 0;
-	#pragma unroll 8
-	for (unsigned t = ts; t < te; ++t) own += thist[(size_t) t * R + d];
-	s_a[g][d] = own;
-	__syncthreads();
-	unsigned before = 0, tot = 0;
-	#pragma unroll
-	for (int k = 0; k < G; ++k) {
-		const unsigned v = s_a[k][d];
-		if ((unsigned) k < g) before += v;
-		tot += v;
-	}
-	const unsigned t0 = tid < (unsigned) R ? tot : 0u;
-	const unsigned incl = clo_wave_scan_inclusive<unsigned>(t0, lane);
-	if (lane == 63) s_w[wave] = incl;
-	__syncthreads();
-	if (tid < (unsigned) R) {
-		unsigned dbase = incl - t0;
-		#pragma unroll
-		for (unsigned w = 0; w < 4; ++w) if (w < wave) dbase += s_w[w];
-		s_base[tid] = dbase;
-	}
-	__syncthreads();
-	unsigned run = s_base[d] + before;
-	#pragma unroll 8
-	for (unsigned t = ts; t < te; ++t) {
-		const unsigned c = thist[(size_t) t * R + d];
-		toff[(size_t) t * R + d] = run;
-		run += c;
 	}
 }
 
@@ -480,116 +674,92 @@
 }
 
 
-unsigned clo_radixw_clear_words(int bits, unsigned tiles);
-
-template <typename E>
-static int rw_launch_tilehist(const void* in, size_t n, int bits, unsigned shift, unsigned mask, const clo_radix_counters& c, clo_keyx kx,
-	hipStream_t s) {
+#ifndef CLO_RW_CHUNKS_MAX
+#define CLO_RW_CHUNKS_MAX 512
+#endif
+constexpr unsigned RW_CHUNKS_MAX = CLO_RW_CHUNKS_MAX;
+void clo_radixw_chunk_plan(size_t tiles, unsigned* ch, unsigned* chunks) {
+	const int least = clo_hip_env()->chunk_tiles;
+	size_t c = least >= 32 ? 32 : 1;
+	while ((int) c < least) c *= 2;
+	while (c < 32 && (tiles + c - 1) / c > RW_CHUNKS_MAX) c *= 2;
+	if ((tiles + c - 1) / c > RW_CHUNKS_MAX) {
+		c = (tiles + RW_CHUNKS_MAX - 1) / RW_CHUNKS_MAX;
+		c += c & 1;
+	}
+	*ch = (unsigned) c;
+	*chunks = (unsigned) ((tiles + c - 1) / c);
+}
+size_t clo_radixw_csum_rows(size_t tiles) { return tiles < RW_CHUNKS_MAX ? tiles : RW_CHUNKS_MAX; }
+
+template <typename E, typename L>
+static int rw_launch_chunkhist(const L* in, size_t n, int bits, unsigned shift, unsigned mask, const clo_radix_counters& c, clo_keyx kx, hipStream_t s) {
 	const int aligned = (int) ((uintptr_t) in % 16 == 0);
-	const unsigned clear_words = c.partial ? clo_radixw_clear_words(bits, c.tiles) : 0u;
-	#define CLO_RW_TH(B) case B: \
-		if (c.big && sizeof(E) >= 4) hipLaunchKernelGGL((clo_radixw_tilehist_kernel<E, B, (sizeof(E) >= 4)>), dim3(c.tiles), dim3(rw_shape<E, (sizeof(E) >= 4)>::THREADS), 0, s, \
-			(const E*) in, n, shift, mask, c.thist, c.tinfo, aligned, kx, c.partial, clear_words); \
-		else hipLaunchKernelGGL((clo_radixw_tilehist_kernel<E, B, false>), dim3(c.tiles), dim3(rw_shape<E, false>::THREADS), 0, s, \
-			(const E*) in, n, shift, mask, c.thist, c.tinfo, aligned, kx, c.partial, clear_words); \
+	unsigned ch, chunks;
+	clo_radixw_chunk_plan(c.tiles, &ch, &chunks);
+	constexpr bool BIG_OK = sizeof(E) >= 4;
+	#define CLO_RW_CH(B) case B: \
+		if (c.big && BIG_OK) hipLaunchKernelGGL((clo_radixw_tilehist_chunk_kernel<E, B, BIG_OK, L>), dim3(chunks), dim3(rw_shape<E, BIG_OK>::THREADS), 0, s, \
+			in, n, c.tiles, ch, shift, mask, c.delta, c.tinfo, c.csum, aligned, kx); \
+		else hipLaunchKernelGGL((clo_radixw_tilehist_chunk_kernel<E, B, false, L>), dim3(chunks), dim3(rw_shape<E, false>::THREADS), 0, s, \
+			in, n, c.tiles, ch, shift, mask, c.delta, c.tinfo, c.csum, aligned, kx); \
 		break
-	switch (bits) {
-		CLO_RW_TH(1); CLO_RW_TH(2); CLO_RW_TH(3); CLO_RW_TH(4); CLO_RW_TH(5); CLO_RW_TH(6); CLO_RW_TH(7); CLO_RW_TH(8);
-		default: return CLO_HIP_EUNSUPPORTED;
-	}
-	#undef CLO_RW_TH
+	if constexpr (!std::is_same<E, L>::value) {
+		switch (bits) { CLO_RW_CH(8); default: return CLO_HIP_EUNSUPPORTED; }
+	} else {
+		switch (bits) {
+			CLO_RW_CH(2); CLO_RW_CH(3); CLO_RW_CH(4); CLO_RW_CH(5); CLO_RW_CH(6); CLO_RW_CH(7); CLO_RW_CH(8);
+			default: return CLO_HIP_EUNSUPPORTED;
+		}
+	}
+	#undef CLO_RW_CH
 	return (int) hipGetLastError();
 }
 
 int clo_radixw_launch_tilehist(const void* in, size_t n, int elem_size, int bits, unsigned shift, unsigned mask,
 	const clo_radix_counters& c, clo_keyx kx, hipStream_t s) {
 	switch (elem_size) {
-		case 1: return rw_launch_tilehist<uint8_t>(in, n, bits, shift, mask, c, kx, s);
-		case 2: return rw_launch_tilehist<uint16_t>(in, n, bits, shift, mask, c, kx, s);
-		case 4: return rw_launch_tilehist<uint32_t>(in, n, bits, shift, mask, c, kx, s);
-		case 8: return rw_launch_tilehist<uint64_t>(in, n, bits, shift, mask, c, kx, s);
+		case 1: return rw_launch_chunkhist<uint8_t>((const uint8_t*) in, n, bits, shift, mask, c, kx, s);
+		case 2: return rw_launch_chunkhist<uint16_t>((const uint16_t*) in, n, bits, shift, mask, c, kx, s);
+		case 4: return rw_launch_chunkhist<uint32_t>((const uint32_t*) in, n, bits, shift, mask, c, kx, s);
+		case 8: return rw_launch_chunkhist<uint64_t>((const uint64_t*) in, n, bits, shift, mask, c, kx, s);
 		default: return CLO_HIP_EUNSUPPORTED;
 	}
-}
-
-template <typename K>
-static int rw_launch_tilehist_kv(const void* keys, size_t n, unsigned shift, unsigned mask, const clo_radix_counters& c, clo_keyx kx, hipStream_t s) {
-	const int aligned = (int) ((uintptr_t) keys % 16 == 0);
-	const unsigned clear_words = c.partial ? clo_radixw_clear_words(8, c.tiles) : 0u;
-	if (c.big)
-		hipLaunchKernelGGL((clo_radixw_tilehist_kernel<uint64_t, 8, true, false, 1, K>), dim3(c.tiles), dim3(rw_shape<uint64_t, true>::THREADS), 0, s,
-			(const K*) keys, n, shift, mask, c.thist, c.tinfo, aligned, kx, c.partial, clear_words, nullptr, nullptr);
-	else
-		hipLaunchKernelGGL((clo_radixw_tilehist_kernel<uint64_t, 8, false, false, 1, K>), dim3(c.tiles), dim3(rw_shape<uint64_t, false>::THREADS), 0, s,
-			(const K*) keys, n, shift, mask, c.thist, c.tinfo, aligned, kx, c.partial, clear_words, nullptr, nullptr);
-	return (int) hipGetLastError();
 }
 
 int clo_radixw_launch_tilehist_kv(const void* keys, size_t n, int key_size, int bits, unsigned shift, unsigned mask,
 	const clo_radix_counters& c, clo_keyx kx, hipStream_t s) {
 	if (bits != 8) return CLO_HIP_EUNSUPPORTED;
 	switch (key_size) {
-		case 1: return rw_launch_tilehist_kv<uint8_t>(keys, n, shift, mask, c, kx, s);
-		case 2: return rw_launch_tilehist_kv<uint16_t>(keys, n, shift, mask, c, kx, s);
-		case 4: return rw_launch_tilehist_kv<uint32_t>(keys, n, shift, mask, c, kx, s);
+		case 1: return rw_launch_chunkhist<uint64_t>((const uint8_t*) keys, n, bits, shift, mask, c, kx, s);
+		case 2: return rw_launch_chunkhist<uint64_t>((const uint16_t*) keys, n, bits, shift, mask, c, kx, s);
+		case 4: return rw_launch_chunkhist<uint64_t>((const uint32_t*) keys, n, bits, shift, mask, c, kx, s);
 		default: return CLO_HIP_EUNSUPPORTED;
 	}
 }
 
 int clo_radixw_launch_tilehist_bytes(const unsigned char* dig, size_t n, int elem_size, int bits, unsigned mask,
 	const clo_radix_counters& c, hipStream_t s) {
-	const unsigned clear_words = c.partial ? clo_radixw_clear_words(bits, c.tiles) : 0u;
-	#define CLO_RW_THB1(B, I, T, W, UA) hipLaunchKernelGGL((clo_radixw_tilehist_bytes_kernel<B, I, T, false, W, UA>), dim3((c.tiles + W - 1u) / W), dim3(T), 0, s, dig, n, c.tiles, mask, c.thist, c.tinfo, c.partial, clear_words)
-	#define CLO_RW_THB4(B) CLO_RW_THB1(B, 32, 1024, 2u, false)
-	#define CLO_RW_THB(B) case B: \
-		if (!c.big) return CLO_HIP_EUNSUPPORTED;    \
-		if (elem_size == 8) CLO_RW_THB1(B, 16, 1024, 2u, false); else CLO_RW_THB4(B); \
-		break
-	if (elem_size != 4 && elem_size != 8) return CLO_HIP_EUNSUPPORTED;
-	if ((uintptr_t) dig % 16 != 0) {
-		if (bits != 8 || !c.big) return CLO_HIP_EUNSUPPORTED;
-		if (elem_size == 8) CLO_RW_THB1(8, 16, 1024, 2u, true); else CLO_RW_THB1(8, 32, 1024, 2u, true);
-		return (int) hipGetLastError();
-	}
+	if ((elem_size != 4 && elem_size != 8) || bits != 8 || !c.big) return CLO_HIP_EUNSUPPORTED;
+	unsigned ch, chunks;
+	clo_radixw_chunk_plan(c.tiles, &ch, &chunks);
+	#define CLO_RW_CHB(I, UA) hipLaunchKernelGGL((clo_radixw_tilehist_chunk_bytes_kernel<8, I, 1024, 2, UA>), dim3(chunks), dim3(1024), 0, s, \
+		dig, n, c.tiles, ch, mask, c.delta, c.tinfo, c.csum)
+	if ((uintptr_t) dig % 16 != 0) { if (elem_size == 8) CLO_RW_CHB(16, true); else CLO_RW_CHB(32, true); }
+	else { if (elem_size == 8) CLO_RW_CHB(16, false); else CLO_RW_CHB(32, false); }
+	#undef CLO_RW_CHB
+	return (int) hipGetLastError();
+}
+
+int clo_radixw_launch_offsets(int bits, const clo_radix_counters& c, hipStream_t s) {
+	unsigned ch, chunks;
+	clo_radixw_chunk_plan(c.tiles, &ch, &chunks);
+	#define CLO_RW_SC(B) case B: hipLaunchKernelGGL((clo_radixw_chunkscan_kernel<(1 << B)>), dim3(1), dim3(RW_SCAN_THREADS), 0, s, c.csum, chunks); break
 	switch (bits) {
-		CLO_RW_THB(1); CLO_RW_THB(2); CLO_RW_THB(3); CLO_RW_THB(4); CLO_RW_THB(5); CLO_RW_THB(6); CLO_RW_THB(7); CLO_RW_THB(8);
+		CLO_RW_SC(2); CLO_RW_SC(3); CLO_RW_SC(4); CLO_RW_SC(5); CLO_RW_SC(6); CLO_RW_SC(7); CLO_RW_SC(8);
 		default: return CLO_HIP_EUNSUPPORTED;
 	}
-	#undef CLO_RW_THB
-	#undef CLO_RW_THB4
-	#undef CLO_RW_THB1
-	return (int) hipGetLastError();
-}
-
-unsigned clo_radixw_clear_words(int bits, unsigned tiles) {
-	const unsigned chunk = (unsigned) rw_chunk_for(tiles), chunks = (tiles + chunk - 1) / chunk;
-	return tiles > 1 ? ((chunks + 1u) << bits) : 0u;
-}
-size_t clo_radixw_partial_rows(size_t tiles) { const size_t chunk = (size_t) rw_chunk_for((unsigned) (tiles > 0xffffffffull ? 0xffffffffull : tiles)); return (tiles + chunk - 1) / chunk + 2; }
-
-int clo_radixw_launch_offsets(int bits, const clo_radix_counters& c, const unsigned** dbase, hipStream_t s) {
-	const unsigned chunk = (unsigned) rw_chunk_for(c.tiles);
-	const unsigned chunks = (c.tiles + chunk - 1) / chunk;
-	*dbase = nullptr;
-	#define CLO_RW_OFF1(B) case B: hipLaunchKernelGGL((clo_radixw_offsets1_kernel<(1 << B)>), dim3(1), dim3(256), 0, s, c.thist, c.tiles, c.toff); break
-	if (c.tiles == 1) {
-		switch (bits) {
-			CLO_RW_OFF1(1); CLO_RW_OFF1(2); CLO_RW_OFF1(3); CLO_RW_OFF1(4); CLO_RW_OFF1(5); CLO_RW_OFF1(6); CLO_RW_OFF1(7); CLO_RW_OFF1(8);
-			default: return CLO_HIP_EUNSUPPORTED;
-		}
-		return (int) hipGetLastError();
-	}
-	#undef CLO_RW_OFF1
-	#define CLO_RW_LB(B) case B: \
-		if (chunk == (unsigned) RW_CHUNK) hipLaunchKernelGGL((clo_radixw_offsets_lb_kernel<(1 << B), false, RW_CHUNK>), dim3(chunks), dim3(RW_CS_THREADS), 0, s, c.thist, c.tiles, chunks, c.partial, c.toff); \
-		else hipLaunchKernelGGL((clo_radixw_offsets_lb_kernel<(1 << B), false, RW_CHUNK_SMALL>), dim3(chunks), dim3(RW_CS_THREADS), 0, s, c.thist, c.tiles, chunks, c.partial, c.toff); \
-		break
-	switch (bits) {
-		CLO_RW_LB(1); CLO_RW_LB(2); CLO_RW_LB(3); CLO_RW_LB(4); CLO_RW_LB(5); CLO_RW_LB(6); CLO_RW_LB(7); CLO_RW_LB(8);
-		default: return CLO_HIP_EUNSUPPORTED;
-	}
-	#undef CLO_RW_LB
-	*dbase = c.partial + ((size_t) (chunks + 1u) << bits);
+	#undef CLO_RW_SC
 	return (int) hipGetLastError();
 }
 
diff --git a/cl_ops_amd/csrc/hip/clo_hip_runtime.hip b/cl_ops_amd/csrc/hip/clo_hip_runtime.hip
--- a/cl_ops_amd/csrc/hip/clo_hip_runtime.hip
+++ b/cl_ops_amd/csrc/hip/clo_hip_runtime.hip
@@ -167,20 +167,22 @@
 int clo_hip_event_record(void* event, void* stream) {
 	return (int) hipEventRecord((hipEvent_t) event, (hipStream_t) stream);
 }
-static clo_hip_env_t g_env = { CLO_MAX_SPINS, 2, 0, 0, 1 };
+static clo_hip_env_t g_env = { CLO_MAX_SPINS, 2, 0, 0, 1, 0 };
 static int g_env_read = 0;
 void clo_hip_env_refresh(void) {
-	clo_hip_env_t e = { CLO_MAX_SPINS, 2, 0, 0, 1 };
+	clo_hip_env_t e = { CLO_MAX_SPINS, 2, 0, 0, 1, 0 };
 	if (const char* m = getenv("CLO_MAX_SPINS")) e.max_spins = (unsigned) strtoul(m, nullptr, 10);
 	if (const char* m = getenv("CLO_RADIX_SWEEP")) e.radix_sweep = atoi(m) != 0 ? 1 : 0;
 	if (const char* m = getenv("CLO_R1_POOLS")) e.r1_pools = atoi(m);
 	e.no_digits = getenv("CLO_RADIX_NO_DIGITS") != nullptr;
 	if (const char* m = getenv("CLO_BITONIC_MERGE2")) e.bitonic_merge2 = atoi(m);
+	if (const char* m = getenv("CLO_RADIX_CHUNK_TILES")) e.chunk_tiles = atoi(m);
 	__atomic_store_n(&g_env.max_spins, e.max_spins, __ATOMIC_RELAXED);
 	__atomic_store_n(&g_env.radix_sweep, e.radix_sweep, __ATOMIC_RELAXED);
 	__atomic_store_n(&g_env.r1_pools, e.r1_pools, __ATOMIC_RELAXED);
 	__atomic_store_n(&g_env.no_digits, e.no_digits, __ATOMIC_RELAXED);
 	__atomic_store_n(&g_env.bitonic_merge2, e.bitonic_merge2, __ATOMIC_RELAXED);
+	__atomic_store_n(&g_env.chunk_tiles, e.chunk_tiles, __ATOMIC_RELAXED);
 	__atomic_store_n(&g_env_read, 1, __ATOMIC_RELEASE);
 }
 int clo_hip_event_synchronize(void* event) { return (int) hipEventSynchronize((hipEvent_t) event); }
diff --git a/include/clo_hip.h b/include/clo_hip.h
--- a/include/clo_hip.h
+++ b/include/clo_hip.h
@@ -251,6 +251,7 @@
 int clo_hip_radix_preload(void);
 size_t clo_hip_radix_workspace_bytes(size_t numel, int elem_size, int key_bits, int digit_bits);
 int clo_hip_radix_polls(size_t numel, int elem_size, int digit_bits);
+void clo_hip_radix_chunk_plan(size_t tiles, unsigned* chunk_tiles, unsigned* chunks);
 int clo_hip_radix_sort(const void* src, void* dst, void* tmp, size_t numel,
 	int elem_size, int key_shift, int key_bits, int key_kind, int digit_bits,
 	void* workspace, size_t workspace_bytes, void* stream);
```
